# rikuu/Gap2Seq

Measured on AMD Instinct MI355X. Metric: gaps filled/sec (whole node), k=31 synthetic 3 Mbp DBG, higher is better.
Workload: dtype u32

## Files before the change

### gap2seq_amd/csrc/d3_device.h

```cpp
#pragma once
#include <hip/hip_runtime_api.h>
#include <stdint.h>

#include "d2_device.h"
#include "fill_device.h"

#define G2S_D3_BLOCK_VARS 16u
#define G2S_RAND_BLOCK 4096u
#define G2S_RAND_WINDOW 160u
#define G2S_D3_TABLE_BUDGET (8u << 20)

#define G2S_D3_UNHANDLED 0x1u
#define G2S_D3_BUDGET 0x2u
#define G2S_D3_ANOMALY 0x4u

namespace g2s {

struct D3Gap {
  uint64_t arena_off;
  int32_t skip_thr;
  uint16_t lmf;
  uint8_t kind;
  uint8_t pad;
};

struct D3HostItem {
  uint32_t gap, n_segs;
  uint64_t seg_off;
  uint64_t rnd_off;
  uint32_t draws;
  uint32_t pad;
};
struct D3Side {
  D3HostItem* items = nullptr;
  GapOut* outs = nullptr;
  SegRec* segs = nullptr;
  uint32_t* rnd = nullptr;
  uint64_t cap_items = 0, cap_segs = 0, cap_rnd = 0;
  unsigned long long* count = nullptr;
};

struct alignas(16) D3Var {
  uint32_t gap, R, toff, tile0;
  uint32_t base, dmin, dspread, ns;
  uint64_t sub_at;
  uint32_t start_seg, start_t;
  int32_t len0, len1, n_len;
  uint32_t pad;
};
struct alignas(16) D3Trace {
  uint64_t arena_off;
  uint64_t sub_at;
  uint32_t gi;
  uint32_t off, want;
  uint16_t lmf, nsegs;
};
static_assert(sizeof(D3Var) == 64 && sizeof(D3Trace) == 32, "record layouts");

struct D3Summary {
  uint32_t status, unhandled, n_var, anomalies;
  unsigned long long host_items, host_segs, host_rnd;
  uint32_t handoff_waves, tiles;
  uint64_t table_entries, block_entries;
  uint64_t draws_min, draws_spread, draws_total;
  uint64_t xA, sA, xB, sB, xD, sD, segs, fill_bytes;
  uint32_t seg_gaps, filled;
  uint32_t rand_state[31];
  uint32_t trace_waves;
  uint32_t big_gaps;
  uint32_t traced_gaps;
  uint32_t spec_gaps;
  uint32_t handoff_gaps;
};
static_assert(sizeof(D3Summary) <= 512, "the lap stamps live at byte 512 of the summary's slot");

struct RandTables {
  const uint32_t* hi = nullptr;
  const uint32_t* mid = nullptr;
  const uint32_t* lane = nullptr;
};
void rand_tables_host(uint32_t* hi , uint32_t* mid , uint32_t* lane );

struct D3Work {
  uint32_t* ginfo = nullptr;
  uint32_t* dmin = nullptr;
  uint32_t* dspread = nullptr;
  uint32_t* base = nullptr;
  uint32_t* vrank = nullptr;
  uint32_t* var_gap = nullptr;
  uint32_t* var_R = nullptr;
  uint32_t* var_toff = nullptr;
  uint32_t* var_tile = nullptr;
  uint32_t* blk_toff = nullptr;
  uint32_t* blk_in = nullptr;
  uint32_t* dvar = nullptr;
  int32_t* skip = nullptr;
  uint32_t* tile_var = nullptr;
  D3Var* vdesc = nullptr;
  D3Trace* tdesc = nullptr;
  uint32_t* host_slot = nullptr;
  D3HostItem* hitems = nullptr;
  uint16_t* tab = nullptr;
  uint32_t* btab = nullptr;
  D3Summary* sum = nullptr;
  unsigned long long* fill_bytes = nullptr;
  uint32_t* link = nullptr;
  const D2Out* d2out = nullptr;
  const uint32_t* d2runs = nullptr;
  uint64_t* hops = nullptr;
  const char* spec_text = nullptr;
  const uint32_t* spec_res = nullptr;
  uint8_t* tab_bad = nullptr;
};
size_t d3_work_bytes(uint32_t n);
void d3_work_carve(void* p, uint32_t n, D3Work* w);

struct D3Params {
  int32_t k, skip_confident, all_paths, unique_paths;
  uint64_t max_states;
  uint64_t arena_base;
  uint32_t n;
  uint32_t has_skip;
  uint32_t seg_cap;
  uint32_t map_cap;
  uint32_t group_size;
  uint64_t sub_region;
  uint32_t laps;
  uint32_t self_clean;
  uint32_t base0, R0, d_in;
  const unsigned long long* d2_done;
  uint32_t d2_wgs;
  uint32_t restart;
};

hipError_t launch_rand_fill(hipStream_t st, uint32_t* rnd_all, const RandTables& rt, const D3Summary* sum_dev, uint64_t capacity,
                            uint64_t first_value = 0);

hipError_t launch_d3_sharded_classes(hipStream_t st, const D3Params& P, const D3Work& W, const GapOut* outs, const D3Gap* dgaps,
                                     bool summary_is_clean);
hipError_t launch_d3_sharded_tables(hipStream_t st, const D3Params& P, const D3Work& W, const GapOut* outs, const SubRec* sub,
                                    uint32_t* rnd_all, uint64_t rnd_capacity, uint32_t* group_fn );
hipError_t launch_d3_sharded_trace(hipStream_t st, const D3Params& P, const D3Work& W, const GapOut* outs, const SubRec* sub,
                                   const char* lastch_up, const char* lastch_dn, uint32_t* rnd_all, uint64_t rnd_capacity,
                                   void* results, char* arena, const D3Side& side, void* summary_host,
                                   hipEvent_t ev_d2 = nullptr );

hipError_t launch_rand_window(hipStream_t st, uint32_t* rnd_all, const uint32_t* link);

hipError_t launch_d3(hipStream_t st, const D3Params& P, const D3Work& W, const GapDev* gaps, const GapOut* outs,
                     const D3Gap* dgaps, const SubRec* sub, const char* lastch_up, const char* lastch_dn,
                     const RandTables& rt, uint32_t* rnd_all ,
                     uint64_t rnd_capacity, void* results ,
                     char* arena , const D3Side& side ,
                     void* summary_host ,
                     bool summary_is_clean ,
                     uint32_t* clean_words ,
                     hipEvent_t ev_chain = nullptr ,
                     hipEvent_t ev_d2 = nullptr ,
                     hipEvent_t ev_stop = nullptr );

hipError_t test_d3_tables(const uint32_t* segs, uint32_t nsegs, int32_t n_len, int32_t len0, int32_t len1, uint32_t start_seg,
                          const uint32_t* rnd, uint64_t rnd_cap, uint32_t base, uint32_t R, uint32_t dmin, uint32_t dspread,
                          uint16_t* entries, uint8_t* bad, uint32_t* anomalies);

uint64_t d3_chain_launches();

}
```

### gap2seq_amd/csrc/d3_device.hip

```cpp
#include "sync_debug.h"
#include <hip/hip_runtime.h>
#include <hip/hip_ext.h>

#include <algorithm>
#include <atomic>
#include <cstddef>
#include <cstdlib>
#include <cstring>
#include <mutex>
#include <set>
#include <vector>

#include "../../include/g2s.h"
#include "d3_device.h"
#include "envcache.hpp"

namespace {

using g2s::D3Gap;
using g2s::D3Params;
using g2s::D3Summary;
using g2s::D3Work;

__device__ __forceinline__ uint32_t uni(uint32_t x) { return (uint32_t)__builtin_amdgcn_readfirstlane((int)x); }

#define GI_CLASS(x) ((x) & 3u)
#define GI_FILLED 0x4u
#define GI_SKIPPED 0x8u
#define GI_BAD 0x10u
#define GI_MEM 0x20u
#define GI_PHASE_D 0x40u
#define D3_TILE 256u
#define GI_HOST 0x80u

__device__ __forceinline__ void stamp(const D3Work& W, int slot) {
  ((unsigned long long*)((char*)W.sum + 512))[slot] = wall_clock64();
}

__device__ __forceinline__ const SubRec* sub_of(const D3Params& P, const SubRec* sub, uint32_t i) {
  return sub + (uint64_t)(i / P.group_size) * P.sub_region;
}

__device__ __forceinline__ int gap_count(const GapOut& go, const D3Params& P, bool phase_d) {
  if (phase_d && !P.skip_confident && P.all_paths) return go.count_s;
  return go.c_count;
}

__device__ __forceinline__ uint32_t dpp_scan_add(uint32_t x) {
  x += (uint32_t)__builtin_amdgcn_update_dpp(0, (int)x, 0x111, 0xF, 0xF, false);
  x += (uint32_t)__builtin_amdgcn_update_dpp(0, (int)x, 0x112, 0xF, 0xF, false);
  x += (uint32_t)__builtin_amdgcn_update_dpp(0, (int)x, 0x114, 0xF, 0xF, false);
  x += (uint32_t)__builtin_amdgcn_update_dpp(0, (int)x, 0x118, 0xF, 0xF, false);
  x += (uint32_t)__builtin_amdgcn_update_dpp(0, (int)x, 0x142, 0xA, 0xF, false);
  x += (uint32_t)__builtin_amdgcn_update_dpp(0, (int)x, 0x143, 0xC, 0xF, false);
  return x;
}
__device__ __forceinline__ uint32_t sat_add(uint32_t a, uint32_t b) { const uint32_t t = a + b; return t < a ? 0xFFFFFFFFu : t; }
__device__ __forceinline__ uint32_t dpp_scan_sat(uint32_t x) {
  x = sat_add(x, (uint32_t)__builtin_amdgcn_update_dpp(0, (int)x, 0x111, 0xF, 0xF, false));
  x = sat_add(x, (uint32_t)__builtin_amdgcn_update_dpp(0, (int)x, 0x112, 0xF, 0xF, false));
  x = sat_add(x, (uint32_t)__builtin_amdgcn_update_dpp(0, (int)x, 0x114, 0xF, 0xF, false));
  x = sat_add(x, (uint32_t)__builtin_amdgcn_update_dpp(0, (int)x, 0x118, 0xF, 0xF, false));
  x = sat_add(x, (uint32_t)__builtin_amdgcn_update_dpp(0, (int)x, 0x142, 0xA, 0xF, false));
  x = sat_add(x, (uint32_t)__builtin_amdgcn_update_dpp(0, (int)x, 0x143, 0xC, 0xF, false));
  return x;
}
__device__ __forceinline__ uint32_t dpp_sum(uint32_t x) { return (uint32_t)__builtin_amdgcn_readlane((int)dpp_scan_add(x), 63); }
__device__ __forceinline__ unsigned long long wave_add64(unsigned long long v) {
  const unsigned long long lo = dpp_sum((uint32_t)v & 0xFFFFFFu), mid = dpp_sum((uint32_t)(v >> 24) & 0xFFFFFFu), hi = dpp_sum((uint32_t)(v >> 48));
  return lo + (mid << 24) + (hi << 48);
}

__device__ __forceinline__ uint32_t d3_classify_body(const D3Params& P, const D3Work& W, const GapOut* __restrict__ outs,
                                                     const D3Gap* __restrict__ dgaps, uint32_t first, uint32_t stride,
                                                     uint32_t* l_gi, uint32_t* l_dm, uint32_t* l_ds, int32_t* l_sk,
                                                     unsigned long long* red, bool one_wg) {
  const uint32_t n = P.n;
  unsigned long long xA = 0, sA = 0, xB = 0, sB = 0, xD = 0, sD = 0, segs = 0;
  uint32_t unhandled = 0, seg_gaps = 0, big = 0, traced = 0, spec = 0, handoff = 0;
  for (uint32_t i = first; i < n; i += stride) {
    const D3Gap dg = dgaps[i];
    const GapOut& go = outs[i];
    const uint32_t flags = go.flags, n_states = go.n_states, n_right = go.n_right, x_right = go.x_right, x_left = go.x_left;
    const uint32_t x_sub = go.x_sub, n_sub = go.n_sub, nseg_b = go.stat[3], dflags = go.dflags, stop0 = go.stop[0], stop1 = go.stop[1];
    const int c_count = go.c_count, n_len = go.n_len, len0 = go.len[0], len1 = go.len[1], reached_j = go.reached_j, count_s = go.count_s;
    const uint32_t n_xl = go.n_xl;
    const uint64_t sub_off = go.sub_off;
    uint32_t gi = 0, dmin = 0, spread = 0;
    if (dg.kind != 0) gi = GI_BAD;
    else {
      if (flags & (G2S_DEV_OVERFLOW_A | G2S_DEV_OVERFLOW_B)) unhandled++;
      else if ((uint64_t)n_states > P.max_states || (uint64_t)n_right > P.max_states) gi = GI_MEM;
      else {
        xA += x_right; sA += n_right; xB += x_left; sB += n_states; xD += x_sub; sD += n_sub;
        segs += nseg_b;
        seg_gaps++;
        if (flags & G2S_DEV_BIG) big++;
        if (dflags & G2S_DEVA_TRACED) traced++;
        if (dflags & G2S_DEVA_SPEC) spec++;
        const bool phase_d = c_count > 0 && n_len > 0;
        const bool by_host = phase_d && !(dflags & (G2S_DEVA_ANALYSED | G2S_DEVA_D2_PENDING));
        const int cnt = (phase_d && !P.skip_confident && P.all_paths) ? count_s : c_count;
        if (cnt > 0 && (!P.unique_paths || cnt == 1)) gi |= GI_FILLED;
        if (n_len > 0) gi |= ((uint32_t)reached_j & 0xFFu) << 8;
        if (phase_d) {
          gi |= GI_PHASE_D;
          if (by_host) gi |= GI_HOST;
          if (by_host || (!P.skip_confident && (dflags & G2S_DEVA_D2_PENDING))) handoff++;
          int lo_d = 0x7FFFFFFF, hi_d = 0;
#pragma unroll
          for (int q = 0; q < 2; q++) {
            if (q >= n_len) continue;
            const uint32_t sw = q ? stop1 : stop0;
            const int lq = q ? len1 : len0;
            int lo = (int)(sw & 0xFFFFu), hi = (int)(sw >> 16);
            if (lo > hi || hi > (int)dg.lmf) { lo = 0; hi = (int)dg.lmf; }
            lo_d = min(lo_d, 1 + lq - hi);
            hi_d = max(hi_d, 1 + lq - lo);
          }
          lo_d = max(lo_d, 1);
          hi_d = max(hi_d, lo_d);
          dmin = (uint32_t)lo_d;
          spread = (uint32_t)(hi_d - lo_d);
          gi |= spread ? 2u : 1u;
        }
      }
    }
    gi |= (uint32_t)dg.lmf << 16;
    W.ginfo[i] = gi;
    W.dmin[i] = dmin;
    W.dspread[i] = spread;
    W.skip[i] = dg.skip_thr;
    if (l_gi) { l_gi[i] = gi; l_dm[i] = dmin; l_ds[i] = spread; l_sk[i] = dg.skip_thr; }
    uint4 h0;
    const uint64_t ao = P.arena_base + dg.arena_off, sa = (uint64_t)(i / P.group_size) * P.sub_region + sub_off;
    h0.x = (uint32_t)ao; h0.y = (uint32_t)(ao >> 32); h0.z = (uint32_t)sa; h0.w = (uint32_t)(sa >> 32);
    ((uint4*)&W.tdesc[i])[0] = h0;
    (void)n_xl;
  }
  xA = wave_add64(xA); sA = wave_add64(sA); xB = wave_add64(xB); sB = wave_add64(sB); xD = wave_add64(xD); sD = wave_add64(sD);
  segs = wave_add64(segs);
  const unsigned long long cnts = wave_add64(((unsigned long long)unhandled << 32) | seg_gaps);
  big = dpp_sum(big);
  if ((threadIdx.x & 63u) == 0u && big) atomicAdd(&W.sum->big_gaps, big);
  traced = dpp_sum(traced);
  if ((threadIdx.x & 63u) == 0u && traced) atomicAdd(&W.sum->traced_gaps, traced);
  spec = dpp_sum(spec);
  if ((threadIdx.x & 63u) == 0u && spec) atomicAdd(&W.sum->spec_gaps, spec);
  handoff = dpp_sum(handoff);
  if ((threadIdx.x & 63u) == 0u && handoff) atomicAdd(&W.sum->handoff_gaps, handoff);
  const uint32_t wave = threadIdx.x >> 6, nwaves = blockDim.x >> 6;
  if ((threadIdx.x & 63u) == 0u) {
    unsigned long long* r = red + wave * 8u;
    r[0] = xA; r[1] = sA; r[2] = xB; r[3] = sB; r[4] = xD; r[5] = sD; r[6] = segs; r[7] = cnts;
  }
  __syncthreads();
  unsigned long long tot = 0;
  if (threadIdx.x < 8u) for (uint32_t w = 0; w < nwaves; w++) tot += red[w * 8u + threadIdx.x];
  unsigned long long all_cnts = 0;
  for (uint32_t w = 0; w < nwaves; w++) all_cnts += red[w * 8u + 7u];
  D3Summary* S = W.sum;
  if (threadIdx.x < 7u) {
    unsigned long long* dst = (unsigned long long*)&S->xA + threadIdx.x;
    if (one_wg) *dst = tot; else if (tot) atomicAdd(dst, tot);
  } else if (threadIdx.x == 7u) {
    if (one_wg) { S->unhandled = (uint32_t)(tot >> 32); S->seg_gaps = (uint32_t)tot; }
    else {
      if (tot >> 32) atomicAdd(&S->unhandled, (uint32_t)(tot >> 32));
      if (tot & 0xFFFFFFFFull) atomicAdd(&S->seg_gaps, (uint32_t)tot);
    }
  }
  return (uint32_t)(all_cnts >> 32);
}
__global__ __launch_bounds__(256) void g2s_d3_classify(const D3Params P, const D3Work W, const GapOut* __restrict__ outs,
                                                       const D3Gap* __restrict__ dgaps) {
  __shared__ unsigned long long red[4 * 8];
  (void)d3_classify_body(P, W, outs, dgaps, blockIdx.x * blockDim.x + threadIdx.x, gridDim.x * blockDim.x, nullptr, nullptr, nullptr, nullptr, red, false);
}

__device__ __forceinline__ void block_scan3(uint64_t& a, uint64_t& b, uint32_t& c, uint64_t* sh , uint64_t* tot_a, uint64_t* tot_b,
                                            uint32_t* tot_c) {
  const int lane = (int)(threadIdx.x & 63u), wave = (int)(threadIdx.x >> 6);
  uint64_t ia = a, ib = b;
  uint32_t ic = c;
  for (int o = 1; o < 64; o <<= 1) {
    const uint64_t ya = __shfl_up(ia, o), yb = __shfl_up(ib, o);
    const uint32_t yc = __shfl_up(ic, o);
    if (lane >= o) { ia += ya; ib += yb; ic += yc; }
  }
  if (lane == 63) { sh[wave * 3] = ia; sh[wave * 3 + 1] = ib; sh[wave * 3 + 2] = ic; }
  __syncthreads();
  uint64_t wa = lane < 16 ? sh[lane * 3] : 0, wb = lane < 16 ? sh[lane * 3 + 1] : 0, wc = lane < 16 ? sh[lane * 3 + 2] : 0;
  for (int o = 1; o < 16; o <<= 1) {
    const uint64_t ya = __shfl_up(wa, o), yb = __shfl_up(wb, o), yc = __shfl_up(wc, o);
    if (lane >= o) { wa += ya; wb += yb; wc += yc; }
  }
  *tot_a = __shfl(wa, 15); *tot_b = __shfl(wb, 15); *tot_c = (uint32_t)__shfl(wc, 15);
  const uint64_t oa = wave ? __shfl(wa, wave - 1) : 0, ob = wave ? __shfl(wb, wave - 1) : 0, oc = wave ? __shfl(wc, wave - 1) : 0;
  a = oa + ia - a; b = ob + ib - b; c = (uint32_t)oc + ic - c;
}

__device__ __forceinline__ void block_scan3_short(uint32_t& a, uint32_t& b, uint32_t& c, uint32_t* sh , uint32_t* tot_a, uint32_t* tot_b,
                                                  uint32_t* tot_c) {
  const int lane = (int)(threadIdx.x & 63u), wave = (int)(threadIdx.x >> 6);
  const uint32_t ia = dpp_scan_add(a), ib = dpp_scan_add(b), ic = dpp_scan_sat(c);
  if (lane == 63) { sh[wave * 3] = ia; sh[wave * 3 + 1] = ib; sh[wave * 3 + 2] = ic; }
  __syncthreads();
  uint32_t wa = lane < 16 ? sh[lane * 3] : 0u, wb = lane < 16 ? sh[lane * 3 + 1] : 0u, wc = lane < 16 ? sh[lane * 3 + 2] : 0u;
  wa = dpp_scan_add(wa); wb = dpp_scan_add(wb); wc = dpp_scan_sat(wc);
  *tot_a = (uint32_t)__builtin_amdgcn_readlane((int)wa, 15); *tot_b = (uint32_t)__builtin_amdgcn_readlane((int)wb, 15);
  *tot_c = (uint32_t)__builtin_amdgcn_readlane((int)wc, 15);
  const int wp = (int)uni((uint32_t)max(wave - 1, 0));
  const uint32_t oa = wave ? (uint32_t)__builtin_amdgcn_readlane((int)wa, wp) : 0u, ob = wave ? (uint32_t)__builtin_amdgcn_readlane((int)wb, wp) : 0u;
  const uint32_t oc = wave ? (uint32_t)__builtin_amdgcn_readlane((int)wc, wp) : 0u;
  a = oa + ia - a; b = ob + ib - b;
  const uint32_t incl_c = sat_add(oc, ic);
  c = incl_c == 0xFFFFFFFFu ? 0xFFFFFFFFu : incl_c - c;
}

__device__ __forceinline__ void d3_scan_body(const D3Params& P, const D3Work& W, const GapOut* __restrict__ outs, uint32_t* gi_a,
                                             uint32_t* dm_a, uint32_t* ds_a, const int32_t* sk_a, bool dual, uint32_t unhandled,
                                             uint64_t* sh , uint32_t* sh_f , bool short_list ) {
  const uint32_t t = threadIdx.x, n = P.n;
  const uint32_t per = (n + 1023u) / 1024u;
  const uint32_t lo = min(n, t * per), hi = min(n, lo + per);
  if (P.has_skip) {
    auto s_of = [&](uint32_t i) -> bool {
      if (i == 0) return false;
      const int thr = sk_a[i];
      if (thr < 0) return false;
      const uint32_t pg = gi_a[i - 1];
      return (pg & GI_FILLED) && !(pg & (GI_BAD | GI_MEM)) && (int)((pg >> 8) & 0xFFu) > thr;
    };
    bool o0 = false, o1 = true;
    for (uint32_t i = lo; i < hi; i++) { const bool s = s_of(i); o0 = s && !o0; o1 = s && !o1; }
    sh_f[t] = (o0 ? 1u : 0u) | (o1 ? 2u : 0u);
    __syncthreads();
    if (t < 64u) {
      auto apply = [](uint32_t f, bool in) -> bool { return in ? (f & 2u) != 0 : (f & 1u) != 0; };
      uint32_t f = 2u;
      for (uint32_t q = 0; q < 16u; q++) { const uint32_t g = sh_f[t * 16u + q]; f = (apply(g, apply(f, false)) ? 1u : 0u) | (apply(g, apply(f, true)) ? 2u : 0u); }
      uint32_t inc = f;
      for (int o = 1; o < 64; o <<= 1) {
        const uint32_t pv = (uint32_t)__shfl_up((int)inc, o);
        if ((int)t >= o) inc = (apply(inc, apply(pv, false)) ? 1u : 0u) | (apply(inc, apply(pv, true)) ? 2u : 0u);
      }
      uint32_t before = (uint32_t)__shfl_up((int)inc, 1);
      if (t == 0) before = 2u;
      bool cur = apply(before, false);
      for (uint32_t q = 0; q < 16u; q++) { const uint32_t g = sh_f[t * 16u + q]; sh_f[t * 16u + q] = cur ? 1u : 0u; cur = apply(g, cur); }
    }
    __syncthreads();
    bool sk = sh_f[t] != 0;
    for (uint32_t i = lo; i < hi; i++) {
      sk = s_of(i) && !sk;
      if (sk) {
        const uint32_t g = (gi_a[i] & ~3u) | GI_SKIPPED;
        gi_a[i] = g; dm_a[i] = 0; ds_a[i] = 0;
        if (dual) { W.ginfo[i] = g; W.dmin[i] = 0; W.dspread[i] = 0; }
      }
    }
    __threadfence_block();
    __syncthreads();
  }
  auto load8 = [&](uint32_t i0, uint32_t* g8, uint32_t* m8, uint32_t* s8) {
#pragma unroll
    for (int q = 0; q < 8; q++) {
      const uint32_t i = i0 + (uint32_t)q;
      const bool have = i < hi;
      g8[q] = have ? gi_a[i] : GI_SKIPPED;
      m8[q] = have ? dm_a[i] : 0u;
      s8[q] = have ? ds_a[i] : 0u;
    }
  };
  if (t == 0) stamp(W, 20);
  uint64_t sd = 0, ss = 0;
  uint32_t nv = 0;
  for (uint32_t i0 = lo; i0 < hi; i0 += 8u) {
    uint32_t g8[8], m8[8], s8[8];
    load8(i0, g8, m8, s8);
#pragma unroll
    for (int q = 0; q < 8; q++) {
      if (g8[q] & GI_SKIPPED) continue;
      sd += m8[q];
      if (GI_CLASS(g8[q]) == 2u) { nv++; ss += s8[q]; }
    }
  }
  uint64_t tot_d, tot_s;
  uint32_t V;
  if (short_list) {
    uint32_t a = (uint32_t)sd, b = (uint32_t)ss, ta, tb;
    block_scan3_short(a, b, nv, (uint32_t*)sh, &ta, &tb, &V);
    sd = a; ss = b; tot_d = ta; tot_s = tb;
  } else block_scan3(sd, ss, nv, sh, &tot_d, &tot_s, &V);
  if (t == 0) stamp(W, 21);
  const bool too_wide = tot_d + tot_s + P.base0 + P.R0 >= 0xFFFF0000ull || tot_s + P.R0 >= (uint64_t)G2S_D3_TABLE_BUDGET;
  uint64_t my_tab = 0, my_blk = 0;
  uint32_t my_tiles = 0;
  {
    uint64_t d = sd + P.base0, r = ss + P.R0;
    uint32_t v = nv;
    for (uint32_t i0 = lo; i0 < hi; i0 += 8u) {
      uint32_t g8[8], m8[8], s8[8];
      load8(i0, g8, m8, s8);
#pragma unroll
      for (int q = 0; q < 8; q++) {
        const uint32_t i = i0 + (uint32_t)q;
        if (i >= hi) break;
        W.base[i] = (uint32_t)d;
        W.vrank[i] = v;
        if (g8[q] & GI_SKIPPED) continue;
        d += m8[q];
        if (GI_CLASS(g8[q]) == 2u) {
          W.var_gap[v] = i;
          W.var_R[v] = (uint32_t)r;
          my_tab += r + 1u;
          my_tiles += (uint32_t)((r + D3_TILE) / D3_TILE);
          if (v % G2S_D3_BLOCK_VARS == 0u) my_blk += r + 1u;
          v++;
          r += s8[q];
        }
      }
    }
    if (t == 1023u) W.var_R[V] = (uint32_t)tot_s + P.R0;
  }
  if (t == 0) stamp(W, 22);
  uint64_t to = my_tab, bo = my_blk, T, TB;
  uint32_t tl = my_tiles, tiles;
  if (short_list) {
    uint32_t b = (uint32_t)std::min<uint64_t>(bo, 0xFFFFFFFFull), c = (uint32_t)std::min<uint64_t>(to, 0xFFFFFFFFull), tb, tc;
    block_scan3_short(tl, b, c, (uint32_t*)(sh + 48), &tiles, &tb, &tc);
    bo = b; to = c; TB = tb; T = tc == 0xFFFFFFFFu ? ~0ull : tc;
  } else block_scan3(to, bo, tl, sh + 48, &T, &TB, &tiles);
  const bool over = too_wide || T > (uint64_t)G2S_D3_TABLE_BUDGET || TB > (uint64_t)(G2S_D3_TABLE_BUDGET / 4u);
  if (!over) {
    uint64_t d = sd + P.base0, r = ss + P.R0;
    uint32_t v = nv;
    for (uint32_t i0 = lo; i0 < hi; i0 += 8u) {
      uint32_t g8[8], m8[8], s8[8];
      load8(i0, g8, m8, s8);
#pragma unroll
      for (int q = 0; q < 8; q++) {
        if (g8[q] & GI_SKIPPED) continue;
        const uint32_t base_i = (uint32_t)d;
        d += m8[q];
        if (GI_CLASS(g8[q]) != 2u) continue;
        W.var_toff[v] = (uint32_t)to;
        W.var_tile[v] = tl;
        {
          const uint32_t i = i0 + (uint32_t)q;
          uint4 h0, h1;
          h0.x = i; h0.y = (uint32_t)r; h0.z = (uint32_t)to; h0.w = tl;
          h1.x = base_i; h1.y = m8[q]; h1.z = s8[q]; h1.w = 0u;
          ((uint4*)&W.vdesc[v])[0] = h0;
          ((uint4*)&W.vdesc[v])[1] = h1;
        }
        tl += (uint32_t)((r + D3_TILE) / D3_TILE);
        to += r + 1u;
        if (v % G2S_D3_BLOCK_VARS == 0u) { W.blk_toff[v / G2S_D3_BLOCK_VARS] = (uint32_t)bo; bo += r + 1u; }
        v++;
        r += s8[q];
      }
    }
    if (t == 1023u) { W.var_toff[V] = (uint32_t)T; W.var_tile[V] = tiles; W.blk_toff[(V + G2S_D3_BLOCK_VARS - 1u) / G2S_D3_BLOCK_VARS] = (uint32_t)TB; }
    __threadfence_block();
    __syncthreads();
    for (uint32_t v = t; v < V; v += 1024u) {
      const uint4 h0 = ((const uint4*)&W.vdesc[v])[0];
      const uint32_t i = h0.x, r = h0.y, tl0 = h0.w;
      const GapOut& go = outs[i];
      uint4 h2, h3;
      const uint64_t sa = (uint64_t)(i / P.group_size) * P.sub_region + go.sub_off;
      ((uint32_t*)&W.vdesc[v])[7] = go.n_xl;
      h2.x = (uint32_t)sa; h2.y = (uint32_t)(sa >> 32); h2.z = go.start_seg; h2.w = go.start_t;
      h3.x = (uint32_t)go.len[0]; h3.y = (uint32_t)go.len[1]; h3.z = (uint32_t)go.n_len; h3.w = 0u;
      ((uint4*)&W.vdesc[v])[2] = h2;
      ((uint4*)&W.vdesc[v])[3] = h3;
      const uint32_t nt = (r + D3_TILE) / D3_TILE;
      for (uint32_t x = 0; x < nt; x++) W.tile_var[tl0 + x] = v;
    }
  }
  if (t == 0) {
    stamp(W, 23);
    D3Summary* S = W.sum;
    S->status = (unhandled ? G2S_D3_UNHANDLED : 0u) | (over ? G2S_D3_BUDGET : 0u);
    S->n_var = V;
    S->tiles = over ? 0u : tiles;
    S->table_entries = T;
    S->block_entries = TB;
    S->draws_min = tot_d;
    S->draws_spread = tot_s;
  }
}
#define D3_SCAN_LDS_GAPS 12288u
__global__ __launch_bounds__(1024) void g2s_d3_scan(const D3Params P, const D3Work W, const GapOut* __restrict__ outs) {
  extern __shared__ __attribute__((aligned(16))) uint32_t dyn[];
  __shared__ uint64_t sh[96];
  __shared__ uint32_t sh_f[1024];
  if (P.n <= D3_SCAN_LDS_GAPS) {
    uint32_t *l_gi = dyn, *l_dm = dyn + P.n, *l_ds = dyn + 2u * P.n;
    for (uint32_t i = threadIdx.x; i < P.n; i += 1024u) { l_gi[i] = W.ginfo[i]; l_dm[i] = W.dmin[i]; l_ds[i] = W.dspread[i]; }
    const uint32_t unhandled = W.sum->unhandled;
    __syncthreads();
    d3_scan_body(P, W, outs, l_gi, l_dm, l_ds, W.skip, true, unhandled, sh, sh_f, true);
    return;
  }
  d3_scan_body(P, W, outs, W.ginfo, W.dmin, W.dspread, W.skip, false, W.sum->unhandled, sh, sh_f, P.n <= 262144u);
}

__global__ __launch_bounds__(64) void g2s_rand_window(uint32_t* __restrict__ Wd, const uint32_t* __restrict__ link) {
  __shared__ uint32_t w[G2S_RAND_WINDOW + 2];
  const uint32_t lane = threadIdx.x;
  if (lane < 31u) w[lane] = link[lane];
  __syncthreads();
  for (uint32_t i = 31u; i < G2S_RAND_WINDOW; i += 3u) {
    if (lane < 3u) w[i + lane] = w[i + lane - 31u] + w[i + lane - 3u];
    __syncthreads();
  }
  for (uint32_t i = lane; i < G2S_RAND_WINDOW; i += 64u) Wd[i] = w[i];
}
__global__ __launch_bounds__(64) void g2s_rand_fill(uint32_t* __restrict__ Wd, const g2s::RandTables rt, const D3Summary* sum,
                                                    uint64_t capacity, uint64_t first_block) {
  __shared__ uint32_t base[G2S_RAND_WINDOW], s1[96], s2[64];
  if (sum && sum->status) return;
  const uint64_t need = sum ? min(capacity, sum->draws_min + sum->draws_spread + 64ull) : capacity;
  const uint32_t lane = threadIdx.x;
  for (uint32_t i = lane; i < G2S_RAND_WINDOW; i += 64u) base[i] = Wd[i];
  __syncthreads();
  const uint64_t nblocks = (need + G2S_RAND_BLOCK - 1u) / G2S_RAND_BLOCK;
  for (uint64_t B = first_block + blockIdx.x; B < nblocks; B += gridDim.x) {
    const uint32_t* ph = rt.hi + (size_t)((B >> 8) & 127u) * 31u;
    const uint32_t* pm = rt.mid + (size_t)(B & 255u) * 31u;
    const uint32_t* pl = rt.lane + (size_t)lane * 31u;
    for (uint32_t i = lane; i < 91u; i += 64u) {
      uint32_t a = 0;
#pragma unroll
      for (int j = 0; j < 31; j++) a += ph[j] * base[i + (uint32_t)j];
      s1[i] = a;
    }
    __syncthreads();
    if (lane < 61u) {
      uint32_t a = 0;
#pragma unroll
      for (int j = 0; j < 31; j++) a += pm[j] * s1[lane + (uint32_t)j];
      s2[lane] = a;
    }
    __syncthreads();
    uint32_t c[31], r[31];
#pragma unroll
    for (int j = 0; j < 31; j++) c[j] = pl[j];
#pragma unroll
    for (int i = 0; i < 31; i++) {
      uint32_t a = 0;
#pragma unroll
      for (int j = 0; j < 31; j++) a += c[j] * s2[i + j];
      r[i] = a;
    }
    uint32_t* out = Wd + 31u + B * G2S_RAND_BLOCK + (uint64_t)lane * 64u;
    const uint64_t room = capacity > B * G2S_RAND_BLOCK + (uint64_t)lane * 64u ? capacity - (B * G2S_RAND_BLOCK + (uint64_t)lane * 64u) : 0ull;
#pragma unroll
    for (int q = 0; q < 64; q++) {
      const uint32_t v = r[q % 31] + r[(q + 28) % 31];
      r[q % 31] = v;
      if ((uint64_t)q < room) out[q] = v;
    }
    __syncthreads();
  }
}

struct SegW { uint32_t node, depth_len, cnt, ts_tt, par01, par23, flags, pad; };

__device__ __forceinline__ int seg_nparents(uint32_t p01, uint32_t p23) {
  return ((p01 & 0xFFFFu) != 0xFFFFu) + ((p01 >> 16) != 0xFFFFu) + ((p23 & 0xFFFFu) != 0xFFFFu) + ((p23 >> 16) != 0xFFFFu);
}
__device__ __forceinline__ uint32_t seg_parent(uint32_t p01, uint32_t p23, int sel) {
  const uint32_t ps[4] = {p01 & 0xFFFFu, p01 >> 16, p23 & 0xFFFFu, p23 >> 16};
  uint32_t chosen = 0xFFFFu;
  int idx = 0;
#pragma unroll
  for (int q = 0; q < 4; q++)
    if (ps[q] != 0xFFFFu) { if (idx == sel) chosen = ps[q]; idx++; }
  return chosen;
}

__device__ __forceinline__ int pick_parent(uint32_t rv, int nb) { return nb == 2 ? (int)(rv & 1u) : nb == 3 ? (int)(rv % 3u) : (int)(rv & 3u); }

struct SegLite { uint32_t depth_len, par01, par23, flags; };

__device__ __forceinline__ SegLite seg_lite(const SegLite* p, int i) { return p[i]; }
__device__ __forceinline__ SegLite seg_lite(const SegW* p, int i) {
  SegLite l;
  l.depth_len = p[i].depth_len; l.par01 = p[i].par01; l.par23 = p[i].par23; l.flags = p[i].flags;
  return l;
}
template <typename SegT>
__device__ int d3_walk_count(int n_len, int len0, int len1, uint32_t start_seg, uint32_t start_t, int nsegs,
                             const SegT* __restrict__ segs, const uint32_t* lwin ,
                             uint32_t nwin , uint64_t avail ,
                             bool* bad) {
  int draws = 1;
  if (avail < 1 || nwin < 1) { *bad = true; return draws; }
  const int pick = n_len > 1 ? (int)((lwin[0] >> 1) & 1u) : 0;
  int d2 = pick ? len1 : len0;
  const uint32_t sg = (start_seg >> (16 * pick)) & 0xFFFFu;
  int i = sg == 0xFFFFu ? -1 : (int)sg;
  int t = (int)((start_t >> (16 * pick)) & 0xFFFFu);
  if (i < 0 || i >= nsegs) { *bad = true; return draws; }
  SegLite s = seg_lite(segs, i);
  bool ended = false;
  for (int guard = 0; d2 >= 0; guard++) {
    if (guard > 70000) { *bad = true; break; }
    const int run = min(t, d2);
    draws += run; d2 -= run; t -= run;
    if (t == 0 && (s.flags & G2S_SUB_SOURCE)) { ended = true; break; }
    if (d2 > 0) {
      const int nb = seg_nparents(s.par01, s.par23);
      if (nb == 0 || (nb > 1 && !(s.flags & G2S_SEG_ORDERED)) || (uint64_t)draws >= avail || (uint32_t)draws >= nwin) { *bad = true; break; }
      const uint32_t rv = nb > 1 ? lwin[draws] >> 1 : 0u;
      draws++;
      i = (int)seg_parent(s.par01, s.par23, nb == 1 ? 0 : pick_parent(rv, nb));
// ... 221 lines not shown
      const uint32_t v = uni(u == uni(u_first) ? v_unit : W.tile_var[tile]);
      const uint4* vp = (const uint4*)&W.vdesc[v];
      const uint4 h0 = vp[0], h1 = vp[1], h2 = vp[2], h3 = vp[3];
      static_assert(offsetof(g2s::D3Var, R) == 4 && offsetof(g2s::D3Var, toff) == 8 && offsetof(g2s::D3Var, tile0) == 12 && offsetof(g2s::D3Var, base) == 16 &&
                    offsetof(g2s::D3Var, dmin) == 20 && offsetof(g2s::D3Var, dspread) == 24 && offsetof(g2s::D3Var, ns) == 28 && offsetof(g2s::D3Var, sub_at) == 32 &&
                    offsetof(g2s::D3Var, start_seg) == 40 && offsetof(g2s::D3Var, len0) == 48 && offsetof(g2s::D3Var, len1) == 52 && offsetof(g2s::D3Var, n_len) == 56, "D3Var by words");
      const uint32_t R = uni(h0.y), toff = h0.z, tile0 = uni(h0.w), base = uni(h1.x), dmin = h1.y, dspread = h1.z, ns = uni(h1.w);
      const uint32_t d = (tile - tile0) * D3_TILE + u % D3_TILE;
      if (stw) stamp(W, 5);
      if (d > R || ns > D3_TAB_SEGS) continue;
      worked = true;
      const uint64_t sub_at = (uint64_t)uni(h2.x) | ((uint64_t)uni(h2.y) << 32);
      const uint64_t at = (uint64_t)base + d;
      bool bad = false;
      const int draws = d3_count_wave((int)uni(h3.z), (int)h3.x, (int)h3.y, h2.z, ns, (const SegW*)(sub + sub_at), rnd + at,
                                      min(win_cap, dmin + dspread + 1u), capacity > at ? capacity - at : 0ull, jmp, dep, &bad);
      if (stw) stamp(W, 6);
      const int dev = draws - (int)dmin;
      if (dev < 0 || dev > (int)dspread) bad = true;
      if ((tid & 63u) == 0u) {
        W.tab[(uint64_t)toff + d] = bad ? (uint16_t)0 : (uint16_t)dev;
        if (W.tab_bad) W.tab_bad[(uint64_t)toff + d] = bad ? 1 : 0;
        bad_any |= bad;
      }
    }
  }
  for (uint32_t tile = blockIdx.x; tile < tiles; tile += gridDim.x) {
    if (by_wave && tile == blockIdx.x && ns_first <= D3_TAB_SEGS) continue;
    const uint32_t v = tile == blockIdx.x ? v_first : W.tile_var[tile];
    const g2s::D3Var vd = W.vdesc[v];
    const uint32_t ns = vd.ns;
    if (by_wave && ns <= D3_TAB_SEGS) continue;
    worked = true;
    const uint32_t d0 = (tile - vd.tile0) * D3_TILE, d = d0 + tid;
    const uint64_t at0 = (uint64_t)vd.base + d0;
    const bool mine = d <= vd.R;
    const uint32_t want = min(win_cap, min(vd.R - d0, D3_TILE - 1u) + vd.dmin + vd.dspread + 1u);
    if (st0 && !by_wave) stamp(W, 5);
    __syncthreads();
    {
      const SegW* gs = (const SegW*)(sub + vd.sub_at);
      const uint32_t in_lds = ns <= D3_TAB_SEGS ? ns : 0u;
#pragma unroll
      for (uint32_t it = 0; it < D3_TAB_SEGS / 256u; it++) {
        const uint32_t q = tid + 256u * it;
        if (q >= in_lds) continue;
        SegLite l;
        l.depth_len = gs[q].depth_len; l.par01 = gs[q].par01; l.par23 = gs[q].par23; l.flags = gs[q].flags;
        lseg[q] = l;
      }
      for (uint32_t x = tid; x < want; x += 256u) lwin[x] = at0 + x < capacity ? rnd[at0 + x] : 0u;
    }
    __syncthreads();
    if (st0 && !by_wave) stamp(W, 6);
    if (mine) {
      bool bad = false;
      const uint64_t at = at0 + tid;
      const uint32_t nw = want > tid ? want - tid : 0u;
      const uint64_t av = capacity > at ? capacity - at : 0ull;
      const int draws = ns > D3_TAB_SEGS
                            ? d3_walk_count(vd.n_len, vd.len0, vd.len1, vd.start_seg, vd.start_t, (int)ns, (const SegW*)(sub + vd.sub_at), lwin + tid, nw, av, &bad)
                            : d3_walk_count_lite(vd.n_len, vd.len0, vd.len1, vd.start_seg, (int)ns, lseg, lwin + tid, nw, av, &bad);
      const int dev = draws - (int)vd.dmin;
      if (dev < 0 || dev > (int)vd.dspread) bad = true;
      W.tab[(uint64_t)vd.toff + d] = bad ? (uint16_t)0 : (uint16_t)dev;
      if (W.tab_bad) W.tab_bad[(uint64_t)vd.toff + d] = bad ? 1 : 0;
      bad_any |= bad;
    }
  }
  if (bad_any) atomicAdd(&W.sum->anomalies, 1u);
  if (st0) stamp(W, 7);
  if (P.laps && (tid & 63u) == 0u) {
    unsigned long long* laps = (unsigned long long*)((char*)W.sum + 512);
    if (worked) atomicMax(&laps[32], wall_clock64());
    if (tid == 0) atomicMax(&laps[33], wall_clock64());
  }
}

__device__ __forceinline__ void d3_blocks_body(const D3Work& W, uint64_t first, uint64_t stride) {
  const D3Summary* S = W.sum;
  const uint32_t V = S->n_var;
  const uint32_t NB = (V + G2S_D3_BLOCK_VARS - 1u) / G2S_D3_BLOCK_VARS;
  const uint64_t TB = S->block_entries;
  for (uint64_t e = first; e < TB; e += stride) {
    uint32_t lo = 0, hi = NB;
    while (hi - lo > 1u) { const uint32_t mid = (lo + hi) >> 1; if ((uint64_t)W.blk_toff[mid] <= e) lo = mid; else hi = mid; }
    const uint32_t b = lo;
    uint32_t d = (uint32_t)(e - W.blk_toff[b]);
    const uint32_t v1 = min(V, (b + 1u) * G2S_D3_BLOCK_VARS);
    for (uint32_t v = b * G2S_D3_BLOCK_VARS; v < v1; v++) d += W.tab[(uint64_t)W.var_toff[v] + d];
    W.btab[e] = d;
  }
}
__global__ __launch_bounds__(256) void g2s_d3_blocks(const D3Work W) {
  if (W.sum->status) return;
  d3_blocks_body(W, (uint64_t)blockIdx.x * blockDim.x + threadIdx.x, (uint64_t)gridDim.x * blockDim.x);
}

__device__ __forceinline__ void d3_chain_body(const D3Work& W, const uint32_t* __restrict__ Wd, uint32_t* total_dev ,
                                              uint32_t base0 = 0u, uint32_t d_in = 0u) {
  D3Summary* S = W.sum;
  const uint32_t V = S->n_var;
  const uint32_t NB = (V + G2S_D3_BLOCK_VARS - 1u) / G2S_D3_BLOCK_VARS;
  __shared__ uint32_t l_toff[2048], l_in[2048];
  const bool in_lds = NB <= 2048u;
  if (in_lds) for (uint32_t b = threadIdx.x; b < NB; b += blockDim.x) l_toff[b] = W.blk_toff[b];
  __syncthreads();
  if (threadIdx.x == 0) {
    uint32_t d = d_in;
    if (in_lds) for (uint32_t b = 0; b < NB; b++) { l_in[b] = d; d = W.btab[(uint64_t)l_toff[b] + d]; }
    else for (uint32_t b = 0; b < NB; b++) { W.blk_in[b] = d; d = W.btab[(uint64_t)W.blk_toff[b] + d]; }
    W.dvar[V] = d;
    *total_dev = d;
  }
  __threadfence_block();
  __syncthreads();
  for (uint32_t b = threadIdx.x; b < NB; b += blockDim.x) {
    uint32_t d = in_lds ? l_in[b] : W.blk_in[b];
    if (in_lds) W.blk_in[b] = d;
    const uint32_t v0 = b * G2S_D3_BLOCK_VARS, v1 = min(V, (b + 1u) * G2S_D3_BLOCK_VARS);
    uint32_t toff[G2S_D3_BLOCK_VARS];
#pragma unroll
    for (uint32_t q = 0; q < G2S_D3_BLOCK_VARS; q++) toff[q] = v0 + q < v1 ? W.var_toff[v0 + q] : 0u;
#pragma unroll
    for (uint32_t q = 0; q < G2S_D3_BLOCK_VARS; q++)
      if (v0 + q < v1) { W.dvar[v0 + q] = d; d += W.tab[(uint64_t)toff[q] + d]; }
  }
  const uint64_t total = (uint64_t)base0 + S->draws_min + *total_dev;
  if (threadIdx.x == 0) S->draws_total = total;
  if (threadIdx.x < 31u) {
    const uint32_t w = Wd[total + threadIdx.x];
    S->rand_state[threadIdx.x] = w;
    if (W.link) W.link[threadIdx.x] = w;
  }
}
__global__ __launch_bounds__(1024) void g2s_d3_chain(const D3Work W, const uint32_t* __restrict__ Wd, uint32_t base0, uint32_t d_in) {
  __shared__ uint32_t total_dev;
  if (W.sum->status) return;
  d3_chain_body(W, Wd, &total_dev, base0, d_in);
}
__global__ __launch_bounds__(256) void g2s_d3_groupfn(const D3Work W, uint32_t R0, uint32_t* __restrict__ fn) {
  const D3Summary* S = W.sum;
  if (S->status) return;
  const uint32_t V = S->n_var;
  const uint32_t NB = (V + G2S_D3_BLOCK_VARS - 1u) / G2S_D3_BLOCK_VARS;
  for (uint32_t d0 = blockIdx.x * blockDim.x + threadIdx.x; d0 <= R0; d0 += gridDim.x * blockDim.x) {
    uint32_t d = d0;
    for (uint32_t b = 0; b < NB; b++) d = W.btab[(uint64_t)W.blk_toff[b] + d];
    fn[d0] = d;
  }
}

#define D3_FRONT_GAPS 3072u
__global__ __launch_bounds__(1024) void g2s_d3_front(const D3Params P, const D3Work W, const GapOut* __restrict__ outs,
                                                     const D3Gap* __restrict__ dgaps) {
  __shared__ uint64_t sh[96];
  __shared__ unsigned long long red[16 * 8];
  __shared__ uint32_t sh_f[1024];
  __shared__ uint32_t l_gi[D3_FRONT_GAPS], l_dm[D3_FRONT_GAPS], l_ds[D3_FRONT_GAPS];
  __shared__ int32_t l_sk[D3_FRONT_GAPS];
  if (threadIdx.x == 0) stamp(W, 0);
  const uint32_t unhandled = d3_classify_body(P, W, outs, dgaps, threadIdx.x, 1024u, l_gi, l_dm, l_ds, l_sk, red, true);
  __syncthreads();
  if (threadIdx.x == 0) stamp(W, 1);
  d3_scan_body(P, W, outs, l_gi, l_dm, l_ds, l_sk, true, unhandled, sh, sh_f, true);
  if (threadIdx.x == 0) stamp(W, 2);
}

template <bool RESTART>
__device__ __forceinline__ bool d3_handoff_body(const D3Params& P, const D3Work& W, const GapOut* __restrict__ outs,
                                                const SubRec* __restrict__ sub, const uint32_t* __restrict__ rnd, uint64_t capacity,
                                                const g2s::D3Side& side, uint32_t i0, const uint32_t* ldvar, const uint16_t* ltab,
                                                const uint32_t* ltoff, unsigned long long* lcur) {
  D3Summary* S = W.sum;
  const int lane = (int)(threadIdx.x & 63u);
  const uint32_t mine = i0 + (uint32_t)lane;
  const bool have = mine < P.n;
  uint32_t gi = 0, my_off = 0, my_want = 0, my_ns = 0;
  if (have) {
    gi = W.ginfo[mine];
    const uint32_t dmin = W.dmin[mine];
    const GapOut& go = outs[mine];
    my_ns = go.n_xl;
    if ((gi & GI_PHASE_D) && !P.skip_confident) {
      const uint32_t dfl = go.dflags;
      if ((dfl & G2S_DEVA_D2_PENDING) && (dfl & G2S_DEVA_D2_FAILED)) gi |= GI_HOST;
    }
    my_want = dmin;
    if constexpr (RESTART) {
      if (GI_CLASS(gi) == 2u) {
        const uint32_t dspread = W.dspread[mine];
        const uint4 h0 = ((const uint4*)&W.tdesc[mine])[0];
        const SegW* gs = (const SegW*)(sub + ((uint64_t)h0.z | ((uint64_t)h0.w << 32)));
        const uint32_t nwin = min(P.map_cap + D3_TILE, dmin + dspread + 1u);
        bool bad = false;
        const int draws = my_ns > D3_TAB_SEGS
                              ? d3_walk_count(go.n_len, go.len[0], go.len[1], go.start_seg, go.start_t, (int)my_ns, gs, rnd, nwin, capacity, &bad)
                              : d3_walk_count_lite(go.n_len, go.len[0], go.len[1], go.start_seg, (int)my_ns, gs, rnd, nwin, capacity, &bad);
        const int dev = draws - (int)dmin;
        if (dev < 0 || dev > (int)dspread) bad = true;
        if (bad) atomicAdd(&S->anomalies, 1u);
        else my_want += (uint32_t)dev;
      }
    } else {
      const uint32_t vr = W.vrank[mine], base = W.base[mine];
      const uint32_t dv = ldvar ? ldvar[vr] : W.dvar[vr];
      my_off = base + dv;
      if (GI_CLASS(gi) == 2u) my_want += ltab ? (uint32_t)ltab[ltoff[vr] + dv] : (uint32_t)W.tab[(uint64_t)W.var_toff[vr] + dv];
    }
    ((uint4*)&W.tdesc[mine])[1] = make_uint4(gi, my_off, my_want, (gi >> 16) | (min(my_ns, 0xFFFFu) << 16));
  }
  const bool host = have && (gi & GI_HOST) != 0u;
  const uint64_t hm = __ballot(host);
  for (uint64_t m = hm; m; m &= m - 1) {
    const int l = __builtin_ctzll(m);
    const uint32_t i = i0 + (uint32_t)l;
    const uint32_t off = (uint32_t)__shfl((int)my_off, l), want = (uint32_t)__shfl((int)my_want, l), ns = (uint32_t)__shfl((int)my_ns, l);
    unsigned long long it = 0, so = 0, ro = 0;
    if (lane == 0) {
      if (lcur) {
        it = atomicAdd(&lcur[0], 1ull); so = atomicAdd(&lcur[1], (unsigned long long)ns); ro = atomicAdd(&lcur[2], ((unsigned long long)want + 8ull) / 8ull);
      } else {
        it = atomicAdd(&S->host_items, 1ull);
        so = atomicAdd(&S->host_segs, (unsigned long long)ns);
        ro = atomicAdd(&S->host_rnd, ((unsigned long long)want + 8ull) / 8ull);
      }
    }
    it = __shfl(it, 0); so = __shfl(so, 0); ro = __shfl(ro, 0);
    if (it >= side.cap_items || so + ns > side.cap_segs || ro + (want + 8ull) / 8ull > side.cap_rnd || (uint64_t)off + want + 1ull > capacity) {
      if (lane == 0) { atomicAdd(&S->anomalies, 1u); W.host_slot[i] = 0xFFFFFFFFu; }
      continue;
    }
    if (lane == 0) {
      g2s::D3HostItem h;
      h.gap = i; h.n_segs = ns; h.seg_off = so; h.rnd_off = ro; h.draws = want; h.pad = 0;
      W.hitems[it] = h;
      W.host_slot[i] = (uint32_t)it;
      uint32_t* hi = (uint32_t*)&side.items[it];
      hi[0] = i; hi[1] = ns; hi[2] = (uint32_t)so; hi[3] = (uint32_t)(so >> 32); hi[4] = (uint32_t)ro; hi[5] = (uint32_t)(ro >> 32); hi[6] = want;
    }
  }
  if (hm != 0ull) __threadfence_system();
  (void)sub; (void)rnd; (void)outs;
  if constexpr (RESTART) {
    const uint32_t nv = (uint32_t)__popcll(__ballot(have && GI_CLASS(gi) == 2u));
    uint32_t mx = have ? my_want : 0u;
    for (int o = 32; o > 0; o >>= 1) mx = max(mx, (uint32_t)__shfl_xor((int)mx, o));
    if (lane == 0) {
      if (nv) atomicAdd(&S->n_var, nv);
      atomicMax((unsigned long long*)&S->draws_total, (unsigned long long)mx);
    }
  }
  return hm != 0ull;
}
__global__ __launch_bounds__(64) void g2s_d3_handoff(const D3Params P, const D3Work W, const GapOut* __restrict__ outs,
                                                     const SubRec* __restrict__ sub, const uint32_t* __restrict__ rnd, uint64_t capacity,
                                                     const g2s::D3Side side) {
  D3Summary* S = W.sum;
  const bool dead = S->status != 0u;
  if (!dead) (void)d3_handoff_body<false>(P, W, outs, sub, rnd, capacity, side, blockIdx.x * 64u, nullptr, nullptr, nullptr, nullptr);
  if ((threadIdx.x & 63u) == 0u) {
    asm volatile("s_waitcnt vmcnt(0)" ::: "memory");
    const unsigned int done = atomicAdd(&S->handoff_waves, 1u) + 1u;
    if (done == gridDim.x) {
      const unsigned long long items = atomicAdd(&S->host_items, 0ull);
      const uint32_t anomalies = atomicAdd(&S->anomalies, 0u);
      __hip_atomic_store(side.count, (items & 0x7FFFFFFFFFFFFFFFull) | ((unsigned long long)((anomalies || dead) ? 1u : 0u) << 63),
                         __ATOMIC_RELEASE, __HIP_MEMORY_SCOPE_SYSTEM);
    }
  }
}
__global__ __launch_bounds__(256) void g2s_d3_restart(const D3Params P, const D3Work W, const GapOut* __restrict__ outs,
                                                      const D3Gap* __restrict__ dgaps, const SubRec* __restrict__ sub,
                                                      const uint32_t* __restrict__ rnd, uint64_t capacity, const g2s::D3Side side) {
  __shared__ unsigned long long red[4 * 8];
  D3Summary* S = W.sum;
  (void)d3_classify_body(P, W, outs, dgaps, blockIdx.x * 256u + threadIdx.x, gridDim.x * 256u, nullptr, nullptr, nullptr, nullptr, red, false);
  (void)d3_handoff_body<true>(P, W, outs, sub, rnd, capacity, side, blockIdx.x * 256u + (threadIdx.x & ~63u), nullptr, nullptr, nullptr, nullptr);
  if ((threadIdx.x & 63u) == 0u) {
    asm volatile("s_waitcnt vmcnt(0)" ::: "memory");
    const unsigned int done = atomicAdd(&S->handoff_waves, 1u) + 1u;
    if (done == gridDim.x * 4u) {
      const unsigned long long items = atomicAdd(&S->host_items, 0ull);
      const uint32_t anomalies = atomicAdd(&S->anomalies, 0u), unhandled = atomicAdd(&S->unhandled, 0u);
      S->status = unhandled ? G2S_D3_UNHANDLED : 0u;
      __hip_atomic_store(side.count, (items & 0x7FFFFFFFFFFFFFFFull) | ((unsigned long long)((anomalies || unhandled) ? 1u : 0u) << 63),
                         __ATOMIC_RELEASE, __HIP_MEMORY_SCOPE_SYSTEM);
    }
  }
}
#define D3_BACK_TAB 24576u
#define D3_CHAIN_GAPS 768u
#define D3_CHAIN_ROOM 4096u
__global__ __launch_bounds__(1024) void g2s_d3_back(const D3Params P, const D3Work W, const GapOut* __restrict__ outs,
                                                    const SubRec* __restrict__ sub, const uint32_t* __restrict__ Wd, uint64_t capacity,
                                                    const g2s::D3Side side) {
  __shared__ uint32_t total_dev;
  __shared__ unsigned long long lcur[3];
  if (threadIdx.x < 3u) lcur[threadIdx.x] = 0ull;
  __shared__ uint16_t ltab[D3_BACK_TAB];
  __shared__ uint32_t ltoff[1025], ldvar[1025];
  D3Summary* S = W.sum;
  if (threadIdx.x == 0) stamp(W, 8);
  const uint32_t status = S->status, V = S->n_var;
  const uint64_t T = S->table_entries;
  if (status) {
    if (threadIdx.x == 0) __hip_atomic_store(side.count, 1ull << 63, __ATOMIC_RELEASE, __HIP_MEMORY_SCOPE_SYSTEM);
    return;
  }
  const bool in_lds = T <= (uint64_t)D3_BACK_TAB && V <= 1024u;
  if (in_lds) {
    for (uint32_t e = threadIdx.x; e < (uint32_t)T; e += 1024u) ltab[e] = W.tab[e];
    if (threadIdx.x <= V) ltoff[threadIdx.x] = W.var_toff[threadIdx.x];
    __syncthreads();
    if (threadIdx.x == 0) {
      stamp(W, 9);
      uint32_t d = 0;
      for (uint32_t v = 0; v < V; v++) { ldvar[v] = d; d += ltab[ltoff[v] + d]; }
      ldvar[V] = d;
      total_dev = d;
    }
    __syncthreads();
    if (threadIdx.x <= V) W.dvar[threadIdx.x] = ldvar[threadIdx.x];
    const uint64_t total = S->draws_min + total_dev;
    if (threadIdx.x == 0) S->draws_total = total;
    if (threadIdx.x < 31u) {
      const uint32_t w = Wd[total + threadIdx.x];
      S->rand_state[threadIdx.x] = w;
      if (W.link) W.link[threadIdx.x] = w;
    }
  } else {
    d3_blocks_body(W, threadIdx.x, 1024u);
    __threadfence();
    __syncthreads();
    d3_chain_body(W, Wd, &total_dev);
    __threadfence();
    __syncthreads();
  }
  if (threadIdx.x == 0) stamp(W, 10);
  for (uint32_t i0 = (threadIdx.x >> 6) * 64u; i0 < P.n; i0 += 1024u)
    (void)d3_handoff_body<false>(P, W, outs, sub, Wd + 31, capacity, side, i0, in_lds ? ldvar : nullptr, in_lds ? ltab : nullptr,
                          in_lds ? ltoff : nullptr, lcur);
  __syncthreads();
  if (threadIdx.x == 0) {
    stamp(W, 11);
    const unsigned long long items = lcur[0];
    S->host_items = items; S->host_segs = lcur[1]; S->host_rnd = lcur[2];
    const uint32_t anomalies = atomicAdd(&S->anomalies, 0u);
    __hip_atomic_store(side.count, (items & 0x7FFFFFFFFFFFFFFFull) | ((unsigned long long)(anomalies ? 1u : 0u) << 63), __ATOMIC_RELEASE,
                       __HIP_MEMORY_SCOPE_SYSTEM);
    stamp(W, 12);
  }
}

template <int NW, bool CHAIN = false>
__global__ __launch_bounds__(64 * NW) void g2s_d3_trace(const D3Params P, const D3Work W, GapOut* __restrict__ outs,
                                                   const SubRec* __restrict__ sub, const char* __restrict__ chu,
                                                   const char* __restrict__ chd, const uint32_t* __restrict__ rnd,
                                                   uint64_t capacity, g2s_result* __restrict__ results,
                                                   char* __restrict__ arena, uint32_t* __restrict__ summary_host,
                                                   const g2s::D3Side side, uint32_t* __restrict__ clean_words ,
                                                   uint32_t chain_room ) {
  static_assert(!CHAIN || NW == 4, "the chain's loads are laid out for 256 threads");
  extern __shared__ __attribute__((aligned(16))) uint32_t lds[];
  D3Summary* S = W.sum;
  const uint32_t i = blockIdx.x;
  constexpr int NT = 64 * NW;
  const int tid = (int)threadIdx.x, lane = tid & 63;
  const bool w0 = tid < 64;
#ifdef G2S_SYNC_DEBUG
  auto wg_sync = [&]() { if constexpr (NW > 1) __syncthreads(); else { g2s_sync_jitter(0xD3u); g2s_wait_all(); asm volatile("s_waitcnt lgkmcnt(0)" ::: "memory"); __builtin_amdgcn_wave_barrier(); } };
#else
  auto wg_sync = [&]() { if constexpr (NW > 1) __syncthreads(); else { asm volatile("s_waitcnt lgkmcnt(0)" ::: "memory"); __builtin_amdgcn_wave_barrier(); } };
#endif
  SegW* segs = (SegW*)lds;
  static_assert(sizeof(g2s_result) == 112, "g2s_result layout");
  unsigned long long* laps = (unsigned long long*)((char*)W.sum + 512);
  const unsigned long long tk0 = P.laps ? wall_clock64() : 0ull;
  unsigned long long tk1 = 0, tk2 = 0, tk3 = 0, hops = 0, tkm = 0;
  if (P.laps && i == 0 && tid == 0) laps[13] = tk0;
  const uint32_t status = uni(S->status);
  struct {
    uint32_t flags, dflags, start_seg, start_t, sub_vertices, sub_edges, top_level;
    int32_t c_count, n_len, len[2], reached_j, count_s;
  } go;
  {
    const GapOut& g = outs[i];
    go.top_level = uni(g.top_level);
    go.flags = uni(g.flags); go.dflags = uni(g.dflags); go.start_seg = uni(g.start_seg); go.start_t = uni(g.start_t);
    go.sub_vertices = uni(g.sub_vertices); go.sub_edges = uni(g.sub_edges);
    go.c_count = (int32_t)uni((uint32_t)g.c_count); go.n_len = (int32_t)uni((uint32_t)g.n_len);
    go.len[0] = (int32_t)uni((uint32_t)g.len[0]); go.len[1] = (int32_t)uni((uint32_t)g.len[1]);
    go.reached_j = (int32_t)uni((uint32_t)g.reached_j); go.count_s = (int32_t)uni((uint32_t)g.count_s);
  }
  g2s::D3Trace td;
  uint32_t c_dmin = 0, c_vr = 0, c_base = 0, c_V = 0, c_dev = 0, c_step = 0, c_ns = 0, c_handoff = 0;
  uint64_t c_T = 0, c_draws_min = 0;
  if constexpr (!CHAIN) {
    const uint4 h0 = ((const uint4*)&W.tdesc[i])[0], h1 = ((const uint4*)&W.tdesc[i])[1];
    td.arena_off = (uint64_t)uni(h0.x) | ((uint64_t)uni(h0.y) << 32);
    td.sub_at = (uint64_t)uni(h0.z) | ((uint64_t)uni(h0.w) << 32);
    td.gi = uni(h1.x); td.off = uni(h1.y); td.want = uni(h1.z);
    td.lmf = (uint16_t)(uni(h1.w) & 0xFFFFu); td.nsegs = (uint16_t)(uni(h1.w) >> 16);
  } else {
    const uint32_t n = P.n;
    const uint32_t toff_len = (n + 2u) & ~1u;
    const uint32_t tab_room = chain_room > toff_len ? min(chain_room - toff_len, D3_CHAIN_ROOM) & ~1u : 0u;
    uint16_t* ltoff = (uint16_t*)lds;
    uint16_t* ltab = ltoff + toff_len;
    const uint4 h0 = ((const uint4*)&W.tdesc[i])[0];
    uint32_t gi_w = W.ginfo[i], dm_w = W.dmin[i], vr_w = W.vrank[i], bs_w = W.base[i], ns_w = outs[i].n_xl, V_w = S->n_var;
    c_T = S->table_entries;
    c_draws_min = S->draws_min;
    uint32_t hg_w = S->handoff_gaps;
    static_assert(D3_CHAIN_ROOM <= 8u * 2u * 256u && D3_CHAIN_GAPS <= 4u * 256u, "the unrolled loads below cover the room");
    uint32_t tw[8], ow[4];
    const uint32_t* tab32 = (const uint32_t*)W.tab;
    const uint32_t tab_last = max(tab_room / 2u, 1u) - 1u;
#pragma unroll
    for (uint32_t q = 0; q < 8u; q++) tw[q] = tab32[min((uint32_t)tid + 256u * q, tab_last)];
#pragma unroll
    for (uint32_t q = 0; q < 4u; q++) ow[q] = W.var_toff[min((uint32_t)tid + 256u * q, n)];
#pragma unroll
    for (uint32_t q = 0; q < 8u; q++) { const uint32_t x = (uint32_t)tid + 256u * q; if (x < tab_room / 2u) ((uint32_t*)ltab)[x] = tw[q]; }
#pragma unroll
    for (uint32_t q = 0; q < 4u; q++) { const uint32_t x = (uint32_t)tid + 256u * q; if (x <= n) ltoff[x] = (uint16_t)ow[q]; }
    td.arena_off = (uint64_t)uni(h0.x) | ((uint64_t)uni(h0.y) << 32);
    td.sub_at = (uint64_t)uni(h0.z) | ((uint64_t)uni(h0.w) << 32);
    td.gi = uni(gi_w); td.off = 0u; td.want = 0u;
    td.lmf = (uint16_t)(td.gi >> 16);
    c_ns = uni(ns_w);
    td.nsegs = (uint16_t)min(c_ns, 0xFFFFu);
    c_dmin = uni(dm_w); c_vr = uni(vr_w); c_base = uni(bs_w); c_V = uni(V_w); c_handoff = uni(hg_w);
    c_T = (uint64_t)uni((uint32_t)c_T) | ((uint64_t)uni((uint32_t)(c_T >> 32)) << 32);
    c_draws_min = (uint64_t)uni((uint32_t)c_draws_min) | ((uint64_t)uni((uint32_t)(c_draws_min >> 32)) << 32);
    __syncthreads();
    if (!status) {
      const bool in_lds = c_T <= (uint64_t)tab_room && c_T <= 0xFFFFull && c_V <= n;
      const uint32_t v0 = min(c_vr, c_V), var = GI_CLASS(td.gi) == 2u && v0 < c_V ? 1u : 0u;
      const uint32_t v_end = i + 1u == n ? c_V : v0 + var;
      uint32_t d = 0, dv = 0, d1 = 0;
      if (in_lds) {
        uint32_t t = ltoff[0];
        for (uint32_t v = 0; v < v_end; v++) {
          const uint32_t tn = ltoff[v + 1u];
          if (v == v0) dv = d;
          d += ltab[min(t + d, tab_room - 1u)];
          if (v == v0) d1 = d;
          t = tn;
        }
      } else {
        for (uint32_t v = 0; v < v_end; v++) {
          if (v == v0) dv = d;
          d += W.tab[min((uint64_t)W.var_toff[v] + d, (uint64_t)G2S_D3_TABLE_BUDGET - 1u)];
          if (v == v0) d1 = d;
        }
      }
      if (v_end <= v0) dv = d;
      c_dev = uni(dv);
      c_step = var ? uni(d1) - c_dev : 0u;
      td.off = c_base + c_dev;
      td.want = c_dmin + c_step;
      if (i + 1u == n && w0) {
        const uint32_t d_all = uni(d);
        const uint64_t total = c_draws_min + d_all;
        if (lane == 0) {
          W.dvar[c_V] = d_all;
          __hip_atomic_store((unsigned long long*)&S->draws_total, (unsigned long long)total, __ATOMIC_RELAXED, __HIP_MEMORY_SCOPE_AGENT);
        }
        if (lane < 31) {
          const uint32_t w = (rnd - 31)[total + (uint32_t)lane];
          __hip_atomic_store(&S->rand_state[lane], w, __ATOMIC_RELAXED, __HIP_MEMORY_SCOPE_AGENT);
          if (W.link) W.link[lane] = w;
        }
        __threadfence();
      }
    }
    __syncthreads();
  }
  bool d2_lost = false;
  if ((go.dflags & G2S_DEVA_D2_PENDING) && !(go.dflags & (G2S_DEVA_RUNS | G2S_DEVA_D2_FAILED)) && !P.skip_confident) {
    uint32_t v = go.dflags;
    for (uint32_t spin = 0; spin < (1u << 22) && !(v & (G2S_DEVA_RUNS | G2S_DEVA_D2_FAILED)); spin++) {
      __builtin_amdgcn_s_sleep(8);
      v = uni(__hip_atomic_load(&outs[i].dflags, __ATOMIC_ACQUIRE, __HIP_MEMORY_SCOPE_AGENT));
    }
    __builtin_amdgcn_fence(__ATOMIC_ACQUIRE, "agent");
    go.dflags = v;
    go.sub_vertices = uni(__hip_atomic_load(&outs[i].sub_vertices, __ATOMIC_RELAXED, __HIP_MEMORY_SCOPE_AGENT));
    go.sub_edges = uni(__hip_atomic_load(&outs[i].sub_edges, __ATOMIC_RELAXED, __HIP_MEMORY_SCOPE_AGENT));
    if (!(v & (G2S_DEVA_RUNS | G2S_DEVA_D2_FAILED))) d2_lost = true;
  }
  uint32_t h_it = 0xFFFFFFFFu, h_ns = 0, h_want = 0;
  uint64_t h_so = 0, h_ro = 0;
  bool lost_counted = false;
  if constexpr (CHAIN) {
    const bool counts = (td.gi & GI_HOST) || ((td.gi & GI_PHASE_D) && !P.skip_confident && (go.dflags & G2S_DEVA_D2_PENDING));
    if (!status && !d2_lost) {
      if ((td.gi & GI_PHASE_D) && !P.skip_confident && (go.dflags & G2S_DEVA_D2_PENDING) && (go.dflags & G2S_DEVA_D2_FAILED)) td.gi |= GI_HOST;
      if (td.gi & GI_HOST) {
        __shared__ unsigned long long l_hand[3];
        if (tid == 0) {
          const uint32_t ns = c_ns, want = td.want;
          unsigned long long it = atomicAdd(&S->host_items, 1ull);
          const unsigned long long so = atomicAdd(&S->host_segs, (unsigned long long)ns);
          const unsigned long long ro = atomicAdd(&S->host_rnd, ((unsigned long long)want + 8ull) / 8ull);
          if (it >= side.cap_items || so + ns > side.cap_segs || ro + (want + 8ull) / 8ull > side.cap_rnd || (uint64_t)td.off + want + 1ull > capacity) {
            atomicAdd(&S->anomalies, 1u);
            it = 0xFFFFFFFFull;
          } else {
            uint32_t* hi = (uint32_t*)&side.items[it];
            hi[0] = i; hi[1] = ns; hi[2] = (uint32_t)so; hi[3] = (uint32_t)(so >> 32); hi[4] = (uint32_t)ro; hi[5] = (uint32_t)(ro >> 32); hi[6] = want;
            __threadfence_system();
          }
          l_hand[0] = it; l_hand[1] = so; l_hand[2] = ro;
        }
        __syncthreads();
        h_it = uni((uint32_t)l_hand[0]);
        h_so = (uint64_t)uni((uint32_t)l_hand[1]) | ((uint64_t)uni((uint32_t)(l_hand[1] >> 32)) << 32);
        h_ro = (uint64_t)uni((uint32_t)l_hand[2]) | ((uint64_t)uni((uint32_t)(l_hand[2] >> 32)) << 32);
        h_ns = c_ns; h_want = td.want;
      }
    }
    if (tid == 0 && (counts || (c_handoff == 0u && i == 0u))) {
      if (d2_lost && !status) { atomicAdd(&S->anomalies, 1u); lost_counted = true; }
      asm volatile("s_waitcnt vmcnt(0)" ::: "memory");
      const unsigned int done = counts ? atomicAdd(&S->handoff_waves, 1u) + 1u : 0u;
      if (done == c_handoff) {
        const unsigned long long items = atomicAdd(&S->host_items, 0ull);
        const uint32_t anomalies = atomicAdd(&S->anomalies, 0u);
        __hip_atomic_store(side.count, (items & 0x7FFFFFFFFFFFFFFFull) | ((unsigned long long)((anomalies || status) ? 1u : 0u) << 63),
                           __ATOMIC_RELEASE, __HIP_MEMORY_SCOPE_SYSTEM);
      }
    }
  }
  if ((go.dflags & G2S_DEVA_D2_PENDING) && (go.dflags & G2S_DEVA_D2_FAILED) && !(td.gi & GI_HOST) && (td.gi & GI_PHASE_D)) d2_lost = true;
  uint32_t gsp_all = 0, gsp_sent = 0;
  auto leave = [&](uint32_t fill_len) {
    if (!w0) return;
    uint32_t last = 0;
    if (lane == 0) {
      if (P.laps) {
        const unsigned long long tk4 = wall_clock64();
        atomicMax(&laps[14], tk1 ? tk1 - tk0 : 0ull); atomicMax(&laps[15], tk2 ? tk2 - tk1 : 0ull);
        atomicMax(&laps[16], tk3 ? tk3 - tk2 : 0ull); atomicMax(&laps[17], ((tk4 - tk0) << 24) | ((td.gi & GI_HOST) ? 1ull << 23 : 0ull) | (unsigned long long)(i & 0x7FFFFFu)); atomicMax(&laps[18], tk4);
        atomicMax(&laps[19], ((tk2 ? tk2 - tk1 : 0ull) << 32) | (hops << 16) | (tkm ? tkm - tk1 : 0ull));
        if ((P.laps >> 4) == i + 1u) { laps[26] = tk0; laps[27] = tk1; laps[28] = tkm; laps[29] = tk2; laps[30] = tk3; laps[31] = tk4; }
      }
      const uint32_t c = i & 63u, n = gridDim.x;
      const unsigned long long before = atomicAdd(&W.fill_bytes[c * 16u], (unsigned long long)fill_len | (1ull << 40));
      if (gsp_all) atomicAdd(&W.fill_bytes[c * 16u + 1u], (unsigned long long)gsp_all | ((unsigned long long)gsp_sent << 32));
      if ((uint32_t)(before >> 40) + 1u == (n + 63u - c) / 64u) last = atomicAdd(&S->trace_waves, 1u) + 1u == min(n, 64u) ? 1u : 0u;
    }
    if (P.self_clean && (uint32_t)lane < sizeof(GapOut) / 4u) ((uint32_t*)&outs[i])[lane] = 0u;
    if (!uni(last)) return;
    if (P.d2_done && lane == 0)
      for (uint32_t spin = 0; spin < (1u << 22) && __hip_atomic_load(P.d2_done, __ATOMIC_ACQUIRE, __HIP_MEMORY_SCOPE_AGENT) < (unsigned long long)P.d2_wgs; spin++)
        __builtin_amdgcn_s_sleep(8);
    uint32_t* src = (uint32_t*)S;
    if (P.laps && lane == 0) laps[24] = wall_clock64();
    static_assert(sizeof(D3Summary) <= 512, "two words a lane");
    const uint32_t s0 = __hip_atomic_load(src + lane, __ATOMIC_RELAXED, __HIP_MEMORY_SCOPE_AGENT);
    const uint32_t s1 = __hip_atomic_load(src + 64 + lane, __ATOMIC_RELAXED, __HIP_MEMORY_SCOPE_AGENT);
    const unsigned long long* cl = (const unsigned long long*)(src + 256 + 32 * lane);
    const unsigned long long c0 = __hip_atomic_load(cl, __ATOMIC_RELAXED, __HIP_MEMORY_SCOPE_AGENT);
    const unsigned long long c1 = __hip_atomic_load(cl + 1, __ATOMIC_RELAXED, __HIP_MEMORY_SCOPE_AGENT);
    summary_host[lane] = s0;
    summary_host[64 + lane] = s1;
    ((unsigned long long*)(summary_host + 256 + 32 * lane))[0] = c0;
    ((unsigned long long*)(summary_host + 256 + 32 * lane))[1] = c1;
    if (P.self_clean) {
      src[lane] = 0u; src[64 + lane] = 0u;
      ((unsigned long long*)(src + 256 + 32 * lane))[0] = 0ull;
      ((unsigned long long*)(src + 256 + 32 * lane))[1] = 0ull;
    }
    if (P.self_clean && clean_words && lane < 32) clean_words[lane] = 0u;
    if (P.laps && lane == 0) { asm volatile("s_waitcnt vmcnt(0)" ::: "memory"); laps[25] = wall_clock64(); }
  };
  if (status) { leave(0u); return; }
  if (d2_lost) {
    if (tid == 0) { if (!lost_counted) atomicAdd(&S->anomalies, 1u); arena[td.arena_off + td.lmf] = '\0'; }
    asm volatile("s_waitcnt vmcnt(0)" ::: "memory");
    leave(0u);
    return;
  }
  const uint32_t gi = td.gi;
  if ((go.dflags & G2S_DEVA_TRACED) && !(gi & (GI_BAD | GI_SKIPPED | GI_MEM | GI_HOST)) && (gi & GI_PHASE_D)) {
    asm volatile("s_waitcnt vmcnt(0)" ::: "memory");
    leave((go.top_level >> 16) - (go.top_level & 0xFFFFu));
    return;
  }
  const bool spec = (go.dflags & G2S_DEVA_SPEC) != 0u && W.spec_text != nullptr && !(gi & (GI_BAD | GI_SKIPPED | GI_MEM | GI_HOST)) && (gi & GI_PHASE_D);
  const int spec_stop = (int)(go.top_level & 0xFFFFu), spec_len = (int)(go.top_level >> 16);
  const unsigned long long spec_chain = spec ? ((unsigned long long)uni(outs[i].stat[6]) | ((unsigned long long)uni(outs[i].stat[7]) << 32)) : 0ull;
  struct { uint16_t lmf; } dg = {td.lmf};
  const uint64_t abs_off = td.arena_off;
  char* buf = arena + abs_off;
  const int k = P.k;
  uint32_t rw[24];
#pragma unroll
  for (int q = 0; q < 24; q++) rw[q] = 0u;
  int left_fuz = 0;
  bool spec_rec = false;
  uint32_t g_all = 0, g_sent = 0;
  auto finish = [&](uint32_t fill_len) {
    if (!w0) return;
    const uint64_t fo = abs_off + (uint64_t)((int)dg.lmf - left_fuz);
    rw[1] = (uint32_t)left_fuz;
    rw[4] = (uint32_t)fo; rw[5] = (uint32_t)(fo >> 32);
    rw[6] = fill_len;
    uint32_t mine = 0u;
#pragma unroll
    for (int q = 0; q < 24; q++) mine = lane == q ? rw[q] : mine;
    if (spec_rec) {
      const uint32_t was = lane < 28 ? W.spec_res[(size_t)i * 28u + (uint32_t)lane] : 0u;
      if (__ballot(lane < 28 && was != mine) == 0ull) return;
    }
    if (lane < 28) ((uint32_t*)&results[i])[lane] = mine;
  };
  if (gi & (GI_BAD | GI_SKIPPED | GI_MEM)) {
    rw[3] = (gi & GI_BAD) ? G2S_GAP_BAD_FLANK : (gi & GI_SKIPPED) ? G2S_GAP_SKIPPED : G2S_GAP_MEM_EXCEEDED;
    if (gi & GI_MEM) rw[0] = (uint32_t)-1;
    if (tid == 0) buf[dg.lmf] = '\0';
    finish(0u);
    leave(0u);
    return;
  }
  const bool phase_d = (gi & GI_PHASE_D) != 0;
  rw[20] = (uint32_t)go.c_count;
  rw[21] = (uint32_t)go.n_len;
  rw[22] = (uint32_t)go.len[0];
  rw[23] = (uint32_t)go.len[1];
  rw[3] = (go.flags & (G2S_DEV_Q7_A | G2S_DEV_Q7_B | G2S_DEV_Q7_D)) ? G2S_GAP_Q7 : 0u;
  rw[0] = (uint32_t)((phase_d && !P.skip_confident && P.all_paths) ? go.count_s : go.c_count);
  const bool by_runs = phase_d && !P.skip_confident && (go.dflags & G2S_DEVA_RUNS) != 0u && W.d2out != nullptr;
  uint32_t n_runs = 0;
  const uint32_t* runs = nullptr;
  if (phase_d && !P.skip_confident) {
    rw[8] = go.sub_vertices; rw[10] = go.sub_edges;
    rw[16] = go.sub_vertices; rw[18] = go.sub_edges;
    if (by_runs) {
      const uint4 o0 = ((const uint4*)&W.d2out[i])[0], o1 = ((const uint4*)&W.d2out[i])[1];
      runs = W.d2runs + 2ull * uni(o0.x);
      n_runs = uni(o0.y);
      rw[8] = uni(o0.z); rw[10] = uni(o0.w); rw[12] = uni(o1.x); rw[14] = uni(o1.y); rw[16] = uni(o1.z); rw[18] = uni(o1.w);
    }
  }
  if (!phase_d) {
    if (tid == 0) buf[dg.lmf] = '\0';
    finish(0u);
    leave(0u);
    return;
  }
  if (gi & GI_HOST) {
    const uint32_t it = CHAIN ? h_it : uni(W.host_slot[i]);
    if (it != 0xFFFFFFFFu) {
      const g2s::D3HostItem* hp = &W.hitems[CHAIN ? 0u : it];
      const uint64_t so = CHAIN ? h_so : (uint64_t)uni((uint32_t)hp->seg_off) | ((uint64_t)uni((uint32_t)(hp->seg_off >> 32)) << 32);
      const uint64_t ro = CHAIN ? h_ro : (uint64_t)uni((uint32_t)hp->rnd_off) | ((uint64_t)uni((uint32_t)(hp->rnd_off >> 32)) << 32);
      const uint32_t ns = CHAIN ? h_ns : uni(hp->n_segs), want = CHAIN ? h_want : uni(hp->draws);
      const GapOut& g = outs[i];
      if ((uint32_t)tid < sizeof(GapOut) / 4u) ((uint32_t*)&side.outs[it])[tid] = ((const uint32_t*)&g)[tid];
      const uint4* src = (const uint4*)(sub + td.sub_at);
      uint4* dst = (uint4*)(side.segs + so);
      for (uint32_t w = (uint32_t)tid; w < 2u * ns; w += (uint32_t)NT) dst[w] = src[w];
      for (uint32_t w = (uint32_t)tid; w < (want + 8u) / 8u; w += (uint32_t)NT) {
        uint32_t pk8 = 0u;
#pragma unroll
        for (uint32_t x = 0; x < 8u; x++) {
          const uint32_t at = 8u * w + x;
          if (at <= want) pk8 |= ((rnd[td.off + at] >> 1) % 12u) << (4u * x);
        }
        side.rnd[ro + w] = pk8;
      }
      __threadfence_system();
      if constexpr (NW > 1) __syncthreads();
      if (tid == 0) {
        __hip_atomic_store(&side.items[it].pad, 1u, __ATOMIC_RELEASE, __HIP_MEMORY_SCOPE_SYSTEM);
      }
    }
    leave(0u);
    return;
  }
  const bool big = (uint32_t)td.nsegs > P.seg_cap && by_runs && W.hops != nullptr;
  const uint32_t nsegs = big ? (uint32_t)td.nsegs : min((uint32_t)td.nsegs, P.seg_cap);
  const SegW* gsegs = (const SegW*)(sub + td.sub_at);
  uint64_t* ghop = big ? W.hops + td.sub_at / 2u : nullptr;
  uint32_t* cmap = lds + (size_t)P.seg_cap * 8u;
  uint32_t* lwin = cmap + P.map_cap;
  const uint32_t nwin = min(td.want, P.map_cap);
  for (uint32_t x = (uint32_t)tid; x < nwin; x += (uint32_t)NT) lwin[x] = (uint64_t)td.off + x < capacity ? rnd[td.off + x] : 0u;
  if (!big) {
    const uint4* src = (const uint4*)gsegs;
    uint4* dst = (uint4*)segs;
    for (uint32_t w = (uint32_t)tid; w < 2u * nsegs; w += (uint32_t)NT) dst[w] = src[w];
  }
  __syncthreads();
  if (P.laps) tk1 = wall_clock64();
  const bool sink_safe = (go.dflags & G2S_DEVA_SINK_SAFE) != 0;
  auto outside_safe = [&](uint32_t x) -> bool {
    for (uint32_t q = 0; q < nsegs; q++) {
      const uint32_t onode = segs[q].node, ots = segs[q].ts_tt;
      const int ts = (ots & 0x7FFFu) == 0x7FFFu ? -1 : (int)(ots & 0x7FFFu);
      const uint32_t oidx = onode >> 1;
      const int tq = (onode & 1u) ? (int)oidx - (int)x : (int)x - (int)oidx;
      if (tq >= 0 && tq <= ts) return tq <= (int)segs[q].pad ? (ots & 0x8000u) != 0 : (ots & 0x80000000u) != 0;
    }
    return sink_safe;
  };
  const uint32_t* lruns = nullptr;
  auto run_verdict = [&](uint32_t x, uint32_t* rlo, uint32_t* rhi) -> bool {
    const uint32_t* rr = lruns ? lruns : runs;
    uint32_t lo = 0, hi = n_runs;
    while (lo < hi) { const uint32_t mid = (lo + hi) >> 1; if (rr[2u * mid] <= x) lo = mid + 1u; else hi = mid; }
    if (lo > 0u) {
      const uint32_t f = rr[2u * (lo - 1u)], l = rr[2u * (lo - 1u) + 1u];
      if (x <= (l & 0x7FFFFFFFu)) { *rlo = f; *rhi = l & 0x7FFFFFFFu; return (l >> 31) != 0u; }
    }
    *rlo = x; *rhi = x;
    return sink_safe;
  };
  const uint32_t off = td.off;
  const uint64_t avail = min((uint64_t)nwin, capacity > off ? capacity - off : 0ull);
  const int want = (int)td.want;
  const int n_len = go.n_len, len0 = go.len[0], len1 = go.len[1];
  int draws = 1;
  auto value = [&](uint32_t x) -> uint32_t { return uni(lwin[x]); };
  const int pick = (n_len > 1 && avail > 0) ? (int)((value(0) >> 1) & 1u) : 0;
  int d2 = pick ? len1 : len0;
  const int len = d2;
  bool bad = false, ended = false;
  if ((uint32_t)len + 1u > P.map_cap || (!big && (uint32_t)td.nsegs > P.seg_cap) || td.want > P.map_cap) bad = true;
  uint2* hop = (uint2*)(lwin + P.map_cap);
  uint2* pk = hop + P.seg_cap;
  for (uint32_t q = (uint32_t)tid; q < nsegs && !big; q += (uint32_t)NT) {
    const uint32_t dl = segs[q].depth_len, p01 = segs[q].par01, p23 = segs[q].par23, fl = segs[q].flags;
    const int d0 = (int)(dl & 0xFFFFu);
    const int nb = seg_nparents(p01, p23);
    const int64_t at = 1 + (int64_t)len - d0;
    uint32_t w;
    if (nb == 0 || (nb > 1 && !(fl & G2S_SEG_ORDERED)) || at < 1 || (uint64_t)at >= avail) w = 0x80000000u;
    else {
      const uint32_t rv = nb > 1 ? lwin[at] >> 1 : 0u;
      w = seg_parent(p01, p23, nb == 1 ? 0 : pick_parent(rv, nb));
      if (w >= nsegs) w = 0x80000000u;
    }
    pk[q] = make_uint2(dl, w | ((fl & G2S_SUB_SOURCE) ? 0x40000000u : 0u));
  }
  wg_sync();
  int nh = 0;
  {
    const uint32_t sg = (go.start_seg >> (16 * pick)) & 0xFFFFu;
    int si = sg == 0xFFFFu ? -1 : (int)sg;
    const int t0 = (int)((go.start_t >> (16 * pick)) & 0xFFFFu);
    if (si < 0 || si >= (int)nsegs || avail < 1) bad = true;
    uint32_t last = 0x80000000u;
    const int hop_cap = (int)(big ? nsegs : min(nsegs, P.seg_cap));
    unsigned long long chain_hash = 14695981039346656037ull;
    const uint32_t L = nsegs > 1u ? 32u - (uint32_t)__builtin_clz(nsegs - 1u) : 0u;
    const bool jump = !big && L * nsegs <= 2u * P.map_cap;
    uint16_t* J = (uint16_t*)cmap;
    if (jump) {
      for (uint32_t q = (uint32_t)tid; q < nsegs && L > 0u; q += (uint32_t)NT) { const uint32_t y = pk[q].y; J[q] = (uint16_t)((y & 0xC0000000u) ? q : (y & 0xFFFFu)); }
      wg_sync();
      for (uint32_t j = 1; j < L; j++) {
        for (uint32_t q = (uint32_t)tid; q < nsegs; q += (uint32_t)NT) J[j * nsegs + q] = J[(j - 1u) * nsegs + J[(j - 1u) * nsegs + q]];
        wg_sync();
      }
    }
    if (!bad && jump) {
      bool ended_chain = false;
      for (uint32_t h0 = 0; h0 < (uint32_t)hop_cap; h0 += 64u) {
        const uint32_t h = h0 + (uint32_t)lane;
        const bool in = h < (uint32_t)hop_cap;
        uint32_t sq = (uint32_t)si;
        for (uint32_t j = 0; j < L; j++) { const uint32_t to = J[j * nsegs + sq]; sq = ((h >> j) & 1u) ? to : sq; }
        const uint32_t y = pk[sq].y;
        const uint32_t on = (uint32_t)__popcll(__ballot(in && !(y & 0xC0000000u)));
        if (in && (uint32_t)lane <= on) hop[h].y = sq;
        if (on < min(64u, (uint32_t)hop_cap - h0)) {
          nh = (int)(h0 + on) + 1;
          last = uni((uint32_t)__shfl((int)y, (int)on));
          ended_chain = true;
          break;
        }
      }
      if (!ended_chain) { nh = hop_cap; bad = true; }
      if (!bad && spec) {
        asm volatile("s_waitcnt lgkmcnt(0)" ::: "memory");
        __builtin_amdgcn_wave_barrier();
        for (int h = 0; h < nh; h++) chain_hash = (chain_hash ^ (unsigned long long)uni(hop[h].y)) * 1099511628211ull;
      }
    }
    if (!bad && !big && !jump) {
      if (spec) {
        for (;;) {
          if (nh >= hop_cap) { bad = true; break; }
          last = uni(pk[si].y);
          chain_hash = (chain_hash ^ (unsigned long long)(uint32_t)si) * 1099511628211ull;
          if (lane == 0) hop[nh].y = (uint32_t)si;
          nh++;
          if (last & 0xC0000000u) break;
          si = (int)(last & 0xFFFFu);
        }
      } else {
        uint32_t hv = 0u;
        for (;;) {
          if (nh >= hop_cap) { bad = true; break; }
          last = uni(pk[si].y);
          hv = lane == (nh & 63) ? (uint32_t)si : hv;
          nh++;
          if ((nh & 63) == 0) hop[nh - 64 + lane].y = hv;
          if (last & 0xC0000000u) break;
          si = (int)(last & 0xFFFFu);
        }
        if (!bad && (nh & 63) != 0 && lane < (nh & 63)) hop[(nh & ~63) + lane].y = hv;
      }
    }
    if (!bad && !big) {
      if (P.laps) hops = (unsigned long long)nh;
      if (!bad && spec && pick == 0 && len == spec_len && (last & 0x40000000u) && chain_hash == spec_chain) {
        gsp_all = 1u;
        leave((uint32_t)(spec_len - spec_stop));
        return;
      }
    }
    if (!bad && big) {
      for (;;) {
        if (nh >= hop_cap) { bad = true; break; }
        if (P.laps) hops++;
        const uint32_t dl = uni(gsegs[si].depth_len), p01 = uni(gsegs[si].par01), p23 = uni(gsegs[si].par23), fl = uni(gsegs[si].flags);
        const int d0 = (int)(dl & 0xFFFFu);
        const int nb = seg_nparents(p01, p23);
        const int64_t at = 1 + (int64_t)len - d0;
        uint32_t w;
        if (nb == 0 || (nb > 1 && !(fl & G2S_SEG_ORDERED)) || at < 1 || (uint64_t)at >= avail) w = 0x80000000u;
        else {
          const uint32_t rv = nb > 1 ? value((uint32_t)at) >> 1 : 0u;
          w = seg_parent(p01, p23, nb == 1 ? 0 : pick_parent(rv, nb));
          if (w >= nsegs) w = 0x80000000u;
        }
        last = w | ((fl & G2S_SUB_SOURCE) ? 0x40000000u : 0u);
        if (lane == 0) ghop[nh] = (uint64_t)(uint32_t)si << 32;
        nh++;
        if (last & 0xC0000000u) break;
        si = (int)(last & 0xFFFFu);
      }
      __threadfence_block();
// ... 143 lines not shown
}

}

namespace g2s {

void rand_tables_host(uint32_t* hi, uint32_t* mid, uint32_t* lane) {
  auto mulmod = [](const uint32_t* a, const uint32_t* b, uint32_t* out) {
    uint32_t c[61];
    for (int i = 0; i < 61; i++) c[i] = 0;
    for (int i = 0; i < 31; i++) {
      if (!a[i]) continue;
      for (int j = 0; j < 31; j++) c[i + j] += a[i] * b[j];
    }
    for (int d = 60; d >= 31; d--) { c[d - 3] += c[d]; c[d - 31] += c[d]; }
    for (int i = 0; i < 31; i++) out[i] = c[i];
  };
  auto power = [&](uint64_t N, uint32_t* q) {
    uint32_t r[31] = {0}, b[31] = {0}, t[31];
    r[0] = 1; b[1] = 1;
    for (; N; N >>= 1) {
      if (N & 1) { mulmod(r, b, t); for (int i = 0; i < 31; i++) r[i] = t[i]; }
      mulmod(b, b, t);
      for (int i = 0; i < 31; i++) b[i] = t[i];
    }
    for (int i = 0; i < 31; i++) q[i] = r[i];
  };
  auto series = [&](uint64_t step, int count, uint32_t* out) {
    uint32_t s[31];
    power(step, s);
    for (int i = 0; i < 31; i++) out[i] = i == 0 ? 1u : 0u;
    for (int a = 1; a < count; a++) mulmod(out + (size_t)(a - 1) * 31, s, out + (size_t)a * 31);
  };
  series(1ull << 20, 128, hi);
  series(4096, 256, mid);
  series(64, 64, lane);
}

size_t d3_work_bytes(uint32_t n) {
  const size_t per = (((size_t)n + 64) * 4 + 63) & ~(size_t)63;
  return 14 * per + 64 * 128 + (size_t)G2S_D3_TABLE_BUDGET * 2 + (size_t)(G2S_D3_TABLE_BUDGET / 4u) * 4 + 4096 +
         ((size_t)n + 64) * (sizeof(D3Var) + sizeof(D3Trace) + sizeof(D3HostItem)) + ((size_t)n + G2S_D3_TABLE_BUDGET / 256u + 64) * 4;
}

void d3_work_carve(void* p, uint32_t n, D3Work* w) {
  char* c = (char*)p;
  const size_t per = (((size_t)n + 64) * 4 + 63) & ~(size_t)63;
  w->sum = (D3Summary*)c; c += 1024;
  w->fill_bytes = (unsigned long long*)c; c += 64 * 128;
  w->ginfo = (uint32_t*)c; c += per;
  w->dmin = (uint32_t*)c; c += per;
  w->dspread = (uint32_t*)c; c += per;
  w->base = (uint32_t*)c; c += per;
  w->vrank = (uint32_t*)c; c += per;
  w->var_gap = (uint32_t*)c; c += per;
  w->var_R = (uint32_t*)c; c += per;
  w->var_toff = (uint32_t*)c; c += per;
  w->var_tile = (uint32_t*)c; c += per;
  w->blk_toff = (uint32_t*)c; c += per;
  w->blk_in = (uint32_t*)c; c += per;
  w->dvar = (uint32_t*)c; c += per;
  w->skip = (int32_t*)c; c += per;
  w->host_slot = (uint32_t*)c; c += per;
  w->vdesc = (D3Var*)c; c += ((size_t)n + 64) * sizeof(D3Var);
  w->tdesc = (D3Trace*)c; c += ((size_t)n + 64) * sizeof(D3Trace);
  w->hitems = (D3HostItem*)c; c += ((size_t)n + 64) * sizeof(D3HostItem);
  w->tile_var = (uint32_t*)c; c += ((size_t)n + G2S_D3_TABLE_BUDGET / 256u + 64) * 4;
  w->btab = (uint32_t*)c; c += (size_t)(G2S_D3_TABLE_BUDGET / 4u) * 4;
  w->tab = (uint16_t*)c;
}

hipError_t launch_rand_fill(hipStream_t st, uint32_t* rnd_all, const RandTables& rt, const D3Summary* sum_dev, uint64_t capacity,
                            uint64_t first_value) {
  const uint64_t first_block = first_value / G2S_RAND_BLOCK;
  const uint64_t all = (capacity + G2S_RAND_BLOCK - 1) / G2S_RAND_BLOCK;
  const uint32_t rblocks = (uint32_t)std::min<uint64_t>(all > first_block ? all - first_block : 1, 4096);
  hipLaunchKernelGGL(g2s_rand_fill, dim3(std::max(1u, rblocks)), dim3(64), 0, st, rnd_all, rt, sum_dev, capacity, first_block);
  return hipGetLastError();
}

static void launch_scan(hipStream_t st, const D3Params& P, const D3Work& W, const GapOut* outs) {
  static std::mutex mu;
  static std::set<int> done;
  int dev = 0;
  (void)hipGetDevice(&dev);
  {
    std::lock_guard<std::mutex> lk(mu);
    if (done.insert(dev).second)
      (void)hipFuncSetAttribute((const void*)g2s_d3_scan, hipFuncAttributeMaxDynamicSharedMemorySize, (int)(12u * D3_SCAN_LDS_GAPS));
  }
  const size_t lds = P.n <= D3_SCAN_LDS_GAPS ? 12u * (size_t)P.n : 0u;
  hipLaunchKernelGGL(g2s_d3_scan, dim3(1), dim3(1024), lds, st, P, W, outs);
}

static hipError_t launch_tables(hipStream_t st, const D3Params& P, const D3Work& W, const SubRec* sub, uint32_t* rnd_all, uint64_t rnd_capacity) {
  const size_t win = ((size_t)P.map_cap + D3_TILE) * 4;
  const bool waves = P.n <= D3_FRONT_GAPS;
  const hipError_t e = hipFuncSetAttribute(waves ? (const void*)g2s_d3_tables_waves : (const void*)g2s_d3_tables, hipFuncAttributeMaxDynamicSharedMemorySize, (int)win);
  if (e != hipSuccess) return e;
  if (waves) hipLaunchKernelGGL(g2s_d3_tables_waves, dim3(D3_WAVE_GRID), dim3(256), win, st, P, W, sub, rnd_all + 31, rnd_capacity);
  else hipLaunchKernelGGL(g2s_d3_tables, dim3(std::min(8192u, std::max(128u, P.n / 2u))), dim3(256), win, st, P, W, sub, rnd_all + 31, rnd_capacity);
  return hipGetLastError();
}

hipError_t test_d3_tables(const uint32_t* segs, uint32_t nsegs, int32_t n_len, int32_t len0, int32_t len1, uint32_t start_seg,
                          const uint32_t* rnd, uint64_t rnd_cap, uint32_t base, uint32_t R, uint32_t dmin, uint32_t dspread,
                          uint16_t* entries, uint8_t* bad, uint32_t* anomalies) {
  const uint32_t tiles = (R + D3_TILE) / D3_TILE;
  const size_t n_tile_var = 8192u + tiles, n_rnd = 31u + (size_t)rnd_cap + 64u;
  std::vector<SegW> hs(std::max(nsegs, 1u));
  for (uint32_t q = 0; q < nsegs; q++) {
    SegW w = {};
    w.depth_len = segs[4u * q]; w.par01 = segs[4u * q + 1u]; w.par23 = segs[4u * q + 2u]; w.flags = segs[4u * q + 3u];
    hs[q] = w;
  }
  std::vector<uint32_t> hr(n_rnd, 0u);
  for (uint64_t x = 0; x < rnd_cap; x++) hr[31u + x] = rnd[x];
  D3Var vd = {};
  vd.gap = 0; vd.R = R; vd.toff = 0; vd.tile0 = 0; vd.base = base; vd.dmin = dmin; vd.dspread = dspread; vd.ns = nsegs;
  auto start_t = [&](int pick) -> uint32_t {
    const uint32_t sg = (start_seg >> (16 * pick)) & 0xFFFFu;
    const int t = sg < nsegs ? (pick ? len1 : len0) - (int)(segs[4u * sg] & 0xFFFFu) : 0;
    return t >= 0 && t <= 0xFFFF ? (uint32_t)t : 0u;
  };
  vd.sub_at = 0; vd.start_seg = start_seg; vd.start_t = start_t(0) | (start_t(1) << 16); vd.len0 = len0; vd.len1 = len1; vd.n_len = n_len;
  D3Summary sum = {};
  sum.n_var = 1; sum.tiles = tiles; sum.table_entries = (uint64_t)R + 1u;
  void *d_sum = nullptr, *d_vd = nullptr, *d_tv = nullptr, *d_seg = nullptr, *d_rnd = nullptr, *d_tab = nullptr, *d_bad = nullptr;
  auto release = [&]() { for (void* p : {d_sum, d_vd, d_tv, d_seg, d_rnd, d_tab, d_bad}) if (p) (void)hipFree(p); };
  hipError_t e = hipSuccess;
  auto ok = [&](hipError_t x) { if (e == hipSuccess) e = x; return e == hipSuccess; };
  if (ok(hipMalloc(&d_sum, 1024)) && ok(hipMalloc(&d_vd, 4 * sizeof(D3Var))) && ok(hipMalloc(&d_tv, n_tile_var * 4)) &&
      ok(hipMalloc(&d_seg, hs.size() * sizeof(SegW))) && ok(hipMalloc(&d_rnd, n_rnd * 4)) && ok(hipMalloc(&d_tab, ((size_t)R + 1u) * 2)) &&
      ok(hipMalloc(&d_bad, (size_t)R + 1u)) && ok(hipMemset(d_sum, 0, 1024)) && ok(hipMemset(d_vd, 0, 4 * sizeof(D3Var))) &&
      ok(hipMemset(d_tv, 0, n_tile_var * 4)) && ok(hipMemset(d_tab, 0xFF, ((size_t)R + 1u) * 2)) && ok(hipMemset(d_bad, 0xFF, (size_t)R + 1u)) &&
      ok(hipMemcpy(d_sum, &sum, sizeof sum, hipMemcpyHostToDevice)) && ok(hipMemcpy(d_vd, &vd, sizeof vd, hipMemcpyHostToDevice)) &&
      ok(hipMemcpy(d_seg, hs.data(), hs.size() * sizeof(SegW), hipMemcpyHostToDevice)) &&
      ok(hipMemcpy(d_rnd, hr.data(), n_rnd * 4, hipMemcpyHostToDevice))) {
    D3Params P;
    memset(&P, 0, sizeof P);
    P.n = 1; P.group_size = 1;
    P.map_cap = ((uint32_t)std::max(std::max(len0, len1), 0) + 2u + 3u) & ~3u;
    D3Work W;
    W.sum = (D3Summary*)d_sum; W.vdesc = (D3Var*)d_vd; W.tile_var = (uint32_t*)d_tv; W.tab = (uint16_t*)d_tab; W.tab_bad = (uint8_t*)d_bad;
    if (ok(launch_tables(nullptr, P, W, (const SubRec*)d_seg, (uint32_t*)d_rnd, rnd_cap)) && ok(hipDeviceSynchronize()) &&
        ok(hipMemcpy(entries, d_tab, ((size_t)R + 1u) * 2, hipMemcpyDeviceToHost)) && ok(hipMemcpy(bad, d_bad, (size_t)R + 1u, hipMemcpyDeviceToHost)) &&
        ok(hipMemcpy(&sum, d_sum, sizeof sum, hipMemcpyDeviceToHost)))
      *anomalies = sum.anomalies;
  }
  release();
  return e;
}

hipError_t launch_rand_window(hipStream_t st, uint32_t* rnd_all, const uint32_t* link) {
  hipLaunchKernelGGL(g2s_rand_window, dim3(1), dim3(64), 0, st, rnd_all, link);
  return hipGetLastError();
}

hipError_t launch_d3_sharded_classes(hipStream_t st, const D3Params& P, const D3Work& W, const GapOut* outs, const D3Gap* dgaps,
                                     bool summary_is_clean) {
  if (P.n == 0) return hipSuccess;
  hipError_t e = summary_is_clean ? hipSuccess : hipMemsetAsync(W.sum, 0, 1024 + 64 * 128, st);
  if (e != hipSuccess) return e;
  hipLaunchKernelGGL(g2s_d3_classify, dim3((P.n + 255u) / 256u), dim3(256), 0, st, P, W, outs, dgaps);
  launch_scan(st, P, W, outs);
  return hipGetLastError();
}
hipError_t launch_d3_sharded_tables(hipStream_t st, const D3Params& P, const D3Work& W, const GapOut* outs, const SubRec* sub,
                                    uint32_t* rnd_all, uint64_t rnd_capacity, uint32_t* group_fn) {
  if (P.n == 0) return hipSuccess;
  launch_scan(st, P, W, outs);
  const hipError_t e = launch_tables(st, P, W, sub, rnd_all, rnd_capacity);
  if (e != hipSuccess) return e;
  hipLaunchKernelGGL(g2s_d3_blocks, dim3(256), dim3(256), 0, st, W);
  hipLaunchKernelGGL(g2s_d3_groupfn, dim3(std::min(256u, (P.R0 + 256u) / 256u)), dim3(256), 0, st, W, P.R0, group_fn);
  return hipGetLastError();
}
hipError_t launch_d3_sharded_trace(hipStream_t st, const D3Params& P, const D3Work& W, const GapOut* outs, const SubRec* sub,
                                   const char* lastch_up, const char* lastch_dn, uint32_t* rnd_all, uint64_t rnd_capacity,
                                   void* results, char* arena, const D3Side& side, void* summary_host, hipEvent_t ev_d2) {
  if (P.n == 0) return hipSuccess;
  hipLaunchKernelGGL(g2s_d3_chain, dim3(1), dim3(1024), 0, st, W, rnd_all, P.base0, P.d_in);
  if (ev_d2) { const hipError_t e2 = hipStreamWaitEvent(st, ev_d2, 0); if (e2 != hipSuccess) return e2; }
  hipLaunchKernelGGL(g2s_d3_handoff, dim3((P.n + 63u) / 64u), dim3(64), 0, st, P, W, outs, sub, rnd_all + 31, rnd_capacity, side);
  const size_t lds = (size_t)P.seg_cap * (sizeof(SegRec) + 16) + (size_t)P.map_cap * 8 + 16;
  hipError_t e = hipFuncSetAttribute((const void*)g2s_d3_trace<1>, hipFuncAttributeMaxDynamicSharedMemorySize, (int)lds);
  if (e != hipSuccess) return e;
  hipLaunchKernelGGL(g2s_d3_trace<1>, dim3(P.n), dim3(64), lds, st, P, W, const_cast<GapOut*>(outs), sub, lastch_up, lastch_dn, rnd_all + 31, rnd_capacity,
                     (g2s_result*)results, arena, (uint32_t*)summary_host, side, (uint32_t*)nullptr, 0u);
  return hipGetLastError();
}

static std::atomic<uint64_t> chain_launches{0};
uint64_t d3_chain_launches() { return chain_launches.load(std::memory_order_relaxed); }

hipError_t launch_d3(hipStream_t st, const D3Params& P, const D3Work& W, const GapDev* gaps, const GapOut* outs,
                     const D3Gap* dgaps, const SubRec* sub, const char* lastch_up, const char* lastch_dn,
                     const RandTables& rt, uint32_t* rnd_all, uint64_t rnd_capacity, void* results, char* arena,
                     const D3Side& side, void* summary_host, bool summary_is_clean, uint32_t* clean_words, hipEvent_t ev_chain,
                     hipEvent_t ev_d2, hipEvent_t ev_stop) {
  if (P.n == 0) return hipSuccess;
  (void)gaps;
  (void)rt;
  static_assert(sizeof(D3Summary) <= 1024, "summary slot");
  hipError_t e = summary_is_clean ? hipSuccess : hipMemsetAsync(W.sum, 0, 1024 + 64 * 128, st);
  if (e != hipSuccess) return e;
  const bool short_list = P.n <= D3_FRONT_GAPS;
  if (P.restart) {
    if (ev_d2) { e = hipStreamWaitEvent(st, ev_d2, 0); if (e != hipSuccess) return e; }
    hipLaunchKernelGGL(g2s_d3_restart, dim3((P.n + 255u) / 256u), dim3(256), 0, st, P, W, outs, dgaps, sub, rnd_all + 31, rnd_capacity, side);
  } else if (short_list) hipLaunchKernelGGL(g2s_d3_front, dim3(1), dim3(1024), 0, st, P, W, outs, dgaps);
  else {
    hipLaunchKernelGGL(g2s_d3_classify, dim3((P.n + 255u) / 256u), dim3(256), 0, st, P, W, outs, dgaps);
    launch_scan(st, P, W, outs);
  }
  if (!P.restart) { e = launch_tables(st, P, W, sub, rnd_all, rnd_capacity); if (e != hipSuccess) return e; }
  if (ev_d2 && short_list && !P.restart) { e = hipStreamWaitEvent(st, ev_d2, 0); if (e != hipSuccess) return e; }
  const char* waves_s = GENV("G2S_TRACE_WAVES");
  const int waves_env = waves_s ? atoi(waves_s) : 0;
  const bool four = waves_env ? waves_env == 4 : P.n <= 768u;
  const size_t lds = (size_t)P.seg_cap * (sizeof(SegRec) + 16) + (size_t)P.map_cap * 8 + 16;
  bool chain_in_trace = false;
  uint32_t chain_room = 0;
  static_assert(D3_CHAIN_GAPS <= 768u, "g2s_d3_trace<4, true> is the four-wave kernel");
  if (!P.restart && four && P.n <= D3_CHAIN_GAPS && ev_chain == nullptr && P.group_size >= P.n && !P.base0 && !P.R0 && !P.d_in) {
    const char* back_s = GENV("G2S_D3_BACK");
    chain_in_trace = !(back_s && atoi(back_s) != 0);
    const char* room_s = GENV("G2S_TEST_CHAIN_ROOM");
    chain_room = (uint32_t)std::min<size_t>(lds / 2u, 0x7FFFFFFFu);
    if (room_s) chain_room = std::min(chain_room, (uint32_t)std::max(atoi(room_s), 0));
  }
  if (P.restart) (void)ev_chain;
  else if (chain_in_trace) (void)ev_chain;
  else if (short_list) {
    hipLaunchKernelGGL(g2s_d3_back, dim3(1), dim3(1024), 0, st, P, W, outs, sub, rnd_all, rnd_capacity, side);
    if (ev_chain) { e = hipEventRecord(ev_chain, st); if (e != hipSuccess) return e; }
  } else {
    hipLaunchKernelGGL(g2s_d3_blocks, dim3(256), dim3(256), 0, st, W);
    hipLaunchKernelGGL(g2s_d3_chain, dim3(1), dim3(1024), 0, st, W, rnd_all, 0u, 0u);
    if (ev_chain) { e = hipEventRecord(ev_chain, st); if (e != hipSuccess) return e; }
    if (ev_d2) { e = hipStreamWaitEvent(st, ev_d2, 0); if (e != hipSuccess) return e; }
    hipLaunchKernelGGL(g2s_d3_handoff, dim3((P.n + 63u) / 64u), dim3(64), 0, st, P, W, outs, sub, rnd_all + 31, rnd_capacity, side);
  }
  e = hipFuncSetAttribute(chain_in_trace ? (const void*)g2s_d3_trace<4, true> : four ? (const void*)g2s_d3_trace<4> : (const void*)g2s_d3_trace<1>,
                          hipFuncAttributeMaxDynamicSharedMemorySize, (int)lds);
  if (e != hipSuccess) return e;
  if (chain_in_trace) {
    chain_launches.fetch_add(1, std::memory_order_relaxed);
    if (ev_stop != nullptr)
      hipExtLaunchKernelGGL((g2s_d3_trace<4, true>), dim3(P.n), dim3(256), (uint32_t)lds, st, nullptr, ev_stop, 0u, P, W, const_cast<GapOut*>(outs), sub, lastch_up, lastch_dn,
                            rnd_all + 31, rnd_capacity, (g2s_result*)results, arena, (uint32_t*)summary_host, side, clean_words, chain_room);
    else
      hipLaunchKernelGGL((g2s_d3_trace<4, true>), dim3(P.n), dim3(256), lds, st, P, W, const_cast<GapOut*>(outs), sub, lastch_up, lastch_dn, rnd_all + 31, rnd_capacity,
                         (g2s_result*)results, arena, (uint32_t*)summary_host, side, clean_words, chain_room);
    return hipGetLastError();
  }
  if (ev_stop != nullptr) {
    if (four)
      hipExtLaunchKernelGGL(g2s_d3_trace<4>, dim3(P.n), dim3(256), (uint32_t)lds, st, nullptr, ev_stop, 0u, P, W, const_cast<GapOut*>(outs), sub, lastch_up, lastch_dn,
                            rnd_all + 31, rnd_capacity, (g2s_result*)results, arena, (uint32_t*)summary_host, side, clean_words, 0u);
    else
      hipExtLaunchKernelGGL(g2s_d3_trace<1>, dim3(P.n), dim3(64), (uint32_t)lds, st, nullptr, ev_stop, 0u, P, W, const_cast<GapOut*>(outs), sub, lastch_up, lastch_dn,
                            rnd_all + 31, rnd_capacity, (g2s_result*)results, arena, (uint32_t*)summary_host, side, clean_words, 0u);
    return hipGetLastError();
  }
  if (four)
    hipLaunchKernelGGL(g2s_d3_trace<4>, dim3(P.n), dim3(256), lds, st, P, W, const_cast<GapOut*>(outs), sub, lastch_up, lastch_dn, rnd_all + 31, rnd_capacity,
                       (g2s_result*)results, arena, (uint32_t*)summary_host, side, clean_words, 0u);
  else
    hipLaunchKernelGGL(g2s_d3_trace<1>, dim3(P.n), dim3(64), lds, st, P, W, const_cast<GapOut*>(outs), sub, lastch_up, lastch_dn, rnd_all + 31, rnd_capacity,
                       (g2s_result*)results, arena, (uint32_t*)summary_host, side, clean_words, 0u);
  return hipGetLastError();
}

}
```

### gap2seq_amd/csrc/g2s_api.hip

```cpp
#include <hip/hip_runtime.h>
#include <cstdarg>
#include <sys/prctl.h>
#include <pthread.h>
#include <sched.h>
#include <time.h>

#include <algorithm>
#include <atomic>
#include <chrono>
#include <cstdio>
#include <cstdlib>
#include <condition_variable>
#include <cstring>
#include <functional>
#include <mutex>
#include <string>
#include <thread>
#include <vector>

#include "../../include/g2s.h"
#include "../../include/g2s_test.h"
#include "envcache.hpp"
#include "d2_device.h"
#include "d3_device.h"
// ... 3396 lines not shown
  const FillParams fp = fill_params_of(s);
  const bool timed = dpp->timed, res_direct = dpp->res_direct, arena_direct = dpp->arena_direct;
  const bool self_clean = dpp->self_clean;
  const D3Side& side_h = dpp->side_h;
  const D3Work& W = dpp->W;
  D3Summary* hsum = dpp->hsum;
  hipEvent_t d3_begin = dpp->d3_begin;
  g2s_result* results = dpp->results;
  char* arena = dpp->arena;
  const auto t_enter = dpp->t_enter, t_launched = dpp->t_launched;
  if (hipSetDevice(s->device) != hipSuccess) return fail(G2S_ERR_NO_DEVICE, "cannot select device");
  hipStream_t st = s->stream;
  unsigned long long handed = ~0ull;
  if (dpp->discard) {
    HIP_TRY_S(hipStreamSynchronize(st));
    if (!self_clean) HIP_TRY_S(hipMemsetAsync(W.sum, 0, 1024 + 64 * 128, st));
    s->d_d3.clean = 1024 + 64 * 128;
    s->self_cleaned = self_clean && hsum->status == 0;
    s->side_dirty = SIZE_MAX;
    *ms_d3_out = 0;
    *fell_back = true;
    return G2S_OK;
  }
  const SegEarly eh = s->early_host;
  std::atomic<uint32_t> early_next(0);
  std::atomic<int> early_done(0);
  std::function<void(size_t)> early_worker;
  bool early_posted = false;
  const bool early_inline = eh.cap_items && L.groups.size() == 1 && L.dmax < 2500 && n < 3072;
  std::vector<std::pair<uint32_t, uint32_t>>& inline_done = s->early_inline_done;
  inline_done.clear();
  uint32_t inline_next = 0;
  auto early_take_ready = [&]() {
    while (inline_next < eh.cap_items && __atomic_load_n(&eh.items[8 * (size_t)inline_next + 4], __ATOMIC_ACQUIRE) != 0u) {
      const uint32_t idx = inline_next++;
      const uint32_t gap = eh.items[8 * (size_t)idx], ns = eh.items[8 * (size_t)idx + 1], so = eh.items[8 * (size_t)idx + 2];
      if (ns == 0u || gap >= n) continue;
      if (s->early_prep.size() <= idx) { s->early_prep.resize((size_t)idx + 8); s->early_scratch.resize((size_t)idx + 8); }
      SubPrep& pp = s->early_prep[idx];
      pp.reset();
      std::vector<uint64_t>& sc = s->early_scratch[idx];
      if (sc.size() < 3 * (size_t)ns + 1) sc.resize(3 * (size_t)ns + 1);
      SubView v;
      v.out = &eh.outs[idx]; v.segs = eh.segs + so; v.n_segs = ns;
      if (seg_analyze(fp, L.groups[0]->jobs[gap], v, &pp, sc.data())) inline_done.emplace_back(gap, idx);
    }
  };
  if (!early_inline && eh.cap_items && L.groups.size() == 1 && s->pool->size() > 0 &&
      __atomic_load_n(side_h.count, __ATOMIC_ACQUIRE) == ~0ull) {
    s->early_of_gap.assign(n, -1);
    if (s->early_prep.size() < eh.cap_items) { s->early_prep.resize(eh.cap_items); s->early_scratch.resize(eh.cap_items); }
    early_worker = [&](size_t) {
      for (;;) {
        uint32_t idx = early_next.load(std::memory_order_acquire);
        const bool ready = idx < eh.cap_items && __atomic_load_n(&eh.items[8 * (size_t)idx + 4], __ATOMIC_ACQUIRE) != 0u;
        if (ready) {
          if (!early_next.compare_exchange_weak(idx, idx + 1u)) continue;
          const uint32_t gap = eh.items[8 * (size_t)idx], ns = eh.items[8 * (size_t)idx + 1], so = eh.items[8 * (size_t)idx + 2];
          if (ns == 0u || gap >= n) continue;
          SubPrep& pp = s->early_prep[idx];
          pp.reset();
          std::vector<uint64_t>& sc = s->early_scratch[idx];
          if (sc.size() < 3 * (size_t)ns + 1) sc.resize(3 * (size_t)ns + 1);
          SubView v;
          v.out = &eh.outs[idx]; v.segs = eh.segs + so; v.n_segs = ns;
          if (seg_analyze(fp, L.groups[0]->jobs[gap], v, &pp, sc.data())) s->early_of_gap[gap] = (int32_t)idx;
          continue;
        }
        if (early_done.load(std::memory_order_acquire)) {
          idx = early_next.load(std::memory_order_acquire);
          if (idx < eh.cap_items && __atomic_load_n(&eh.items[8 * (size_t)idx + 4], __ATOMIC_ACQUIRE) != 0u) continue;
          return;
        }
        cpu_relax();
      }
    };
    s->pool->post((size_t)std::min(s->pool->size(), 15), early_worker);
    early_posted = true;
  }
  for (unsigned spins = 0;; spins++) {
    handed = __atomic_load_n(side_h.count, __ATOMIC_ACQUIRE);
    if (handed != ~0ull) break;
    if (early_inline) early_take_ready();
    if ((spins & 1023u) == 1023u && hipStreamQuery(st) != hipErrorNotReady) {
      handed = __atomic_load_n(side_h.count, __ATOMIC_ACQUIRE);
      if (handed == ~0ull) handed = 1ull << 63;
      break;
    }
    cpu_relax();
  }
  if (early_inline && handed != ~0ull && !(handed >> 63) && (handed & 0x7FFFFFFFFFFFFFFFull)) early_take_ready();
  if (early_posted) { early_done.store(1, std::memory_order_release); s->pool->finish(); }
  const auto t_handed = std::chrono::steady_clock::now();
  std::atomic<int> host_bad(0);
  const size_t ni = (size_t)(handed & 0x7FFFFFFFFFFFFFFFull);
  g2s_result* rs_host = res_direct ? results : (g2s_result*)s->h_res.p;
  uint64_t host_fill_bytes = 0;
  if (ni && !(handed >> 63)) {
    char* text = arena_direct ? arena : (char*)s->h_text.p;
    auto one = [&](size_t x) {
      for (unsigned spins = 0; __atomic_load_n(&side_h.items[x].pad, __ATOMIC_ACQUIRE) == 0u; spins++) {
        if ((spins & 4095u) == 4095u && hipStreamQuery(st) != hipErrorNotReady &&
            __atomic_load_n(&side_h.items[x].pad, __ATOMIC_ACQUIRE) == 0u) { host_bad.fetch_add(1); return; }
        cpu_relax();
      }
      const D3HostItem& h = side_h.items[x];
      const size_t q = h.gap / L.group_size, loc = h.gap % L.group_size;
      const g2s_batch* gb = L.groups[q];
      const auto t_one = std::chrono::steady_clock::now();
      struct Lap { const std::chrono::steady_clock::time_point t0, th; const D3HostItem& h; size_t x; bool on;
                   ~Lap() { if (on && h.n_segs >= 2000) fprintf(stderr, "[g2s] host-finished item %zu (gap %u): %u segments, %u draws: picked up %.3f ms after the hand-over, %.3f ms\n", x, h.gap, h.n_segs, h.draws,
                                                              ms_between(th, t0), ms_since(t0)); } }
          lap{t_one, t_handed, h, x, dbg_analysis_stats};
      int32_t ei = early_posted ? s->early_of_gap[h.gap] : -1;
      if (early_inline) for (const auto& pr : inline_done) if (pr.first == h.gap) { ei = (int32_t)pr.second; break; }
      const bool ok = ei >= 0 && eh.items[8 * (size_t)ei + 1] == h.n_segs
          ? finish_gap_on_host(g, fp, gb->jobs[loc], eh.outs[ei], eh.segs + eh.items[8 * (size_t)ei + 2], h.n_segs, side_h.rnd + h.rnd_off,
                               h.draws, (uint64_t)(L.group_arena[q] + gb->arena_off[loc]), text, &rs_host[h.gap], &s->early_prep[(size_t)ei], true)
          : finish_gap_on_host(g, fp, gb->jobs[loc], side_h.outs[x], side_h.segs + h.seg_off, h.n_segs, side_h.rnd + h.rnd_off, h.draws,
                               (uint64_t)(L.group_arena[q] + gb->arena_off[loc]), text, &rs_host[h.gap], nullptr, true);
      if (!ok) host_bad.fetch_add(1);
    };
    std::vector<uint32_t>& lpt = s->host_order;
    lpt.resize(ni);
    for (size_t x = 0; x < ni; x++) lpt[x] = (uint32_t)x;
    if (ni > 2) {
      std::sort(lpt.begin(), lpt.end(), [&](uint32_t a, uint32_t b) {
        const uint32_t na = side_h.items[a].n_segs, nb = side_h.items[b].n_segs;
        return na != nb ? na > nb : a < b;
      });
      s->pool->run(ni, [&](size_t x) { one((size_t)lpt[x]); });
    } else for (size_t x = 0; x < ni; x++) one(x);
    for (size_t x = 0; x < ni; x++) host_fill_bytes += (uint64_t)rs_host[side_h.items[x].gap].fill_len;
    if (const char* path = GENV("G2S_HOST_ITEMS_DUMP")) {
      if (FILE* f = fopen(path, "wb")) {
        for (size_t x = 0; x < ni; x++) {
          const D3HostItem& h = side_h.items[x];
          const GapOut& go = side_h.outs[x];
          const int32_t hd[8] = {(int32_t)h.gap, (int32_t)h.n_segs, go.c_count, go.n_len, go.len[0], go.len[1], go.reached_j, go.final_d};
          fwrite(hd, sizeof hd, 1, f);
          fwrite(side_h.segs + h.seg_off, sizeof(SegRec), h.n_segs, f);
        }
        fclose(f);
      }
    }
  }
  const auto t_finished = std::chrono::steady_clock::now();
  HIP_TRY_S(hipStreamSynchronize(st));
  const auto t_synced = std::chrono::steady_clock::now();
  float ms_d3 = 0;
  if (timed) HIP_TRY_S(hipEventElapsedTime(&ms_d3, d3_begin, s->ev[3]));
  *ms_d3_out = ms_d3;
  if (GENV("G2S_DEBUG")) {
    unsigned long long lp[34];
    HIP_TRY_S(hipMemcpy(lp, (char*)W.sum + 512, sizeof lp, hipMemcpyDeviceToHost));
    auto us = [&](int a, int b) { return lp[a] && lp[b] ? ((double)lp[b] - (double)lp[a]) / 100.0 : -1.0; };
    fprintf(stderr, "[g2s] phase D3 laps (us): front classify %.1f scan %.1f | to tables %.1f: status %.1f records %.1f closure %.1f walks %.1f | to back %.1f: tables into LDS %.1f chain %.1f hand-off %.1f fence %.1f | to trace %.1f, longest wave: to closure %.1f walk %.1f bases %.1f all %.1f, first entry to last end %.1f\n",
            us(0, 1), us(1, 2), us(2, 3), us(3, 4), us(4, 5), us(5, 6), us(6, 7), us(7, 8), us(8, 9), us(9, 10), us(10, 11), us(11, 12), us(12, 13),
            lp[14] / 100.0, lp[15] / 100.0, lp[16] / 100.0, (double)(lp[17] >> 24) / 100.0, us(13, 18));
    fprintf(stderr, "[g2s] the longest wave of the trace kernel: gap %llu%s\n", lp[17] & 0x7FFFFFull, (lp[17] >> 23) & 1ull ? " (handed to the host)" : "");
    fprintf(stderr, "[g2s] scan (us): sums %.1f, base + layout pass %.1f, table offsets + records %.1f\n", us(20, 21), us(21, 22), us(22, 23));
    fprintf(stderr, "[g2s] the last wave of the trace kernel: the summary's copy to the host begins %.1f us after the kernel's first entry and takes %.1f us\n", us(13, 24), us(24, 25));
    if (GENV("G2S_DEBUG_GAP") && lp[26])
      fprintf(stderr, "[g2s] gap %s in the trace kernel (us): enters %.1f behind the kernel's first wave | to closure in LDS %.1f | chain %.1f | bases classified %.1f | text %.1f | record %.1f\n",
              GENV("G2S_DEBUG_GAP"), us(13, 26), us(26, 27), us(27, 28), us(28, 29), us(29, 30), us(30, 31));
    fprintf(stderr, "[g2s] g2s_d3_tables: the last workgroup with a tile ends %.1f us after the first workgroup's entry, the last workgroup of all %.1f us\n", us(3, 32), us(3, 33));
    fprintf(stderr, "[g2s] the wave with the longest walk: %.1f us, %llu segments entered in %.1f us\n", (double)(lp[19] >> 32) / 100.0, (lp[19] >> 16) & 0xFFFF, (double)(lp[19] & 0xFFFF) / 100.0);
  }
  if (!self_clean) HIP_TRY_S(hipMemsetAsync(W.sum, 0, 1024 + 64 * 128, st));
  s->d_d3.clean = 1024 + 64 * 128;
  s->self_cleaned = self_clean && hsum->status == 0;
  uint64_t spec_groups = 0, spec_sent = 0;
  for (int q = 0; q < 64; q++) {
    hsum->fill_bytes += ((const unsigned long long*)((const char*)hsum + 1024))[q * 16] & ((1ull << 40) - 1);
    const unsigned long long gw = ((const unsigned long long*)((const char*)hsum + 1024))[q * 16 + 1];
    spec_groups += gw & 0xFFFFFFFFull; spec_sent += gw >> 32;
  }
  hsum->fill_bytes += host_fill_bytes;
  bool test_fallback = false;
  if (const char* tf = GENV("G2S_RESIDENT_TEST_FALLBACK")) {
    static std::mutex mu;
    static std::string seen;
    static int waits = 0;
    std::lock_guard<std::mutex> lk(mu);
    if (seen != tf) { seen = tf; waits = 0; }
    const int mine = waits++;
    test_fallback = strncmp(tf, "rel:", 4) != 0 || mine == atoi(tf + 4);
  }
  if (hsum->status != 0 || hsum->anomalies != 0 || test_fallback || host_bad.load() || hsum->host_items != ni) {
    if (GENV("G2S_DEBUG"))
      fprintf(stderr, "[g2s] resident mode: list of %zu gaps goes to the host path (status %#x, %u gaps not finished on the device, %u anomalies, %llu table entries, %d host-finished gaps disagree)\n",
              n, hsum->status, hsum->unhandled, hsum->anomalies, (unsigned long long)hsum->table_entries, host_bad.load());
    const bool defect = hsum->anomalies != 0 || host_bad.load();
    if (hsum->unhandled) s->segw_quiet = 0;
    if (!test_fallback && defect && ++s->resident_strikes >= 3) s->resident_off = true;
    *fell_back = true;
    return G2S_OK;
  }
  s->resident_strikes = 0;
  s->segw_quiet = hsum->big_gaps ? 0 : std::min(s->segw_quiet + 1, 1 << 20);
  s->side_dirty = ni;
  if (!res_direct || !arena_direct) {
    const g2s_result* rs = res_direct ? results : (const g2s_result*)s->h_res.p;
    const char* text = (const char*)s->h_text.p;
    const size_t per_task = 256, ntasks = (n + per_task - 1) / per_task;
    auto copy_range = [&](size_t t) {
      const size_t lo = t * per_task, hi = std::min(n, lo + per_task);
      if (!res_direct) memcpy(results + lo, rs + lo, (hi - lo) * sizeof(g2s_result));
      if (!arena_direct)
        for (size_t i = lo; i < hi; i++) memcpy(arena + rs[i].fill_off, text + rs[i].fill_off, (size_t)rs[i].fill_len + 1);
    };
    if (ntasks > 2) s->pool->run(ntasks, copy_range);
    else for (size_t t = 0; t < ntasks; t++) copy_range(t);
  }
  if (!dpp->sharded && !L.restart) s->rcache.jump((size_t)hsum->draws_total, hsum->rand_state);
  g2s_timing& tm = *tm_out;
  tm.xA += hsum->xA; tm.sA += hsum->sA; tm.xB += hsum->xB; tm.sB += hsum->sB; tm.xD += hsum->xD; tm.sD += hsum->sD;
  tm.seg_segments += hsum->segs;
  tm.seg_tier_gaps += hsum->seg_gaps - hsum->big_gaps;
  tm.segx_tier_gaps += hsum->big_gaps;
  tm.fill_bytes += hsum->fill_bytes;
  tm.ms_d3 += ms_d3;
  tm.resident_launches++;
  tm.draw_dependent_gaps += hsum->n_var;
  tm.host_finished_gaps += (uint32_t)hsum->host_items;
  tm.traced_in_fill_gaps += hsum->traced_gaps;
  tm.guessed_in_fill_gaps += hsum->spec_gaps;
  tm.guessed_groups += (uint32_t)spec_groups; tm.guessed_groups_resent += (uint32_t)spec_sent;
  tm.d3_table_entries += hsum->table_entries;
  const auto t_end = std::chrono::steady_clock::now();
  s->lap_d3_queued = t_launched; s->lap_handed = t_handed; s->lap_finished = t_finished; s->lap_synced = t_synced; s->lap_end = t_end;
  s->laps_valid = true;
  if (GENV("G2S_DEBUG"))
    fprintf(stderr, "[g2s] resident mode, phase D3 of %zu gaps: set-up + launches %.3f ms, wait for the hand-over %.3f ms, %zu gaps finished by the host in %.3f ms, wait for the trace kernel %.3f ms, results %.3f ms (kernels %.3f ms); %u draw-dependent gaps, %llu table entries, %llu draws; results %s, text %s\n",
            n, ms_between(t_enter, t_launched), ms_between(t_launched, t_handed), ni, ms_between(t_handed, t_finished),
            ms_between(t_finished, t_synced), ms_between(t_synced, t_end), ms_d3, hsum->n_var,
            (unsigned long long)hsum->table_entries, (unsigned long long)hsum->draws_total, res_direct ? "direct" : "staged",
            arena_direct ? "direct" : "staged");
  return G2S_OK;
}

static int resident_d3(g2s_session* s, const ResidentList& L, bool timed, bool rand_launched, g2s_result* results, char* arena,
                       g2s_timing* tm_out, double* ms_d3_out, bool* fell_back) {
  *fell_back = false;
  const int rc = resident_d3_launch(s, L, timed, rand_launched, results, arena, false);
  if (rc != G2S_OK) return rc;
  return resident_d3_wait(s, tm_out, ms_d3_out, fell_back);
}

static ResidentList resident_list_of(g2s_batch* b, size_t arena_base, size_t arena_total) {
  g2s_session* s = b->s;
  const size_t n = b->jobs.size();
  ResidentList L;
  L.groups.push_back(b);
  L.n = n; L.group_size = std::max<size_t>(n, 1);
  L.group_arena.push_back(arena_base);
  L.arena_bytes = arena_total;
  L.outs_dev = (const GapOut*)s->d_outs.p;
  L.sub_dev = (const SubRec*)s->d_sub.p;
  L.sub_region = 0;
  L.pin = &s->h_d3;
  L.rnd_cap = b->rnd_cap; L.dmax = b->dmax; L.has_skip = b->has_skip;
  L.gaps_dev = (const GapDev*)s->d_gaps.p;
  return L;
}
static void shift_arena_offsets(g2s_session* s, size_t n, size_t base) {
  D3Gap* dq = (D3Gap*)s->h_d3.p;
  for (size_t i = 0; i < n; i++) dq[i].arena_off += (uint64_t)base;
}
static void resident_abandon(g2s_session* s, size_t n) {
  (void)hipSetDevice(s->device);
  (void)hipStreamSynchronize(s->stream);
  (void)hipStreamSynchronize(s->stream2);
  delete (D3Pending*)s->d3_pending;
  s->d3_pending = nullptr;
  s->d_d3.clean = 0;
  if (n) (void)resident_reset_fill(s, n);
}

enum { SHARD_NOT_RESIDENT = 1,
       SHARD_NOT_D3 = 2,
       SHARD_BEYOND_DEVICE = 3
};
static int shard_fill(g2s_batch* b, g2s_result* results, char* arena, size_t arena_total, ResidentLaunch* rl, uint64_t totals[2],
                      const char* what) {
  g2s_session* s = b->s;
  int rc = resident_launch_fill(b, rl);
  if (rc != G2S_OK) return rc == 1 ? (int)SHARD_NOT_RESIDENT : rc;
  const ResidentList L = resident_list_of(b, b->arena_base, arena_total);
  if (b->arena_base) shift_arena_offsets(s, L.n, b->arena_base);
  rc = resident_d3_launch(s, L, rl->timed, false, results, arena, true, true);
  if (rc == 1) return SHARD_NOT_D3;
  if (rc == G2S_OK && hipStreamSynchronize(s->stream) != hipSuccess) rc = fail(G2S_ERR_HIP, what);
  if (rc != G2S_OK) return rc;
  const D3Summary* hs = ((D3Pending*)s->d3_pending)->hsum;
  if (hs->status != 0) return SHARD_BEYOND_DEVICE;
  totals[0] = hs->draws_min; totals[1] = hs->draws_spread;
  return G2S_OK;
}
static int shard_tables(g2s_session* s, uint32_t base0, uint32_t R0, const uint32_t* win, const uint32_t** group_fn, const char* what) {
  int rc = resident_d3_sharded_tables(s, base0, R0, win);
  if (rc == G2S_OK && hipStreamSynchronize(s->stream) != hipSuccess) rc = fail(G2S_ERR_HIP, what);
  if (rc != G2S_OK) return rc;
  const D3Pending* dp = (const D3Pending*)s->d3_pending;
  if (dp->hsum->status != 0) return SHARD_BEYOND_DEVICE;
  *group_fn = dp->group_fn;
  return G2S_OK;
}
static int shard_trace(g2s_batch* b, uint32_t d_in, double* ms_d3, bool* fell_back) {
  g2s_session* s = b->s;
  *fell_back = false;
  int rc = resident_d3_sharded_trace(s, d_in);
  if (rc == G2S_OK) rc = resident_d3_wait(s, &b->timing, ms_d3, fell_back);
  if (rc == G2S_OK) rc = resident_reset_fill(s, b->jobs.size());
  return rc;
// ... 1080 lines not shown
  if (ustart_out) memcpy(ustart_out, g.ustart.data(), (size_t)((g.n + 63) / 64) * 8);
  return G2S_OK;
}

extern "C" int64_t g2s_graph_validate(const g2s_graph* gr, char* msg, size_t msg_cap) {
  if (!gr || !gr->g) return -1;
  const Graph& g = *gr->g;
  std::string text;
  int64_t bad = 0;
  auto note = [&](const char* what, uint64_t i) {
    if (bad++ < 8) text += std::string(what) + " at k-mer " + std::to_string(i) + "; ";
  };
  auto only = [&](uint32_t v, uint32_t want) {
    int cnt = 0;
    bool hit = false;
    for (int nt = 0; nt < 4; nt++) {
      const uint32_t w = g.succ_of(v, nt);
      if (w == kInvalidNode) continue;
      cnt++;
      hit = hit || w == want;
    }
    return cnt == 1 && hit;
  };
  uint64_t starts = 0;
  for (uint64_t i = 0; i < g.n; i++) {
    const bool start = (g.ustart[i >> 6] >> (i & 63)) & 1;
    starts += start;
    if (i == 0) { if (!start) note("first k-mer is not a unitig start", i); continue; }
    if (start) continue;
    const uint32_t a = (uint32_t)(2 * (i - 1)), b = (uint32_t)(2 * i);
    if (!only(a, b)) note("internal edge is not the only successor (even orientation)", i);
    if (!only(b ^ 1u, a ^ 1u)) note("internal edge is not the only successor (odd orientation)", i);
  }
  if (starts != g.n_unitigs) note("bitmap population differs from the unitig count", starts);
  if (!g.set_lo.empty()) {
    if (g.set_lo.front() != 0 || g.set_lo.back() != g.n) note("set ranges do not cover the k-mers", g.n);
    for (size_t s = 0; s + 1 < g.set_lo.size(); s++) {
      if (g.set_lo[s] > g.set_lo[s + 1]) { note("set ranges not ascending", g.set_lo[s]); continue; }
      for (uint64_t i = g.set_lo[s]; i < g.set_lo[s + 1]; i++)
        for (uint32_t v = (uint32_t)(2 * i); v <= (uint32_t)(2 * i + 1); v++)
          for (int nt = 0; nt < 4; nt++) {
            const uint32_t w = g.succ_of(v, nt);
            if (w != kInvalidNode && ((w >> 1) < g.set_lo[s] || (w >> 1) >= g.set_lo[s + 1])) note("successor outside its set", i);
          }
    }
  }
  for (uint64_t v = 0; v < 2 * g.n; v++)
    for (int nt = 0; nt < 4; nt++) {
      const uint32_t w = g.succ_of((uint32_t)v, nt);
      if (w == kInvalidNode) continue;
      if (w >= 2 * g.n) { note("successor out of range", v >> 1); continue; }
      if (g.lastnt[w] != nt) note("last base of a successor differs from its slot", v >> 1);
    }
  if (msg && msg_cap) {
    const size_t c = std::min(text.size(), msg_cap - 1);
    memcpy(msg, text.data(), c);
    msg[c] = 0;
  }
  return bad;
}

extern "C" int g2s_test_worker_pool(int32_t threads, int32_t rounds, int32_t n) {
  if (threads < 1 || rounds < 0 || n < 0) return fail(G2S_ERR_ARG, "g2s_test_worker_pool: bad argument");
  WorkerPool pool(threads - 1);
  std::vector<std::atomic<int>> hits((size_t)n);
  for (int r = 0; r < rounds; r++) {
    for (auto& h : hits) h.store(0);
    std::atomic<long long> sum(0);
    const int nn = (r % 7 == 0) ? std::min(n, 3) : n;
    pool.run((size_t)nn, [&](size_t i) { hits[i].fetch_add(1); sum.fetch_add((long long)i + 1); });
    if (sum.load() != (long long)nn * (nn + 1) / 2) return fail(G2S_ERR_STATE, "worker pool: wrong task sum");
    for (int i = 0; i < nn; i++)
      if (hits[(size_t)i].load() != 1) return fail(G2S_ERR_STATE, "worker pool: task not run exactly once");
  }
  return G2S_OK;
}

extern "C" int g2s_test_group_queue(int32_t nworkers, uint64_t n, uint64_t group_size, int32_t* owner) {
  return g2s_test_group_queue_slow(nworkers, n, group_size, -1, 0, owner);
}
extern "C" int g2s_test_group_queue_slow(int32_t nworkers, uint64_t n, uint64_t group_size, int32_t slow_worker,
                                         uint32_t slow_us, int32_t* owner) {
  if (nworkers < 1 || !owner) return fail(G2S_ERR_ARG, "g2s_test_group_queue: bad argument");
  for (uint64_t i = 0; i < n; i++) owner[i] = -1;
  GroupQueue queue((size_t)n, (size_t)group_size);
  std::atomic<int> clash(0);
  auto worker = [&](int t) {
    size_t gi = 0, off = 0, cnt = 0;
    while (queue.pull(&gi, &off, &cnt)) {
      for (size_t i = off; i < off + cnt; i++) { if (owner[i] != -1) clash.fetch_add(1); owner[i] = t; }
      std::this_thread::sleep_for(std::chrono::microseconds(20 + (t == slow_worker ? slow_us : 0u)));
    }
  };
  std::vector<std::thread> th;
  for (int t = 1; t < nworkers; t++) th.emplace_back(worker, t);
  worker(0);
  for (auto& x : th) x.join();
  if (clash.load()) return fail(G2S_ERR_STATE, "group queue: a gap was handed out twice");
  for (uint64_t i = 0; i < n; i++) if (owner[i] < 0) return fail(G2S_ERR_STATE, "group queue: a gap was never handed out");
  return G2S_OK;
}

extern "C" int g2s_test_device_rand(int device, uint32_t seed, uint64_t skip, uint32_t n, int32_t* out) {
  if (!out) return fail(G2S_ERR_ARG, "g2s_test_device_rand: bad argument");
  int ndev = 0;
  if (hipGetDeviceCount(&ndev) != hipSuccess || device < 0 || device >= ndev) return fail(G2S_ERR_NO_DEVICE, "no such device");
  HIP_TRY(hipSetDevice(device));
  GlibcRandStream st;
  st.seed(seed);
  for (uint64_t left = skip; left;) {
    const size_t c = (size_t)std::min<uint64_t>(left, 1u << 20);
    st.ensure(c);
    st.consume(c);
    left -= c;
  }
  std::vector<uint32_t> tables((128 + 256 + 64) * 31);
  rand_tables_host(tables.data(), tables.data() + 128 * 31, tables.data() + (128 + 256) * 31);
  const uint64_t cap = ((uint64_t)n + 2 * G2S_RAND_BLOCK) & ~(uint64_t)(G2S_RAND_BLOCK - 1);
  uint32_t *d_tab = nullptr, *d_rnd = nullptr;
  D3Summary* d_sum = nullptr;
  HIP_TRY(hipMalloc((void**)&d_tab, tables.size() * 4));
  HIP_TRY(hipMalloc((void**)&d_rnd, (31 + cap + 64) * 4));
  HIP_TRY(hipMalloc((void**)&d_sum, sizeof(D3Summary)));
  D3Summary sum;
  memset(&sum, 0, sizeof sum);
  sum.draws_min = n;
  HIP_TRY(hipMemcpy(d_tab, tables.data(), tables.size() * 4, hipMemcpyHostToDevice));
  HIP_TRY(hipMemcpy(d_sum, &sum, sizeof sum, hipMemcpyHostToDevice));
  HIP_TRY(hipMemcpy(d_rnd, st.window(G2S_RAND_WINDOW), G2S_RAND_WINDOW * 4, hipMemcpyHostToDevice));
  RandTables rt;
  rt.hi = d_tab; rt.mid = d_tab + 128 * 31; rt.lane = d_tab + (128 + 256) * 31;
  HIP_TRY(launch_rand_fill(nullptr, d_rnd, rt, d_sum, cap));
  HIP_TRY(hipDeviceSynchronize());
  std::vector<uint32_t> h(n);
  HIP_TRY(hipMemcpy(h.data(), d_rnd + 31, (size_t)n * 4, hipMemcpyDeviceToHost));
  for (uint32_t i = 0; i < n; i++) out[i] = (int32_t)(h[i] >> 1);
  (void)hipFree(d_tab); (void)hipFree(d_rnd); (void)hipFree(d_sum);
  return G2S_OK;
}

extern "C" int g2s_test_d3_tables(int device, const uint32_t* segs, uint32_t n_segs, int32_t n_len, int32_t len0, int32_t len1,
                                  uint32_t start_seg, const uint32_t* rnd, uint64_t rnd_cap, uint32_t base, uint32_t R, uint32_t dmin,
                                  uint32_t dspread, uint16_t* entries, uint8_t* bad, uint32_t* anomalies) {
  if ((!segs && n_segs) || (!rnd && rnd_cap) || !entries || !bad || !anomalies || n_segs > 0xFFFFu || n_len < 1 || n_len > 2 ||
      (uint64_t)R + 1u > (uint64_t)G2S_D3_TABLE_BUDGET)
    return fail(G2S_ERR_ARG, "g2s_test_d3_tables: bad argument");
  int ndev = 0;
  if (hipGetDeviceCount(&ndev) != hipSuccess || device < 0 || device >= ndev) return fail(G2S_ERR_NO_DEVICE, "no such device");
  HIP_TRY(hipSetDevice(device));
  HIP_TRY(test_d3_tables(segs, n_segs, n_len, len0, len1, start_seg, rnd, rnd_cap, base, R, dmin, dspread, entries, bad, anomalies));
  return G2S_OK;
}

extern "C" uint64_t g2s_test_d3_chain_launches(void) { return d3_chain_launches(); }

extern "C" int g2s_test_rand_skip(uint32_t seed, uint64_t skip, uint32_t n, int32_t* out) {
  if (!out) return fail(G2S_ERR_ARG, "g2s_test_rand_skip: bad argument");
  GlibcRandStream st;
  st.seed(seed);
  st.skip(skip);
  st.ensure(n);
  for (uint32_t i = 0; i < n; i++) out[i] = st.value(i);
  return G2S_OK;
}
extern "C" int g2s_test_rand_stream(uint32_t seed, uint32_t skip, uint32_t n, int32_t* out) {
  if (!out) return fail(G2S_ERR_ARG, "g2s_test_rand_stream: bad argument");
  GlibcRandStream st;
  st.seed(seed);
  st.ensure(skip / 2 + 1);
  st.consume(skip / 2);
  st.ensure(skip - skip / 2 + n);
  st.consume(skip - skip / 2);
  for (uint32_t i = 0; i < n; i++) out[i] = st.value(i);
  return G2S_OK;
}
```

### gap2seq_amd/lib.py

```python
import ctypes as C
import os

G2S_OK = 0
G2S_ERR_IO = -2
G2S_ERR_NO_DEVICE = -3
G2S_ERR_STATE = -6
G2S_INVALID_NODE = 0xFFFFFFFF
G2S_MAX_PATHS = 2147483647 // 2 - 1
G2S_MAX_IN_FLIGHT = 3
G2S_GROUP_PER_SESSION = (1 << 64) - 1
G2S_GAP_SKIPPED = 0x1
G2S_GAP_Q7 = 0x2
G2S_GAP_MEM_EXCEEDED = 0x4
G2S_GAP_BACKTRACE_FAIL = 0x8
G2S_GAP_BAD_FLANK = 0x10
G2S_GAP_PHASE_D = 0x20


class G2SError(RuntimeError):
    def __init__(self, code, msg):
        super().__init__("g2s error %d: %s" % (code, msg))
        self.code = code


# ... 48 lines not shown
class g2s_filter_opts(C.Structure):
    _fields_ = [("mean_insert", C.c_int32), ("std_dev", C.c_int32), ("breakpoint", C.c_int32), ("gap_length", C.c_int32),
                ("flank_length", C.c_int32), ("unmapped_only", C.c_int32), ("threads", C.c_int32),
                ("scaffold", C.c_char_p)]


class g2s_filter_gap(C.Structure):
    _fields_ = [("scaffold", C.c_char_p), ("breakpoint", C.c_int32), ("gap_length", C.c_int32),
                ("flank_length", C.c_int32)]


class g2s_filter_stats(C.Structure):
    _fields_ = [("file_passes", C.c_uint32), ("on_device", C.c_uint32), ("ms_inflate", C.c_double),
                ("ms_join", C.c_double), ("ms_text", C.c_double)]


class g2s_read_pool(C.Structure):
    _fields_ = [("n_reads", C.c_uint64), ("bases", C.POINTER(C.c_char)), ("base_off", C.POINTER(C.c_uint64)),
                ("names", C.POINTER(C.c_char)), ("name_off", C.POINTER(C.c_uint64)), ("gap_begin", C.POINTER(C.c_uint64)),
                ("gap_read", C.POINTER(C.c_uint32)), ("n_unmapped", C.c_uint64), ("unmapped_read", C.POINTER(C.c_uint32))]


_VP = C.c_void_p
TEXT_FN = C.CFUNCTYPE(None, C.POINTER(C.c_char), C.c_size_t, C.c_void_p)
_SIGS = {
    "g2s_abi_version": (C.c_int, []),
    "g2s_fill_begin": (C.c_int, [_VP, C.POINTER(g2s_gap), C.c_size_t, C.POINTER(g2s_result), C.c_void_p, C.c_size_t]),
    "g2s_fill_end": (C.c_int, [_VP]),
    "g2s_fill_in_flight": (C.c_int, [_VP]),
    "g2s_share_begin": (C.c_int, [_VP, C.POINTER(g2s_gap), C.c_size_t, C.POINTER(g2s_result), C.c_void_p, C.c_size_t,
                                  C.POINTER(C.c_uint64)]),
    "g2s_share_tables": (C.c_int, [_VP, C.c_uint64, C.c_uint64, C.POINTER(C.POINTER(C.c_uint32))]),
    "g2s_share_trace": (C.c_int, [_VP, C.c_uint32]),
    "g2s_share_end": (C.c_int, [_VP, C.c_uint64]),
    "g2s_backtrace_text": (C.c_size_t, [C.POINTER(g2s_gap), C.POINTER(g2s_result), C.c_int, C.c_char_p, C.c_size_t]),
    "g2s_last_error": (C.c_char_p, []),
    "g2s_graph_build_files": (C.c_int, [C.c_char_p, C.c_int, C.c_int, C.c_int, C.POINTER(_VP)]),
    "g2s_graph_build_seqs": (C.c_int, [C.POINTER(C.c_char_p), C.POINTER(C.c_uint64), C.c_int, C.c_int, C.c_int,
                                       C.c_int, C.POINTER(_VP)]),
    "g2s_graph_build_sets": (C.c_int, [C.POINTER(C.c_char_p), C.POINTER(C.c_uint64), C.POINTER(C.c_uint32), C.c_int,
                                       C.c_uint32, C.c_int, C.c_int, C.c_int, C.POINTER(_VP)]),
    "g2s_graph_build_pool": (C.c_int, [C.POINTER(C.c_char_p), C.POINTER(C.c_uint64), C.c_uint64, C.POINTER(C.c_uint64),
                                       C.POINTER(C.c_uint32), C.POINTER(C.c_uint32), C.c_uint64, C.POINTER(C.c_uint8),
                                       C.c_uint32, C.c_int, C.c_int, C.c_int, C.POINTER(_VP)]),
    "g2s_graph_build_pool_reach": (C.c_int, [C.POINTER(C.c_char_p), C.POINTER(C.c_uint64), C.c_uint64, C.POINTER(C.c_uint64),
                                             C.POINTER(C.c_uint32), C.POINTER(C.c_uint32), C.c_uint64, C.POINTER(C.c_uint8),
                                             C.c_uint32, C.c_int, C.c_int, C.c_int, C.POINTER(g2s_gap), C.POINTER(C.c_int32),
                                             C.POINTER(_VP)]),
    "g2s_test_last_pool_reach": (C.c_int, [C.POINTER(C.c_uint64), C.POINTER(C.c_uint64), C.POINTER(C.c_int), C.POINTER(C.c_uint64),
                                           C.POINTER(C.c_uint32), C.POINTER(C.c_int)]),
    "g2s_test_last_pool_build": (C.c_int, [C.POINTER(C.c_uint64), C.POINTER(C.c_uint64), C.POINTER(C.c_uint64),
                                           C.POINTER(C.c_int)]),
    "g2s_test_last_solid_count": (C.c_int, [C.POINTER(C.c_uint64), C.POINTER(C.c_uint32), C.POINTER(C.c_uint32),
                                            C.POINTER(C.c_uint64), C.POINTER(C.c_uint64), C.POINTER(C.c_int)]),
    "g2s_test_plan_passes": (C.c_int, [C.POINTER(C.c_uint64), C.c_uint32, C.c_uint64, C.POINTER(C.c_uint32), C.c_uint32,
                                       C.POINTER(C.c_uint32), C.POINTER(C.c_uint32)]),
    "g2s_test_seg_back_record": (C.c_int, [_VP, C.c_int, C.c_uint32, C.POINTER(C.c_uint32)]),
    "g2s_graph_num_sets": (C.c_uint32, [_VP]),
    "g2s_graph_set_nodes": (C.c_int, [_VP, C.c_uint32, C.POINTER(C.c_uint64), C.POINTER(C.c_uint64)]),
    "g2s_graph_set_node": (C.c_uint32, [_VP, C.c_uint32, C.c_char_p]),
    "g2s_graph_save": (C.c_int, [_VP, C.c_char_p]),
    "g2s_graph_load": (C.c_int, [C.c_char_p, C.POINTER(_VP)]),
    "g2s_graph_free": (None, [_VP]),
    "g2s_graph_k": (C.c_int, [_VP]),
    "g2s_graph_solid": (C.c_int, [_VP]),
    "g2s_graph_num_kmers": (C.c_uint64, [_VP]),
    "g2s_graph_num_unitigs": (C.c_uint64, [_VP]),
    "g2s_graph_node": (C.c_uint32, [_VP, C.c_char_p]),
    "g2s_graph_successors": (C.c_int, [_VP, C.c_uint32, C.POINTER(C.c_uint32)]),
    "g2s_graph_predecessors": (C.c_int, [_VP, C.c_uint32, C.POINTER(C.c_uint32)]),
    "g2s_graph_node_string": (C.c_int, [_VP, C.c_uint32, C.c_char_p]),
    "g2s_graph_upload": (C.c_int, [_VP, C.c_int]),
    "g2s_graph_device_bytes": (C.c_uint64, [_VP, C.c_int]),
    "g2s_session_create": (C.c_int, [_VP, C.c_int, C.POINTER(g2s_params), C.POINTER(_VP)]),
    "g2s_session_destroy": (None, [_VP]),
    "g2s_session_srand": (C.c_int, [_VP, C.c_uint32]),
    "g2s_session_skip_draws": (C.c_int, [_VP, C.c_uint64]),
    "g2s_session_graph": (_VP, [_VP]),
    "g2s_session_get_params": (C.c_int, [_VP, C.POINTER(g2s_params)]),
    "g2s_batch_prepare": (C.c_int, [_VP, C.POINTER(g2s_gap), C.c_size_t, C.POINTER(_VP)]),
    "g2s_batch_run": (C.c_int, [_VP, C.POINTER(g2s_result), C.c_char_p, C.c_size_t]),
    "g2s_batch_arena_bytes": (C.c_size_t, [_VP]),
    "g2s_batch_timing": (C.c_int, [_VP, C.POINTER(g2s_timing)]),
    "g2s_batch_free": (None, [_VP]),
    "g2s_session_last_timing": (C.c_int, [_VP, C.POINTER(g2s_timing)]),
    "g2s_fill_batch": (C.c_int, [_VP, C.POINTER(g2s_gap), C.c_size_t, C.POINTER(g2s_result), C.c_char_p,
                                 C.c_size_t]),
    "g2s_team_fill": (C.c_int, [C.POINTER(_VP), C.c_int, C.POINTER(g2s_gap), C.c_size_t, C.c_size_t,
                                C.POINTER(g2s_result), C.c_char_p, C.c_size_t, C.POINTER(g2s_timing)]),
    "g2s_team_arena_bytes": (C.c_size_t, [_VP, C.POINTER(g2s_gap), C.c_size_t]),
    "g2s_fill_sets": (C.c_int, [_VP, C.POINTER(g2s_gap), C.POINTER(C.c_uint32), C.c_size_t, C.POINTER(g2s_result),
                                C.c_char_p, C.c_size_t]),
    "g2s_session_set_team": (C.c_int, [_VP, C.POINTER(_VP), C.c_int, C.c_size_t]),
    "g2s_execute_scaffolds_stream": (C.c_int, [_VP, C.POINTER(g2s_run_opts), C.c_char_p, C.c_char_p, C.c_char_p, C.c_size_t,
                                             TEXT_FN, TEXT_FN, _VP, C.POINTER(C.c_int32), C.POINTER(C.c_int32)]),
    "g2s_execute_scaffolds": (C.c_int, [_VP, C.POINTER(g2s_run_opts), C.c_char_p, C.c_char_p, C.c_char_p,
                                        C.POINTER(_VP), C.POINTER(_VP), C.POINTER(C.c_int32),
                                        C.POINTER(C.c_int32)]),
    "g2s_execute_single": (C.c_int, [_VP, C.POINTER(g2s_run_opts), C.c_char_p, C.c_char_p, C.c_char_p, C.c_char_p,
                                     C.c_int32, C.POINTER(_VP), C.POINTER(_VP)]),
    "g2s_free": (None, [_VP]),
    "g2s_host_alloc": (_VP, [C.c_size_t]),
    "g2s_host_free": (None, [_VP]),
    "g2s_cut_scaffolds": (C.c_int, [C.c_char_p, C.c_int, C.c_int, C.c_int, C.c_int, C.c_char_p, C.c_char_p, C.c_char_p,
                                    C.c_char_p, C.POINTER(_VP), C.POINTER(_VP), C.POINTER(_VP), C.POINTER(_VP)]),
    "g2s_merge_scaffolds": (C.c_int, [C.c_char_p, C.c_char_p, C.c_char_p, C.c_char_p, C.c_char_p, C.POINTER(_VP),
                                      C.POINTER(_VP)]),
    "g2s_filter_reads": (C.c_int, [C.c_char_p, C.POINTER(g2s_filter_opts), C.POINTER(_VP), C.POINTER(_VP),
                                   C.POINTER(_VP), C.POINTER(C.c_int64), C.POINTER(C.c_int64)]),
    "g2s_filter_reads_mem": (C.c_int, [C.c_char_p, C.c_size_t, C.POINTER(g2s_filter_opts), C.POINTER(_VP),
                                       C.POINTER(_VP), C.POINTER(_VP), C.POINTER(C.c_int64), C.POINTER(C.c_int64)]),
    "g2s_filter_reads_gaps": (C.c_int, [C.c_char_p, C.POINTER(g2s_filter_opts), C.POINTER(g2s_filter_gap), C.c_size_t,
                                        C.c_int, C.POINTER(_VP), C.POINTER(_VP), C.POINTER(_VP), C.POINTER(C.c_int64),
                                        C.POINTER(C.c_int64), C.POINTER(_VP), C.POINTER(C.c_int64),
                                        C.POINTER(g2s_filter_stats)]),
    "g2s_filter_reads_gaps_mem": (C.c_int, [C.c_char_p, C.c_size_t, C.POINTER(g2s_filter_opts), C.POINTER(g2s_filter_gap),
                                            C.c_size_t, C.c_int, C.POINTER(_VP), C.POINTER(_VP), C.POINTER(_VP),
                                            C.POINTER(C.c_int64), C.POINTER(C.c_int64), C.POINTER(_VP),
                                            C.POINTER(C.c_int64), C.POINTER(g2s_filter_stats)]),
    "g2s_filter_reads_gaps_pool": (C.c_int, [C.c_char_p, C.POINTER(g2s_filter_opts), C.POINTER(g2s_filter_gap), C.c_size_t,
                                             C.c_int, C.c_int, C.c_int, C.POINTER(C.POINTER(g2s_read_pool)),
                                             C.POINTER(C.c_int64), C.POINTER(g2s_filter_stats)]),
    "g2s_filter_reads_gaps_pool_mem": (C.c_int, [C.c_char_p, C.c_size_t, C.POINTER(g2s_filter_opts), C.POINTER(g2s_filter_gap),
                                                 C.c_size_t, C.c_int, C.c_int, C.c_int, C.POINTER(C.POINTER(g2s_read_pool)),
                                                 C.POINTER(C.c_int64), C.POINTER(g2s_filter_stats)]),
    "g2s_read_pool_free": (None, [C.POINTER(g2s_read_pool)]),
    "g2s_filter_reads_gaps_dpool": (C.c_int, [C.c_char_p, C.POINTER(g2s_filter_opts), C.POINTER(g2s_filter_gap), C.c_size_t,
                                              C.c_int, C.c_int, C.POINTER(_VP), C.POINTER(C.c_int64),
                                              C.POINTER(g2s_filter_stats)]),
    "g2s_filter_reads_gaps_dpool_mem": (C.c_int, [C.c_char_p, C.c_size_t, C.POINTER(g2s_filter_opts), C.POINTER(g2s_filter_gap),
                                                  C.c_size_t, C.c_int, C.c_int, C.POINTER(_VP), C.POINTER(C.c_int64),
                                                  C.POINTER(g2s_filter_stats)]),
    "g2s_device_pool_view": (C.POINTER(g2s_read_pool), [_VP]),
    "g2s_device_pool_device": (C.c_int, [_VP]),
    "g2s_device_pool_bytes": (C.c_uint64, [_VP]),
    "g2s_device_pool_read": (C.c_int, [_VP, C.c_uint64, C.c_char_p]),
    "g2s_device_pool_free": (None, [_VP]),
    "g2s_graph_build_dpool_reach": (C.c_int, [C.POINTER(_VP), C.c_uint32, C.POINTER(C.c_uint64), C.POINTER(C.c_uint32),
                                              C.POINTER(C.c_uint32), C.c_uint64, C.POINTER(C.c_uint8), C.c_uint32, C.c_int,
                                              C.c_int, C.c_int, C.POINTER(g2s_gap), C.POINTER(C.c_int32), C.POINTER(_VP)]),
    "g2s_test_last_dpool": (C.c_int, [C.POINTER(C.c_int), C.POINTER(C.c_uint64), C.POINTER(C.c_uint64),
                                      C.POINTER(C.c_uint64)]),
    "g2s_filter_last_error": (C.c_char_p, []),
    "g2s_device_count": (C.c_int, []),
    "g2s_synth_genome": (C.c_int, [C.c_uint64, C.c_uint32, C.c_uint64, C.POINTER(_VP)]),
    "g2s_synth_gaps": (C.c_int, [C.c_char_p, C.c_int, C.c_int, C.c_int, C.c_int, C.c_int, C.c_uint64,
                                 C.POINTER(_VP)]),
    "g2s_test_rand_skip": (C.c_int, [C.c_uint32, C.c_uint64, C.c_uint32, C.POINTER(C.c_int32)]),
    "g2s_test_rand_stream": (C.c_int, [C.c_uint32, C.c_uint32, C.c_uint32, C.POINTER(C.c_int32)]),
    "g2s_test_device_rand": (C.c_int, [C.c_int, C.c_uint32, C.c_uint64, C.c_uint32, C.POINTER(C.c_int32)]),
    "g2s_test_d3_tables": (C.c_int, [C.c_int, C.POINTER(C.c_uint32), C.c_uint32, C.c_int32, C.c_int32, C.c_int32, C.c_uint32,
                                     C.POINTER(C.c_uint32), C.c_uint64, C.c_uint32, C.c_uint32, C.c_uint32, C.c_uint32,
                                     C.POINTER(C.c_uint16), C.POINTER(C.c_uint8), C.POINTER(C.c_uint32)]),
    "g2s_test_d3_chain_launches": (C.c_uint64, []),
    "g2s_test_post_closure": (C.c_int, [_VP, C.POINTER(g2s_params), C.POINTER(g2s_gap), C.c_uint32,
                                        C.POINTER(C.c_uint32), C.c_uint32, C.POINTER(C.c_uint64), C.c_int32, C.c_int32,
                                        C.POINTER(C.c_int32), C.c_int32, C.c_int32, C.c_uint32, C.c_uint64,
                                        C.POINTER(g2s_result), C.c_char_p]),
    "g2s_test_graph_tables": (C.c_int, [_VP, C.POINTER(C.c_uint32), C.POINTER(C.c_uint64)]),
    "g2s_test_post_segments": (C.c_int, [_VP, C.POINTER(g2s_params), C.POINTER(g2s_gap), C.c_uint32,
                                         C.POINTER(C.c_uint32), C.c_int32, C.c_int32, C.POINTER(C.c_int32), C.c_int32,
                                         C.c_int32, C.c_uint32, C.c_uint64, C.POINTER(g2s_result), C.c_char_p,
                                         C.POINTER(C.c_int32)]),
    "g2s_test_seg_expand": (C.c_int, [_VP, C.POINTER(g2s_params), C.POINTER(g2s_gap), C.c_uint32, C.POINTER(C.c_uint32),
                                      C.c_int32, C.POINTER(C.c_int32), C.c_int32, C.c_uint32, C.POINTER(C.c_uint32),
                                      C.c_uint32, C.POINTER(C.c_uint64)]),
    "g2s_test_worker_pool": (C.c_int, [C.c_int32, C.c_int32, C.c_int32]),
    "g2s_test_group_queue": (C.c_int, [C.c_int32, C.c_uint64, C.c_uint64, C.POINTER(C.c_int32)]),
    "g2s_test_group_queue_slow": (C.c_int, [C.c_int32, C.c_uint64, C.c_uint64, C.c_int32, C.c_uint32, C.POINTER(C.c_int32)]),
    "g2s_test_filter_join": (C.c_int, [C.c_int, C.c_int32, C.c_uint64, C.POINTER(C.c_int32), C.POINTER(C.c_int32),
                                       C.POINTER(C.c_int64), C.POINTER(C.c_uint32), C.POINTER(C.c_uint64),
                                       C.POINTER(C.c_uint64), C.c_int64, C.c_uint64, C.c_uint64, C.POINTER(C.c_int64),
                                       C.c_uint64, C.POINTER(C.c_uint64), C.c_uint64, C.POINTER(C.c_uint64),
                                       C.POINTER(C.c_uint64), C.c_uint64, C.POINTER(C.c_uint64)]),
    "g2s_test_reads_text": (C.c_int, [C.c_char_p, C.c_size_t, C.c_int, C.c_size_t, C.POINTER(C.c_uint8), C.c_size_t,
                                      C.POINTER(C.c_size_t)]),
    "g2s_test_last_reads_load": (C.c_int, [C.POINTER(C.c_uint64), C.POINTER(C.c_uint64), C.POINTER(C.c_uint64),
                                           C.POINTER(C.c_uint64), C.POINTER(C.c_uint64), C.POINTER(C.c_int),
                                           C.POINTER(C.c_int), C.c_uint64, C.POINTER(C.c_uint64)]),
    "g2s_test_last_reads_bam": (C.c_int, [C.POINTER(C.c_uint64), C.POINTER(C.c_uint64), C.POINTER(C.c_uint64),
                                          C.POINTER(C.c_int), C.POINTER(C.c_int), C.POINTER(C.c_int)]),
    "g2s_test_last_reads_bam_stream": (C.c_int, [C.POINTER(C.c_uint64), C.POINTER(C.c_uint64), C.POINTER(C.c_uint64)]),
    "g2s_test_bgzf_inflate": (C.c_int, [C.c_char_p, C.c_size_t, C.c_int, C.POINTER(C.c_uint8), C.c_size_t,
                                        C.POINTER(C.c_size_t), C.POINTER(C.c_int64)]),
    "g2s_test_last_filter_inflate": (C.c_int, [C.POINTER(C.c_int), C.POINTER(C.c_uint64), C.POINTER(C.c_uint64),
                                               C.POINTER(C.c_uint64), C.POINTER(C.c_double), C.POINTER(C.c_double)]),
    "g2s_test_bam_rows": (C.c_int, [C.c_char_p, C.c_size_t, C.c_int, C.c_size_t, C.c_uint64, C.POINTER(C.c_int32),
                                    C.POINTER(C.c_int32), C.POINTER(C.c_int64), C.POINTER(C.c_uint32), C.POINTER(C.c_uint64),
                                    C.POINTER(C.c_uint64), C.POINTER(C.c_uint64), C.POINTER(C.c_int32), C.POINTER(C.c_int64)]),
    "g2s_test_bam_rows_kept": (C.c_int, [C.c_char_p, C.c_size_t, C.c_int, C.c_size_t, C.c_uint64, C.POINTER(C.c_int32),
                                         C.POINTER(C.c_int32), C.POINTER(C.c_int64), C.POINTER(C.c_uint32), C.POINTER(C.c_uint64),
                                         C.POINTER(C.c_uint64), C.POINTER(C.c_uint64), C.POINTER(C.c_int32), C.POINTER(C.c_int64)]),
    "g2s_test_name_hash": (C.c_int, [C.c_char_p, C.c_size_t, C.c_int, C.POINTER(C.c_uint64), C.POINTER(C.c_uint64)]),
    "g2s_test_last_filter_rows": (C.c_int, [C.POINTER(C.c_int), C.POINTER(C.c_uint64), C.POINTER(C.c_uint64),
                                            C.POINTER(C.c_uint64), C.POINTER(C.c_int)]),
    "g2s_filter_set_one_pass": (C.c_int, [C.c_int]),
    "g2s_reads_set_device_gzip": (C.c_int, [C.c_int]),
    "g2s_test_gzip_inflate": (C.c_int, [C.c_char_p, C.c_size_t, C.c_int, C.c_uint32, C.c_uint32, C.POINTER(C.c_uint8),
                                        C.c_size_t, C.POINTER(C.c_size_t), C.POINTER(C.c_int)]),
    "g2s_test_last_reads_gzip": (C.c_int, [C.POINTER(C.c_uint64), C.POINTER(C.c_uint64), C.POINTER(C.c_uint64),
                                           C.POINTER(C.c_uint64), C.POINTER(C.c_uint64), C.POINTER(C.c_uint64),
                                           C.POINTER(C.c_int), C.POINTER(C.c_uint64)]),
    "g2s_test_last_filter_text": (C.c_int, [C.POINTER(C.c_int), C.POINTER(C.c_int), C.POINTER(C.c_uint64), C.POINTER(C.c_uint64),
                                            C.POINTER(C.c_uint64)]),
    "g2s_test_bam_text": (C.c_int, [C.c_char_p, C.c_size_t, C.c_int, C.POINTER(C.c_uint32), C.c_uint64, C.c_int, C.c_int,
                                    C.POINTER(C.c_uint8), C.c_uint64, C.POINTER(C.c_uint64), C.POINTER(C.c_uint8), C.c_uint64,
                                    C.POINTER(C.c_uint64), C.POINTER(C.c_uint64), C.POINTER(C.c_uint64), C.c_uint64,
                                    C.POINTER(C.c_uint64)]),
    "g2s_test_bam_text_store": (C.c_int, [C.c_char_p, C.c_size_t, C.c_int, C.c_size_t, C.POINTER(C.c_uint32), C.c_uint64, C.c_int,
                                          C.c_int, C.POINTER(C.c_uint8), C.c_uint64, C.POINTER(C.c_uint64), C.POINTER(C.c_uint8),
                                          C.c_uint64, C.POINTER(C.c_uint64), C.POINTER(C.c_uint64), C.POINTER(C.c_uint64),
                                          C.c_uint64, C.POINTER(C.c_uint64)]),
    "g2s_test_filter_store_plan": (C.c_int, [C.c_char_p, C.c_size_t] + [C.POINTER(C.c_uint64)] * 6),
    "g2s_test_bam_store": (C.c_int, [C.c_char_p, C.c_size_t, C.c_int, C.c_size_t, C.POINTER(C.c_uint8), C.c_uint64,
                                     C.POINTER(C.c_uint64), C.POINTER(C.c_uint64), C.c_uint64, C.POINTER(C.c_uint64)]),
    "g2s_test_last_filter_store": (C.c_int, [C.POINTER(C.c_int)] + [C.POINTER(C.c_uint64)] * 5 + [C.POINTER(C.c_int)]),
    "g2s_graph_validate": (C.c_int64, [C.c_void_p, C.c_char_p, C.c_size_t]),
    "g2s_test_post_gap": (C.c_int, [_VP, C.POINTER(g2s_params), C.POINTER(g2s_gap), C.c_int32,
                                    C.POINTER(C.c_uint32), C.POINTER(C.c_int32), C.POINTER(C.c_uint32), C.c_int32,
                                    C.c_int32, C.POINTER(C.c_int32), C.c_int32, C.c_int32, C.c_uint32, C.c_uint32,
                                    C.POINTER(g2s_result), C.c_char_p]),
}


def library_path():
    return os.environ.get("G2S_LIBRARY") or os.path.join(os.path.dirname(os.path.abspath(__file__)), "libg2s_hip.so")


_LIB = None


def load_library():
    global _LIB
    if _LIB is None:
        path = library_path()
        if not os.path.exists(path):
            raise OSError("%s is missing: run `python -c 'import __graft_entry__ as g; g.build()'` "
                          "(hipcc, gfx950). There is no CPU fallback." % path)
        lib = C.CDLL(path)
        for name, (res, args) in _SIGS.items():
            fn = getattr(lib, name)
            fn.restype = res
            fn.argtypes = args
        _LIB = lib
    return _LIB


def _check(rc):
    if rc != G2S_OK:
        raise G2SError(rc, (load_library().g2s_last_error() or b"").decode("utf-8", "replace"))


def _take_text(ptr):
    lib = load_library()
    if not ptr:
        return ""
    s = C.string_at(ptr).decode("ascii")
    lib.g2s_free(ptr)
    return s


class G2S:

    @staticmethod
    def device_count():
        return load_library().g2s_device_count()

    @staticmethod
    def synth_genome(length, variant, seed):
        out = _VP()
        _check(load_library().g2s_synth_genome(length, variant, seed, C.byref(out)))
        return _take_text(out)

    @staticmethod
    def synth_gaps(reads_fasta, k, fuz, ngaps, min_len, max_len, seed):
        out = _VP()
        _check(load_library().g2s_synth_gaps(reads_fasta.encode("ascii"), k, fuz, ngaps, min_len, max_len, seed,
                                             C.byref(out)))
        return _take_text(out)


def cut_scaffolds(scaffolds_text, k=31, fuz=10, mask=False, no_split=False, labels=("scaffolds.fa", "contigs.fa", "gaps.fa", "gaps.bed")):
    outs = [_VP(), _VP(), _VP(), _VP()]
    _check(load_library().g2s_cut_scaffolds(scaffolds_text.encode("ascii"), k, fuz, int(mask), int(no_split),
                                            *[x.encode() for x in labels], *[C.byref(o) for o in outs]))
    return tuple(_take_text(o) for o in outs)


def merge_scaffolds(contigs_text, gaps_text, labels=("merged.fa", "contigs.fa", "filled.fa")):
    out, log = _VP(), _VP()
    _check(load_library().g2s_merge_scaffolds(contigs_text.encode("ascii"), gaps_text.encode("ascii"),
                                              *[x.encode() for x in labels], C.byref(out), C.byref(log)))
    return _take_text(out), _take_text(log)


def filter_reads(bam, mean, std_dev, scaffold, breakpoint, gap_length=-1, flank_length=-1, unmapped_only=False,
                 threads=0):
    lib = load_library()
    o = g2s_filter_opts(mean, std_dev, breakpoint, gap_length, flank_length, int(unmapped_only), threads,
                        scaffold.encode())
    outs = [_VP(), _VP(), _VP()]
    ext, tot = C.c_int64(0), C.c_int64(0)
    tail = [C.byref(o)] + [C.byref(x) for x in outs] + [C.byref(ext), C.byref(tot)]
    if isinstance(bam, (bytes, bytearray)):
        rc = lib.g2s_filter_reads_mem(bytes(bam), len(bam), *tail)
    else:
# ... 618 lines not shown
            res = rbuf.array(g2s_result, max(1, len(gaps)))
            hs = (_VP * len(sessions))(*[s.h for s in sessions])
            t = g2s_timing()
            try:
                _check(lib.g2s_team_fill(hs, len(sessions), arr, len(gaps), group_size, res, C.cast(arena.p, C.c_char_p), nbytes, C.byref(t)))
                raw = arena.raw
                out = [FillResult(res[i], raw) for i in range(len(gaps))]
            finally:
                arena.free()
                rbuf.free()
            return (out, t) if want_timing else out
        arena = C.create_string_buffer(max(1, nbytes))
        res = (g2s_result * max(1, len(gaps)))()
        prepared = (arr, keep, arena, res, nbytes)
    arr, keep, arena, res, nbytes = prepared
    hs = (_VP * len(sessions))(*[s.h for s in sessions])
    t = g2s_timing()
    _check(lib.g2s_team_fill(hs, len(sessions), arr, len(gaps), group_size, res, arena, nbytes, C.byref(t)))
    if want_timing == "raw":
        return prepared, t
    raw = arena.raw
    out = [FillResult(res[i], raw) for i in range(len(gaps))]
    return (out, t) if want_timing else out


class PreparedBatch:
    def __init__(self, session, gaps):
        lib = load_library()
        self.session = session
        self.n = len(gaps)
        self._arr, self._keep = _gap_array(gaps)
        self.h = _VP()
        _check(lib.g2s_batch_prepare(session.h, self._arr, self.n, C.byref(self.h)))
        self.nbytes = lib.g2s_batch_arena_bytes(self.h)
        self.arena = C.create_string_buffer(max(1, self.nbytes))
        self.res = (g2s_result * max(1, self.n))()

    def run(self):
        _check(load_library().g2s_batch_run(self.h, self.res, self.arena, self.nbytes))

    def timing(self):
        t = g2s_timing()
        _check(load_library().g2s_batch_timing(self.h, C.byref(t)))
        return t

    def results(self):
        raw = self.arena.raw
        return [FillResult(self.res[i], raw) for i in range(self.n)]

    def free(self):
        if self.h:
            load_library().g2s_batch_free(self.h)
            self.h = None


def test_post_gap(graph, params, gap, states, c_count, lengths, reached_j, final_d, seed, skip):
    lib = load_library()
    arr, keep = _gap_array([gap])
    n = len(states)
    nodes = (C.c_uint32 * max(1, n))(*[s[0] for s in states])
    depths = (C.c_int32 * max(1, n))(*[s[1] for s in states])
    counts = (C.c_uint32 * max(1, n))(*[s[2] for s in states])
    lens = (C.c_int32 * 2)(*(list(lengths) + [0, 0])[:2])
    res = g2s_result()
    buf = C.create_string_buffer(gap.gap_len + graph.k + params.d_err + gap.lmf + gap.rmf + 3)
    _check(lib.g2s_test_post_gap(graph.h, C.byref(params), arr, n, nodes, depths, counts, c_count, len(lengths), lens,
                                 reached_j, final_d, seed, skip, C.byref(res), buf))
    return FillResult(res, buf.raw)


def test_post_closure(graph, params, gap, records, xp, c_count, lengths, reached_j, final_d, seed, skip):
    lib = load_library()
    arr, keep = _gap_array([gap])
    n = len(records)
    flat = (C.c_uint32 * max(1, 4 * n))()
    for i, (node, cnt, meta, pred) in enumerate(records):
        flat[4 * i], flat[4 * i + 1], flat[4 * i + 2], flat[4 * i + 3] = node, cnt, meta, pred & 0xFFFFFFFF
    xs = (C.c_uint64 * max(1, len(xp)))(*xp)
    lens = (C.c_int32 * 2)(*(list(lengths) + [0, 0])[:2])
    res = g2s_result()
    buf = C.create_string_buffer(gap.gap_len + graph.k + params.d_err + gap.lmf + gap.rmf + 3)
    _check(lib.g2s_test_post_closure(graph.h, C.byref(params), arr, n, flat, len(xp), xs, c_count, len(lengths), lens,
                                     reached_j, final_d, seed, skip, C.byref(res), buf))
    return FillResult(res, buf.raw)


def test_post_segments(graph, params, gap, segs, c_count, lengths, reached_j, final_d, seed, skip):
    lib = load_library()
    arr, keep = _gap_array([gap])
    flat = (C.c_uint32 * max(1, 8 * len(segs)))()
    for i, rec in enumerate(segs):
        for q in range(8):
            flat[8 * i + q] = rec[q] & 0xFFFFFFFF
    lens = (C.c_int32 * 2)(*(list(lengths) + [0, 0])[:2])
    res = g2s_result()
    on = C.c_int32(0)
    buf = C.create_string_buffer(gap.gap_len + graph.k + params.d_err + gap.lmf + gap.rmf + 3)
    _check(lib.g2s_test_post_segments(graph.h, C.byref(params), arr, len(segs), flat, c_count, len(lengths), lens,
                                      reached_j, final_d, seed, skip, C.byref(res), buf, C.byref(on)))
    return FillResult(res, buf.raw), bool(on.value)


def test_seg_expand(graph, params, gap, segs, lengths, reached_j, n_records, n_xp):
    lib = load_library()
    arr, keep = _gap_array([gap])
    flat = (C.c_uint32 * max(1, 8 * len(segs)))()
    for i, rec in enumerate(segs):
        for q in range(8):
            flat[8 * i + q] = rec[q] & 0xFFFFFFFF
    lens = (C.c_int32 * 2)(*(list(lengths) + [0, 0])[:2])
    out = (C.c_uint32 * max(1, 4 * n_records))()
    xs = (C.c_uint64 * max(1, n_xp))()
    _check(lib.g2s_test_seg_expand(graph.h, C.byref(params), arr, len(segs), flat, len(lengths), lens, reached_j,
                                   n_records, out, n_xp, xs))
    recs = [(out[4 * i], out[4 * i + 1], out[4 * i + 2], out[4 * i + 3] - (1 << 32) if out[4 * i + 3] >> 31 else out[4 * i + 3])
            for i in range(n_records)]
    return recs, sorted(xs[i] for i in range(n_xp))


def test_graph_tables(graph):
    n = graph.num_kmers
    succ = (C.c_uint32 * max(1, 8 * n))()
    words = (C.c_uint64 * max(1, (n + 63) // 64))()
    _check(load_library().g2s_test_graph_tables(graph.h, succ, words))
    return succ, words


def test_worker_pool(threads, rounds, n):
    _check(load_library().g2s_test_worker_pool(threads, rounds, n))


def test_group_queue(nworkers, n, group_size):
    owner = (C.c_int32 * max(1, n))()
    _check(load_library().g2s_test_group_queue(nworkers, n, group_size, owner))
    return [owner[i] for i in range(n)]


def test_device_rand(device, seed, skip, n):
    out = (C.c_int32 * max(1, n))()
    _check(load_library().g2s_test_device_rand(device, seed, skip, n, out))
    return [out[i] for i in range(n)]


def test_d3_tables(device, segs, n_len, len0, len1, start_seg, rnd, base, R, dmin, dspread):
    flat = [w for s in segs for w in s]
    sa = (C.c_uint32 * max(1, len(flat)))(*flat)
    ra = (C.c_uint32 * max(1, len(rnd)))(*rnd)
    ent, bad, anom = (C.c_uint16 * (R + 1))(), (C.c_uint8 * (R + 1))(), C.c_uint32()
    _check(load_library().g2s_test_d3_tables(device, sa, len(segs), n_len, len0, len1, start_seg, ra, len(rnd), base, R, dmin,
                                             dspread, ent, bad, C.byref(anom)))
    return list(ent), list(bad), anom.value


def test_d3_chain_launches():
    return int(load_library().g2s_test_d3_chain_launches())


def test_group_queue_slow(nworkers, n, group_size, slow_worker, slow_us):
    owner = (C.c_int32 * max(1, n))()
    _check(load_library().g2s_test_group_queue_slow(nworkers, n, group_size, slow_worker, slow_us, owner))
    return [owner[i] for i in range(n)]


def test_rand_skip(seed, skip, n):
    out = (C.c_int32 * max(1, n))()
    _check(load_library().g2s_test_rand_skip(seed, skip, n, out))
    return [out[i] for i in range(n)]


def test_rand_stream(seed, skip, n):
    out = (C.c_int32 * max(1, n))()
    _check(load_library().g2s_test_rand_stream(seed, skip, n, out))
    return [out[i] for i in range(n)]


def reach_radius(gap, d_err):
    return max(0, gap.gap_len + d_err) + gap.lmf + gap.rmf


def test_last_pool_reach():
    a, b, d = C.c_uint64(), C.c_uint64(), C.c_uint64()
    known, on = C.c_int(), C.c_int()
    lv = C.c_uint32()
    _check(load_library().g2s_test_last_pool_reach(C.byref(a), C.byref(b), C.byref(known), C.byref(d), C.byref(lv), C.byref(on)))
    return dict(reach_sets=a.value, full_kmers=b.value if known.value else None, kept_kmers=d.value, levels=lv.value,
                on_device=on.value)


def test_seg_back_record(graph, device, node):
    out = (C.c_uint32 * 5)()
    _check(load_library().g2s_test_seg_back_record(graph.h, device, node, out))
    return list(out[:4]), out[4]


def test_last_pool_build():
    a, b, c, d = C.c_uint64(), C.c_uint64(), C.c_uint64(), C.c_int()
    _check(load_library().g2s_test_last_pool_build(C.byref(a), C.byref(b), C.byref(c), C.byref(d)))
    return dict(own_positions=a.value, shared_positions=b.value, keys_sorted=c.value, on_device=d.value)


def test_last_solid_count():
    pos, mx, so = C.c_uint64(), C.c_uint64(), C.c_uint64()
    ps, rf, on = C.c_uint32(), C.c_uint32(), C.c_int()
    _check(load_library().g2s_test_last_solid_count(C.byref(pos), C.byref(ps), C.byref(rf), C.byref(mx), C.byref(so), C.byref(on)))
    return dict(positions=pos.value, passes=ps.value, refined_bins=rf.value, max_pass_keys=mx.value, solid=so.value,
                on_device=on.value)


def test_plan_passes(hist, cap):
    nb = len(hist)
    h = (C.c_uint64 * max(1, nb))(*hist)
    first = (C.c_uint32 * max(1, nb))()
    n, over = C.c_uint32(), C.c_uint32()
    _check(load_library().g2s_test_plan_passes(h, nb, cap, first, nb, C.byref(n), C.byref(over)))
    assert n.value <= nb
    return list(first[:n.value]), (over.value if over.value < nb else None)


def test_filter_join(ref_id, pos, end, flag, h_own, h_mate, max_span, bits, windows, max_pairs, device=-1, threads=1):
    lib = load_library()
    nr, n = len(pos), len(windows) // 3
    assert len(windows) == 3 * n and all(len(x) == nr for x in (ref_id, end, flag, h_own, h_mate))
    flat = [v for w in windows for v in w]
    args = [(C.c_int32 * max(1, nr))(*ref_id), (C.c_int32 * max(1, nr))(*pos), (C.c_int64 * max(1, nr))(*end),
            (C.c_uint32 * max(1, nr))(*flag), (C.c_uint64 * max(1, nr))(*h_own), (C.c_uint64 * max(1, nr))(*h_mate)]
    win = (C.c_int64 * max(1, len(flat)))(*flat)
    cap1 = cap2 = 1 << 16
    while True:
        l1, l2 = (C.c_uint64 * cap1)(), (C.c_uint64 * cap2)()
        n1, n2 = C.c_uint64(0), C.c_uint64(0)
        rc = lib.g2s_test_filter_join(device, threads, nr, *args, max_span, bits, n, win, max_pairs, l1, cap1,
                                      C.byref(n1), l2, cap2, C.byref(n2))
        if rc != G2S_OK or (n1.value <= cap1 and n2.value <= cap2):
            break
        cap1, cap2 = max(cap1, n1.value), max(cap2, n2.value)
    msg = (lib.g2s_filter_last_error() or b"").decode("utf-8", "replace")
    return rc, [(x >> 32, x & 0xFFFFFFFF) for x in l1[:n1.value]], [(x >> 32, x & 0xFFFFFFFF) for x in l2[:n2.value]], msg


def reads_text(data, device=-1, piece_bytes=0):
    lib = load_library()
    data = bytes(data)
    cap = max(1 << 12, 2 * len(data))
    while True:
        out = (C.c_uint8 * cap)()
        n = C.c_size_t(0)
        _check(lib.g2s_test_reads_text(data, len(data), device, piece_bytes, out, cap, C.byref(n)))
        if n.value <= cap:
            return bytes(out[:n.value])
        cap = n.value


def last_reads_load():
    f, rb, ps, rc, pc, gr = (C.c_uint64() for _ in range(6))
    on = C.c_int()
    _check(load_library().g2s_test_last_reads_load(C.byref(f), None, None, None, None, None, None, 0, None))
    how = (C.c_int * max(1, f.value))()
    _check(load_library().g2s_test_last_reads_load(C.byref(f), C.byref(rb), C.byref(ps), C.byref(rc), C.byref(pc), C.byref(on),
                                                   how, f.value, C.byref(gr)))
    return dict(files=f.value, raw_bytes=rb.value, positions=ps.value, records=rc.value, pieces=pc.value,
                on_device=on.value, inflate=[("none", "zlib", "device", "mixed", "device-gzip")[x] for x in how[:f.value]], grows=gr.value)


BAM_READS_REASONS = ("kernels", "not asked", "rows anomaly", "over the cap", "hip")


def last_reads_bam():
    f, kept, skipped = C.c_uint64(), C.c_uint64(), C.c_uint64()
    kernels, reason, anomaly = C.c_int(), C.c_int(), C.c_int()
    _check(load_library().g2s_test_last_reads_bam(C.byref(f), C.byref(kept), C.byref(skipped), C.byref(kernels),
                                                  C.byref(reason), C.byref(anomaly)))
    return dict(files=f.value, kept=kept.value, skipped=skipped.value, kernels=kernels.value,
                reason=BAM_READS_REASONS[reason.value], anomaly=anomaly.value)


def last_reads_bam_stream():
    f, w, peak = C.c_uint64(), C.c_uint64(), C.c_uint64()
    _check(load_library().g2s_test_last_reads_bam_stream(C.byref(f), C.byref(w), C.byref(peak)))
    return dict(streamed_files=f.value, windows=w.value, peak_device_bytes=peak.value)


GZIP_OUTCOMES = ("done", "too few starts", "boundary mismatch", "slot full", "corrupt", "trailer", "memory", "hip", "header")


def set_device_gzip(mode=1):
    return load_library().g2s_reads_set_device_gzip(int(mode))


def gzip_inflate(data, device=-1, chunk_bytes=0, window_chunks=0):
    lib = load_library()
    data = bytes(data)
    cap = max(1 << 16, 8 * len(data))
    while True:
        out = (C.c_uint8 * cap)()
        n, oc = C.c_size_t(0), C.c_int(0)
        _check(lib.g2s_test_gzip_inflate(data, len(data), device, chunk_bytes, window_chunks, out, cap, C.byref(n), C.byref(oc)))
        if n.value <= cap:
            return bytes(out[:n.value]), GZIP_OUTCOMES[oc.value]
        cap = n.value


def last_reads_gzip():
    v = [C.c_uint64() for _ in range(7)]
    oc = C.c_int()
    _check(load_library().g2s_test_last_reads_gzip(C.byref(v[0]), C.byref(v[1]), C.byref(v[2]), C.byref(v[3]), C.byref(v[4]),
                                                   C.byref(v[5]), C.byref(oc), C.byref(v[6])))
# ... 138 lines not shown
```

Measured before the change: 3.213 million.

## Stash per-gap records in LDS during front scan and prefetch trace segments early

For short gap lists, the front kernel now stashes each gap's sub-address, start and length fields in shared memory during classification. The scan writes the full variant descriptors and tile map directly from that stash, skipping its second pass over global memory and one block barrier. The chained trace kernel issues its segment-record and random-window loads into registers before the offset-chain walk and copies them into LDS afterwards, so that load latency overlaps the walk. The trace LDS layout is moved to put the chain table after the main region, which costs extra shared memory and a second specialized front kernel.

```diff
diff --git a/gap2seq_amd/csrc/d3_device.h b/gap2seq_amd/csrc/d3_device.h
--- a/gap2seq_amd/csrc/d3_device.h
+++ b/gap2seq_amd/csrc/d3_device.h
@@ -163,6 +163,11 @@
                           const uint32_t* rnd, uint64_t rnd_cap, uint32_t base, uint32_t R, uint32_t dmin, uint32_t dspread,
                           uint16_t* entries, uint8_t* bad, uint32_t* anomalies);
 
+hipError_t test_d3_front(uint32_t n, bool generic, const uint32_t* segs, uint32_t nsegs, int32_t n_len, int32_t len0, int32_t len1,
+                         uint32_t start_seg, const uint32_t* stops, uint32_t lmf, const uint32_t* rnd, uint64_t rnd_cap,
+                         uint32_t* vdesc, uint32_t* tile_var, uint32_t tile_cap, uint16_t* entries, uint8_t* bad, uint32_t entry_cap,
+                         uint64_t* counts);
+
 uint64_t d3_chain_launches();
 
 }
diff --git a/gap2seq_amd/csrc/d3_device.hip b/gap2seq_amd/csrc/d3_device.hip
--- a/gap2seq_amd/csrc/d3_device.hip
+++ b/gap2seq_amd/csrc/d3_device.hip
@@ -74,18 +74,21 @@
 __device__ __forceinline__ uint32_t d3_classify_body(const D3Params& P, const D3Work& W, const GapOut* __restrict__ outs,
                                                      const D3Gap* __restrict__ dgaps, uint32_t first, uint32_t stride,
                                                      uint32_t* l_gi, uint32_t* l_dm, uint32_t* l_ds, int32_t* l_sk,
-                                                     unsigned long long* red, bool one_wg) {
+                                                     uint4* l_st, unsigned long long* red, bool one_wg) {
   const uint32_t n = P.n;
   unsigned long long xA = 0, sA = 0, xB = 0, sB = 0, xD = 0, sD = 0, segs = 0;
   uint32_t unhandled = 0, seg_gaps = 0, big = 0, traced = 0, spec = 0, handoff = 0;
   for (uint32_t i = first; i < n; i += stride) {
     const D3Gap dg = dgaps[i];
     const GapOut& go = outs[i];
-    const uint32_t flags = go.flags, n_states = go.n_states, n_right = go.n_right, x_right = go.x_right, x_left = go.x_left;
-    const uint32_t x_sub = go.x_sub, n_sub = go.n_sub, nseg_b = go.stat[3], dflags = go.dflags, stop0 = go.stop[0], stop1 = go.stop[1];
-    const int c_count = go.c_count, n_len = go.n_len, len0 = go.len[0], len1 = go.len[1], reached_j = go.reached_j, count_s = go.count_s;
-    const uint32_t n_xl = go.n_xl;
+    uint32_t flags = go.flags, n_states = go.n_states, n_right = go.n_right, x_right = go.x_right, x_left = go.x_left;
+    uint32_t nseg_b = go.stat[3], dflags = go.dflags, stop0 = go.stop[0], stop1 = go.stop[1];
+    const uint32_t x_sub = go.x_sub, n_sub = go.n_sub;
+    const int c_count = go.c_count, n_len = go.n_len, len0 = go.len[0], len1 = go.len[1], reached_j = go.reached_j;
+    int count_s = go.count_s;
+    const uint32_t n_xl = go.n_xl, start_seg = go.start_seg, start_t = go.start_t;
     const uint64_t sub_off = go.sub_off;
+    asm volatile("" : "+v"(flags), "+v"(n_states), "+v"(n_right), "+v"(x_right), "+v"(x_left), "+v"(nseg_b), "+v"(dflags), "+v"(stop0), "+v"(stop1), "+v"(count_s));
     uint32_t gi = 0, dmin = 0, spread = 0;
     if (dg.kind != 0) gi = GI_BAD;
     else {
@@ -136,7 +139,10 @@
     const uint64_t ao = P.arena_base + dg.arena_off, sa = (uint64_t)(i / P.group_size) * P.sub_region + sub_off;
     h0.x = (uint32_t)ao; h0.y = (uint32_t)(ao >> 32); h0.z = (uint32_t)sa; h0.w = (uint32_t)(sa >> 32);
     ((uint4*)&W.tdesc[i])[0] = h0;
-    (void)n_xl;
+    if (l_st) {
+      l_st[2u * i] = make_uint4(h0.z, h0.w, start_seg, start_t);
+      l_st[2u * i + 1u] = make_uint4((uint32_t)len0, (uint32_t)len1, (uint32_t)n_len, n_xl);
+    }
   }
   xA = wave_add64(xA); sA = wave_add64(sA); xB = wave_add64(xB); sB = wave_add64(sB); xD = wave_add64(xD); sD = wave_add64(sD);
   segs = wave_add64(segs);
@@ -175,7 +181,7 @@
 __global__ __launch_bounds__(256) void g2s_d3_classify(const D3Params P, const D3Work W, const GapOut* __restrict__ outs,
                                                        const D3Gap* __restrict__ dgaps) {
   __shared__ unsigned long long red[4 * 8];
-  (void)d3_classify_body(P, W, outs, dgaps, blockIdx.x * blockDim.x + threadIdx.x, gridDim.x * blockDim.x, nullptr, nullptr, nullptr, nullptr, red, false);
+  (void)d3_classify_body(P, W, outs, dgaps, blockIdx.x * blockDim.x + threadIdx.x, gridDim.x * blockDim.x, nullptr, nullptr, nullptr, nullptr, nullptr, red, false);
 }
 
 __device__ __forceinline__ void block_scan3(uint64_t& a, uint64_t& b, uint32_t& c, uint64_t* sh , uint64_t* tot_a, uint64_t* tot_b,
@@ -220,7 +226,8 @@
 
 __device__ __forceinline__ void d3_scan_body(const D3Params& P, const D3Work& W, const GapOut* __restrict__ outs, uint32_t* gi_a,
                                              uint32_t* dm_a, uint32_t* ds_a, const int32_t* sk_a, bool dual, uint32_t unhandled,
-                                             uint64_t* sh , uint32_t* sh_f , bool short_list ) {
+                                             uint64_t* sh , uint32_t* sh_f , bool short_list ,
+                                             const uint4* l_st = nullptr) {
   const uint32_t t = threadIdx.x, n = P.n;
   const uint32_t per = (n + 1023u) / 1024u;
   const uint32_t lo = min(n, t * per), hi = min(n, lo + per);
@@ -352,6 +359,14 @@
           uint4 h0, h1;
           h0.x = i; h0.y = (uint32_t)r; h0.z = (uint32_t)to; h0.w = tl;
           h1.x = base_i; h1.y = m8[q]; h1.z = s8[q]; h1.w = 0u;
+          if (l_st) {
+            const uint4 s0 = l_st[2u * i], s1 = l_st[2u * i + 1u];
+            h1.w = s1.w;
+            ((uint4*)&W.vdesc[v])[2] = s0;
+            ((uint4*)&W.vdesc[v])[3] = make_uint4(s1.x, s1.y, s1.z, 0u);
+            const uint32_t nt = (uint32_t)((r + D3_TILE) / D3_TILE);
+            for (uint32_t x = 0; x < nt; x++) W.tile_var[tl + x] = v;
+          }
           ((uint4*)&W.vdesc[v])[0] = h0;
           ((uint4*)&W.vdesc[v])[1] = h1;
         }
@@ -363,9 +378,9 @@
       }
     }
     if (t == 1023u) { W.var_toff[V] = (uint32_t)T; W.var_tile[V] = tiles; W.blk_toff[(V + G2S_D3_BLOCK_VARS - 1u) / G2S_D3_BLOCK_VARS] = (uint32_t)TB; }
-    __threadfence_block();
-    __syncthreads();
-    for (uint32_t v = t; v < V; v += 1024u) {
+    if (!l_st) __threadfence_block();
+    if (!l_st) __syncthreads();
+    for (uint32_t v = t; v < V && !l_st; v += 1024u) {
       const uint4 h0 = ((const uint4*)&W.vdesc[v])[0];
       const uint32_t i = h0.x, r = h0.y, tl0 = h0.w;
       const GapOut& go = outs[i];
@@ -893,18 +908,24 @@
 }
 
 #define D3_FRONT_GAPS 3072u
+#define D3_CHAIN_GAPS 768u
+#define D3_CHAIN_ROOM 4096u
+#define D3_WIN_AHEAD 1280u
+template <uint32_t CAP, bool STASH>
 __global__ __launch_bounds__(1024) void g2s_d3_front(const D3Params P, const D3Work W, const GapOut* __restrict__ outs,
                                                      const D3Gap* __restrict__ dgaps) {
   __shared__ uint64_t sh[96];
   __shared__ unsigned long long red[16 * 8];
   __shared__ uint32_t sh_f[1024];
-  __shared__ uint32_t l_gi[D3_FRONT_GAPS], l_dm[D3_FRONT_GAPS], l_ds[D3_FRONT_GAPS];
-  __shared__ int32_t l_sk[D3_FRONT_GAPS];
+  __shared__ uint32_t l_gi[CAP], l_dm[CAP], l_ds[CAP];
+  __shared__ int32_t l_sk[CAP];
+  __shared__ uint4 l_stash[STASH ? 2u * CAP : 1u];
+  uint4* l_st = STASH ? l_stash : nullptr;
   if (threadIdx.x == 0) stamp(W, 0);
-  const uint32_t unhandled = d3_classify_body(P, W, outs, dgaps, threadIdx.x, 1024u, l_gi, l_dm, l_ds, l_sk, red, true);
+  const uint32_t unhandled = d3_classify_body(P, W, outs, dgaps, threadIdx.x, 1024u, l_gi, l_dm, l_ds, l_sk, l_st, red, true);
   __syncthreads();
   if (threadIdx.x == 0) stamp(W, 1);
-  d3_scan_body(P, W, outs, l_gi, l_dm, l_ds, l_sk, true, unhandled, sh, sh_f, true);
+  d3_scan_body(P, W, outs, l_gi, l_dm, l_ds, l_sk, true, unhandled, sh, sh_f, true, l_st);
   if (threadIdx.x == 0) stamp(W, 2);
 }
 
@@ -1016,7 +1037,7 @@
                                                       const uint32_t* __restrict__ rnd, uint64_t capacity, const g2s::D3Side side) {
   __shared__ unsigned long long red[4 * 8];
   D3Summary* S = W.sum;
-  (void)d3_classify_body(P, W, outs, dgaps, blockIdx.x * 256u + threadIdx.x, gridDim.x * 256u, nullptr, nullptr, nullptr, nullptr, red, false);
+  (void)d3_classify_body(P, W, outs, dgaps, blockIdx.x * 256u + threadIdx.x, gridDim.x * 256u, nullptr, nullptr, nullptr, nullptr, nullptr, red, false);
   (void)d3_handoff_body<true>(P, W, outs, sub, rnd, capacity, side, blockIdx.x * 256u + (threadIdx.x & ~63u), nullptr, nullptr, nullptr, nullptr);
   if ((threadIdx.x & 63u) == 0u) {
     asm volatile("s_waitcnt vmcnt(0)" ::: "memory");
@@ -1031,8 +1052,6 @@
   }
 }
 #define D3_BACK_TAB 24576u
-#define D3_CHAIN_GAPS 768u
-#define D3_CHAIN_ROOM 4096u
 __global__ __launch_bounds__(1024) void g2s_d3_back(const D3Params P, const D3Work W, const GapOut* __restrict__ outs,
                                                     const SubRec* __restrict__ sub, const uint32_t* __restrict__ Wd, uint64_t capacity,
                                                     const g2s::D3Side side) {
@@ -1094,6 +1113,9 @@
   }
 }
 
+__host__ __device__ __forceinline__ uint32_t d3_trace_lds_words(const D3Params& P) {
+  return (P.seg_cap * (uint32_t)(sizeof(SegRec) + 16) + P.map_cap * 8u + 16u) / 4u;
+}
 template <int NW, bool CHAIN = false>
 __global__ __launch_bounds__(64 * NW) void g2s_d3_trace(const D3Params P, const D3Work W, GapOut* __restrict__ outs,
                                                    const SubRec* __restrict__ sub, const char* __restrict__ chu,
@@ -1118,16 +1140,17 @@
   static_assert(sizeof(g2s_result) == 112, "g2s_result layout");
   unsigned long long* laps = (unsigned long long*)((char*)W.sum + 512);
   const unsigned long long tk0 = P.laps ? wall_clock64() : 0ull;
-  unsigned long long tk1 = 0, tk2 = 0, tk3 = 0, hops = 0, tkm = 0;
+  unsigned long long tk1 = 0, tk2 = 0, tk3 = 0, hops = 0, tkm = 0, tkw = 0;
   if (P.laps && i == 0 && tid == 0) laps[13] = tk0;
   const uint32_t status = uni(S->status);
   struct {
-    uint32_t flags, dflags, start_seg, start_t, sub_vertices, sub_edges, top_level;
+    uint32_t flags, dflags, start_seg, start_t, sub_vertices, sub_edges, top_level, stat6, stat7;
     int32_t c_count, n_len, len[2], reached_j, count_s;
   } go;
   {
     const GapOut& g = outs[i];
     go.top_level = uni(g.top_level);
+    go.stat6 = uni(g.stat[6]); go.stat7 = uni(g.stat[7]);
     go.flags = uni(g.flags); go.dflags = uni(g.dflags); go.start_seg = uni(g.start_seg); go.start_t = uni(g.start_t);
     go.sub_vertices = uni(g.sub_vertices); go.sub_edges = uni(g.sub_edges);
     go.c_count = (int32_t)uni((uint32_t)g.c_count); go.n_len = (int32_t)uni((uint32_t)g.n_len);
@@ -1137,6 +1160,9 @@
   g2s::D3Trace td;
   uint32_t c_dmin = 0, c_vr = 0, c_base = 0, c_V = 0, c_dev = 0, c_step = 0, c_ns = 0, c_handoff = 0;
   uint64_t c_T = 0, c_draws_min = 0;
+  bool early = false, early_win = false;
+  uint4 cw0 = {}, cw1 = {};
+  uint32_t pw[D3_WIN_AHEAD / 256u] = {};
   if constexpr (!CHAIN) {
     const uint4 h0 = ((const uint4*)&W.tdesc[i])[0], h1 = ((const uint4*)&W.tdesc[i])[1];
     td.arena_off = (uint64_t)uni(h0.x) | ((uint64_t)uni(h0.y) << 32);
@@ -1147,7 +1173,7 @@
     const uint32_t n = P.n;
     const uint32_t toff_len = (n + 2u) & ~1u;
     const uint32_t tab_room = chain_room > toff_len ? min(chain_room - toff_len, D3_CHAIN_ROOM) & ~1u : 0u;
-    uint16_t* ltoff = (uint16_t*)lds;
+    uint16_t* ltoff = (uint16_t*)(lds + d3_trace_lds_words(P));
     uint16_t* ltab = ltoff + toff_len;
     const uint4 h0 = ((const uint4*)&W.tdesc[i])[0];
     uint32_t gi_w = W.ginfo[i], dm_w = W.dmin[i], vr_w = W.vrank[i], bs_w = W.base[i], ns_w = outs[i].n_xl, V_w = S->n_var;
@@ -1175,6 +1201,23 @@
     c_dmin = uni(dm_w); c_vr = uni(vr_w); c_base = uni(bs_w); c_V = uni(V_w); c_handoff = uni(hg_w);
     c_T = (uint64_t)uni((uint32_t)c_T) | ((uint64_t)uni((uint32_t)(c_T >> 32)) << 32);
     c_draws_min = (uint64_t)uni((uint32_t)c_draws_min) | ((uint64_t)uni((uint32_t)(c_draws_min >> 32)) << 32);
+    asm volatile("" ::: "memory");
+    const bool reach = !status && (td.gi & GI_PHASE_D) && !(td.gi & (GI_BAD | GI_SKIPPED | GI_MEM | GI_HOST)) &&
+                       !(go.dflags & (G2S_DEVA_TRACED | G2S_DEVA_D2_PENDING));
+    early = reach && c_ns != 0u && c_ns <= P.seg_cap;
+    {
+      const uint4* src = early ? (const uint4*)(sub + td.sub_at) : (const uint4*)&W.tdesc[i];
+      const uint32_t last = early ? 2u * c_ns - 1u : 0u;
+      cw0 = src[min((uint32_t)tid, last)];
+      cw1 = src[min((uint32_t)tid + 256u, last)];
+    }
+    early_win = reach && (uint64_t)c_base < capacity;
+    {
+      const uint32_t* src = early_win ? rnd + c_base : (const uint32_t*)&W.tdesc[i];
+      const uint32_t last = early_win ? (uint32_t)min(capacity - c_base - 1ull, 0xFFFFFFFFull) : 0u;
+#pragma unroll
+      for (uint32_t q = 0; q < D3_WIN_AHEAD / 256u; q++) pw[q] = src[min((uint32_t)tid + 256u * q, last)];
+    }
     __syncthreads();
     if (!status) {
       const bool in_lds = c_T <= (uint64_t)tab_room && c_T <= 0xFFFFull && c_V <= n;
@@ -1218,6 +1261,7 @@
       }
     }
     __syncthreads();
+    if (P.laps) tkw = wall_clock64();
   }
   bool d2_lost = false;
   if ((go.dflags & G2S_DEVA_D2_PENDING) && !(go.dflags & (G2S_DEVA_RUNS | G2S_DEVA_D2_FAILED)) && !P.skip_confident) {
@@ -1286,7 +1330,8 @@
         atomicMax(&laps[14], tk1 ? tk1 - tk0 : 0ull); atomicMax(&laps[15], tk2 ? tk2 - tk1 : 0ull);
         atomicMax(&laps[16], tk3 ? tk3 - tk2 : 0ull); atomicMax(&laps[17], ((tk4 - tk0) << 24) | ((td.gi & GI_HOST) ? 1ull << 23 : 0ull) | (unsigned long long)(i & 0x7FFFFFu)); atomicMax(&laps[18], tk4);
         atomicMax(&laps[19], ((tk2 ? tk2 - tk1 : 0ull) << 32) | (hops << 16) | (tkm ? tkm - tk1 : 0ull));
-        if ((P.laps >> 4) == i + 1u) { laps[26] = tk0; laps[27] = tk1; laps[28] = tkm; laps[29] = tk2; laps[30] = tk3; laps[31] = tk4; }
+        atomicMax(&laps[34], tkw ? tkw - tk0 : 0ull);
+        if ((P.laps >> 4) == i + 1u) { laps[26] = tk0; laps[27] = tk1; laps[28] = tkm; laps[29] = tk2; laps[30] = tk3; laps[31] = tk4; laps[35] = tkw; }
       }
       const uint32_t c = i & 63u, n = gridDim.x;
       const unsigned long long before = atomicAdd(&W.fill_bytes[c * 16u], (unsigned long long)fill_len | (1ull << 40));
@@ -1333,7 +1378,7 @@
   }
   const bool spec = (go.dflags & G2S_DEVA_SPEC) != 0u && W.spec_text != nullptr && !(gi & (GI_BAD | GI_SKIPPED | GI_MEM | GI_HOST)) && (gi & GI_PHASE_D);
   const int spec_stop = (int)(go.top_level & 0xFFFFu), spec_len = (int)(go.top_level >> 16);
-  const unsigned long long spec_chain = spec ? ((unsigned long long)uni(outs[i].stat[6]) | ((unsigned long long)uni(outs[i].stat[7]) << 32)) : 0ull;
+  const unsigned long long spec_chain = spec ? ((unsigned long long)go.stat6 | ((unsigned long long)go.stat7 << 32)) : 0ull;
   struct { uint16_t lmf; } dg = {td.lmf};
   const uint64_t abs_off = td.arena_off;
   char* buf = arena + abs_off;
@@ -1430,11 +1475,28 @@
   uint32_t* cmap = lds + (size_t)P.seg_cap * 8u;
   uint32_t* lwin = cmap + P.map_cap;
   const uint32_t nwin = min(td.want, P.map_cap);
-  for (uint32_t x = (uint32_t)tid; x < nwin; x += (uint32_t)NT) lwin[x] = (uint64_t)td.off + x < capacity ? rnd[td.off + x] : 0u;
+  uint32_t covered = 0;
+  if (CHAIN && early_win) {
+    const uint32_t dv = td.off - c_base;
+#pragma unroll
+    for (uint32_t q = 0; q < D3_WIN_AHEAD / 256u; q++) {
+      const uint32_t g = (uint32_t)tid + 256u * q;
+      if (g >= dv && g - dv < nwin) lwin[g - dv] = (uint64_t)c_base + g < capacity ? pw[q] : 0u;
+    }
+    covered = dv < D3_WIN_AHEAD ? D3_WIN_AHEAD - dv : 0u;
+  }
+  for (uint32_t x = (uint32_t)tid; x < nwin; x += (uint32_t)NT)
+    if (x >= covered) lwin[x] = (uint64_t)td.off + x < capacity ? rnd[td.off + x] : 0u;
   if (!big) {
     const uint4* src = (const uint4*)gsegs;
     uint4* dst = (uint4*)segs;
-    for (uint32_t w = (uint32_t)tid; w < 2u * nsegs; w += (uint32_t)NT) dst[w] = src[w];
+    uint32_t w = (uint32_t)tid;
+    if (CHAIN && early) {
+      if (w < 2u * nsegs) dst[w] = cw0;
+      if (w + 256u < 2u * nsegs) dst[w + 256u] = cw1;
+      w += 512u;
+    }
+    for (; w < 2u * nsegs; w += (uint32_t)NT) dst[w] = src[w];
   }
   __syncthreads();
   if (P.laps) tk1 = wall_clock64();
@@ -1884,6 +1946,79 @@
   return e;
 }
 
+hipError_t test_d3_front(uint32_t n, bool generic, const uint32_t* segs, uint32_t nsegs, int32_t n_len, int32_t len0, int32_t len1,
+                         uint32_t start_seg, const uint32_t* stops, uint32_t lmf, const uint32_t* rnd, uint64_t rnd_cap,
+                         uint32_t* vdesc, uint32_t* tile_var, uint32_t tile_cap, uint16_t* entries, uint8_t* bad, uint32_t entry_cap,
+                         uint64_t* counts) {
+  std::vector<SegW> hs(std::max(nsegs, 1u));
+  for (uint32_t q = 0; q < nsegs; q++) {
+    SegW w = {};
+    w.depth_len = segs[4u * q]; w.par01 = segs[4u * q + 1u]; w.par23 = segs[4u * q + 2u]; w.flags = segs[4u * q + 3u];
+    hs[q] = w;
+  }
+  const size_t n_rnd = 31u + (size_t)rnd_cap + 64u;
+  std::vector<uint32_t> hr(n_rnd, 0u);
+  for (uint64_t x = 0; x < rnd_cap; x++) hr[31u + x] = rnd[x];
+  auto start_t = [&](int pick) -> uint32_t {
+    const uint32_t sg = (start_seg >> (16 * pick)) & 0xFFFFu;
+    const int t = sg < nsegs ? (pick ? len1 : len0) - (int)(segs[4u * sg] & 0xFFFFu) : 0;
+    return t >= 0 && t <= 0xFFFF ? (uint32_t)t : 0u;
+  };
+  std::vector<GapOut> ho(n);
+  std::vector<D3Gap> hg(n);
+  for (uint32_t i = 0; i < n; i++) {
+    GapOut g;
+    memset(&g, 0, sizeof g);
+    g.c_count = 1; g.count_s = 1; g.n_len = n_len; g.len[0] = len0; g.len[1] = len1;
+    g.n_xl = nsegs; g.stat[3] = nsegs; g.sub_off = 0;
+    g.start_seg = start_seg; g.start_t = start_t(0) | (start_t(1) << 16);
+    g.dflags = G2S_DEVA_ANALYSED; g.stop[0] = stops[2u * i]; g.stop[1] = stops[2u * i + 1u];
+    ho[i] = g;
+    D3Gap d;
+    memset(&d, 0, sizeof d);
+    d.arena_off = (uint64_t)i * 64u; d.skip_thr = -1; d.lmf = (uint16_t)lmf;
+    hg[i] = d;
+  }
+  void *d_work = nullptr, *d_outs = nullptr, *d_gaps = nullptr, *d_seg = nullptr, *d_rnd = nullptr, *d_bad = nullptr;
+  auto release = [&]() { for (void* p : {d_work, d_outs, d_gaps, d_seg, d_rnd, d_bad}) if (p) (void)hipFree(p); };
+  hipError_t e = hipSuccess;
+  auto ok = [&](hipError_t x) { if (e == hipSuccess) e = x; return e == hipSuccess; };
+  const size_t work = d3_work_bytes(n);
+  D3Summary sum = {};
+  if (ok(hipMalloc(&d_work, work)) && ok(hipMalloc(&d_outs, n * sizeof(GapOut))) && ok(hipMalloc(&d_gaps, n * sizeof(D3Gap))) &&
+      ok(hipMalloc(&d_seg, hs.size() * sizeof(SegW))) && ok(hipMalloc(&d_rnd, n_rnd * 4)) && ok(hipMalloc(&d_bad, std::max(entry_cap, 1u))) &&
+      ok(hipMemset(d_work, 0, work - (size_t)G2S_D3_TABLE_BUDGET * 2)) && ok(hipMemset(d_bad, 0xFF, std::max(entry_cap, 1u))) &&
+      ok(hipMemcpy(d_outs, ho.data(), n * sizeof(GapOut), hipMemcpyHostToDevice)) &&
+      ok(hipMemcpy(d_gaps, hg.data(), n * sizeof(D3Gap), hipMemcpyHostToDevice)) &&
+      ok(hipMemcpy(d_seg, hs.data(), hs.size() * sizeof(SegW), hipMemcpyHostToDevice)) &&
+      ok(hipMemcpy(d_rnd, hr.data(), n_rnd * 4, hipMemcpyHostToDevice))) {
+    D3Params P;
+    memset(&P, 0, sizeof P);
+    P.n = n; P.group_size = n; P.all_paths = 1; P.max_states = ~0ull; P.seg_cap = 192u; P.k = 31;
+    P.map_cap = ((uint32_t)std::max(std::max(len0, len1), 0) + 2u + 3u) & ~3u;
+    D3Work W;
+    d3_work_carve(d_work, n, &W);
+    W.tab_bad = (uint8_t*)d_bad;
+    if (ok(hipMemset(W.tab, 0xFF, (size_t)entry_cap * 2))) {
+      if (n <= D3_CHAIN_GAPS && !generic) hipLaunchKernelGGL((g2s_d3_front<D3_CHAIN_GAPS, true>), dim3(1), dim3(1024), 0, nullptr, P, W, (const GapOut*)d_outs, (const D3Gap*)d_gaps);
+      else hipLaunchKernelGGL((g2s_d3_front<D3_FRONT_GAPS, false>), dim3(1), dim3(1024), 0, nullptr, P, W, (const GapOut*)d_outs, (const D3Gap*)d_gaps);
+      if (ok(hipGetLastError()) && ok(hipDeviceSynchronize()) && ok(hipMemcpy(&sum, W.sum, sizeof sum, hipMemcpyDeviceToHost))) {
+        const bool fits = sum.status == 0u && sum.table_entries <= (uint64_t)entry_cap && sum.tiles <= tile_cap;
+        if (fits && ok(launch_tables(nullptr, P, W, (const SubRec*)d_seg, (uint32_t*)d_rnd, rnd_cap)) && ok(hipDeviceSynchronize()) &&
+            ok(hipMemcpy(entries, W.tab, (size_t)sum.table_entries * 2, hipMemcpyDeviceToHost)) &&
+            ok(hipMemcpy(bad, d_bad, (size_t)sum.table_entries, hipMemcpyDeviceToHost)) &&
+            ok(hipMemcpy(tile_var, W.tile_var, (size_t)sum.tiles * 4, hipMemcpyDeviceToHost)))
+          (void)ok(hipMemcpy(&sum, W.sum, sizeof sum, hipMemcpyDeviceToHost));
+        (void)ok(hipMemcpy(vdesc, W.vdesc, ((size_t)n + 1u) * sizeof(D3Var), hipMemcpyDeviceToHost));
+        counts[0] = sum.status; counts[1] = sum.n_var; counts[2] = sum.tiles; counts[3] = sum.table_entries; counts[4] = sum.anomalies;
+        counts[5] = sum.draws_min; counts[6] = sum.draws_spread; counts[7] = fits ? 1u : 0u;
+      }
+    }
+  }
+  release();
+  return e;
+}
+
 hipError_t launch_rand_window(hipStream_t st, uint32_t* rnd_all, const uint32_t* link) {
   hipLaunchKernelGGL(g2s_rand_window, dim3(1), dim3(64), 0, st, rnd_all, link);
   return hipGetLastError();
@@ -1941,8 +2076,13 @@
   if (P.restart) {
     if (ev_d2) { e = hipStreamWaitEvent(st, ev_d2, 0); if (e != hipSuccess) return e; }
     hipLaunchKernelGGL(g2s_d3_restart, dim3((P.n + 255u) / 256u), dim3(256), 0, st, P, W, outs, dgaps, sub, rnd_all + 31, rnd_capacity, side);
-  } else if (short_list) hipLaunchKernelGGL(g2s_d3_front, dim3(1), dim3(1024), 0, st, P, W, outs, dgaps);
-  else {
+  } else if (short_list) {
+    const char* gen_s = GENV("G2S_TEST_FRONT_GENERIC");
+    if (P.n <= D3_CHAIN_GAPS && !(gen_s && atoi(gen_s) != 0))
+      hipLaunchKernelGGL((g2s_d3_front<D3_CHAIN_GAPS, true>), dim3(1), dim3(1024), 0, st, P, W, outs, dgaps);
+    else
+      hipLaunchKernelGGL((g2s_d3_front<D3_FRONT_GAPS, false>), dim3(1), dim3(1024), 0, st, P, W, outs, dgaps);
+  } else {
     hipLaunchKernelGGL(g2s_d3_classify, dim3((P.n + 255u) / 256u), dim3(256), 0, st, P, W, outs, dgaps);
     launch_scan(st, P, W, outs);
   }
@@ -1951,7 +2091,7 @@
   const char* waves_s = GENV("G2S_TRACE_WAVES");
   const int waves_env = waves_s ? atoi(waves_s) : 0;
   const bool four = waves_env ? waves_env == 4 : P.n <= 768u;
-  const size_t lds = (size_t)P.seg_cap * (sizeof(SegRec) + 16) + (size_t)P.map_cap * 8 + 16;
+  size_t lds = (size_t)d3_trace_lds_words(P) * 4u;
   bool chain_in_trace = false;
   uint32_t chain_room = 0;
   static_assert(D3_CHAIN_GAPS <= 768u, "g2s_d3_trace<4, true> is the four-wave kernel");
@@ -1959,8 +2099,10 @@
     const char* back_s = GENV("G2S_D3_BACK");
     chain_in_trace = !(back_s && atoi(back_s) != 0);
     const char* room_s = GENV("G2S_TEST_CHAIN_ROOM");
-    chain_room = (uint32_t)std::min<size_t>(lds / 2u, 0x7FFFFFFFu);
+    const uint32_t toff_len = (P.n + 2u) & ~1u;
+    chain_room = toff_len + D3_CHAIN_ROOM;
     if (room_s) chain_room = std::min(chain_room, (uint32_t)std::max(atoi(room_s), 0));
+    if (chain_in_trace) lds += ((size_t)std::max(chain_room, toff_len) * 2u + 15u) & ~(size_t)15u;
   }
   if (P.restart) (void)ev_chain;
   else if (chain_in_trace) (void)ev_chain;
diff --git a/gap2seq_amd/csrc/g2s_api.hip b/gap2seq_amd/csrc/g2s_api.hip
--- a/gap2seq_amd/csrc/g2s_api.hip
+++ b/gap2seq_amd/csrc/g2s_api.hip
@@ -3572,7 +3572,7 @@
   if (timed) HIP_TRY_S(hipEventElapsedTime(&ms_d3, d3_begin, s->ev[3]));
   *ms_d3_out = ms_d3;
   if (GENV("G2S_DEBUG")) {
-    unsigned long long lp[34];
+    unsigned long long lp[36];
     HIP_TRY_S(hipMemcpy(lp, (char*)W.sum + 512, sizeof lp, hipMemcpyDeviceToHost));
     auto us = [&](int a, int b) { return lp[a] && lp[b] ? ((double)lp[b] - (double)lp[a]) / 100.0 : -1.0; };
     fprintf(stderr, "[g2s] phase D3 laps (us): front classify %.1f scan %.1f | to tables %.1f: status %.1f records %.1f closure %.1f walks %.1f | to back %.1f: tables into LDS %.1f chain %.1f hand-off %.1f fence %.1f | to trace %.1f, longest wave: to closure %.1f walk %.1f bases %.1f all %.1f, first entry to last end %.1f\n",
@@ -3581,6 +3581,8 @@
     fprintf(stderr, "[g2s] the longest wave of the trace kernel: gap %llu%s\n", lp[17] & 0x7FFFFFull, (lp[17] >> 23) & 1ull ? " (handed to the host)" : "");
     fprintf(stderr, "[g2s] scan (us): sums %.1f, base + layout pass %.1f, table offsets + records %.1f\n", us(20, 21), us(21, 22), us(22, 23));
     fprintf(stderr, "[g2s] the last wave of the trace kernel: the summary's copy to the host begins %.1f us after the kernel's first entry and takes %.1f us\n", us(13, 24), us(24, 25));
+    if (lp[34]) fprintf(stderr, "[g2s] the trace kernel's longest walk of the offsets' chain ends %.1f us after its wave's entry\n", lp[34] / 100.0);
+    if (GENV("G2S_DEBUG_GAP") && lp[26] && lp[35]) fprintf(stderr, "[g2s] gap %s in the trace kernel: the offsets' chain walked %.1f us after its entry\n", GENV("G2S_DEBUG_GAP"), us(26, 35));
     if (GENV("G2S_DEBUG_GAP") && lp[26])
       fprintf(stderr, "[g2s] gap %s in the trace kernel (us): enters %.1f behind the kernel's first wave | to closure in LDS %.1f | chain %.1f | bases classified %.1f | text %.1f | record %.1f\n",
               GENV("G2S_DEBUG_GAP"), us(13, 26), us(26, 27), us(27, 28), us(28, 29), us(29, 30), us(30, 31));
@@ -4967,6 +4969,21 @@
   return G2S_OK;
 }
 
+extern "C" int g2s_test_d3_front(int device, uint32_t n, int generic, const uint32_t* segs, uint32_t n_segs, int32_t n_len, int32_t len0,
+                                 int32_t len1, uint32_t start_seg, const uint32_t* stops, uint32_t lmf, const uint32_t* rnd,
+                                 uint64_t rnd_cap, uint32_t* vdesc, uint32_t* tile_var, uint32_t tile_cap, uint16_t* entries,
+                                 uint8_t* bad, uint32_t entry_cap, uint64_t* counts) {
+  if (n < 1 || n > 3072u || (!segs && n_segs) || (!rnd && rnd_cap) || !stops || !vdesc || !tile_var || !entries || !bad || !counts ||
+      n_segs > 0xFFFFu || n_len < 1 || n_len > 2 || lmf > 0xFFFFu || (uint64_t)entry_cap > (uint64_t)G2S_D3_TABLE_BUDGET)
+    return fail(G2S_ERR_ARG, "g2s_test_d3_front: bad argument");
+  int ndev = 0;
+  if (hipGetDeviceCount(&ndev) != hipSuccess || device < 0 || device >= ndev) return fail(G2S_ERR_NO_DEVICE, "no such device");
+  HIP_TRY(hipSetDevice(device));
+  HIP_TRY(test_d3_front(n, generic != 0, segs, n_segs, n_len, len0, len1, start_seg, stops, lmf, rnd, rnd_cap, vdesc, tile_var, tile_cap,
+                        entries, bad, entry_cap, counts));
+  return G2S_OK;
+}
+
 extern "C" uint64_t g2s_test_d3_chain_launches(void) { return d3_chain_launches(); }
 
 extern "C" int g2s_test_rand_skip(uint32_t seed, uint64_t skip, uint32_t n, int32_t* out) {
diff --git a/gap2seq_amd/lib.py b/gap2seq_amd/lib.py
--- a/gap2seq_amd/lib.py
+++ b/gap2seq_amd/lib.py
@@ -224,6 +224,10 @@
     "g2s_test_d3_tables": (C.c_int, [C.c_int, C.POINTER(C.c_uint32), C.c_uint32, C.c_int32, C.c_int32, C.c_int32, C.c_uint32,
                                      C.POINTER(C.c_uint32), C.c_uint64, C.c_uint32, C.c_uint32, C.c_uint32, C.c_uint32,
                                      C.POINTER(C.c_uint16), C.POINTER(C.c_uint8), C.POINTER(C.c_uint32)]),
+    "g2s_test_d3_front": (C.c_int, [C.c_int, C.c_uint32, C.c_int, C.POINTER(C.c_uint32), C.c_uint32, C.c_int32, C.c_int32, C.c_int32,
+                                    C.c_uint32, C.POINTER(C.c_uint32), C.c_uint32, C.POINTER(C.c_uint32), C.c_uint64,
+                                    C.POINTER(C.c_uint32), C.POINTER(C.c_uint32), C.c_uint32, C.POINTER(C.c_uint16),
+                                    C.POINTER(C.c_uint8), C.c_uint32, C.POINTER(C.c_uint64)]),
     "g2s_test_d3_chain_launches": (C.c_uint64, []),
     "g2s_test_post_closure": (C.c_int, [_VP, C.POINTER(g2s_params), C.POINTER(g2s_gap), C.c_uint32,
                                         C.POINTER(C.c_uint32), C.c_uint32, C.POINTER(C.c_uint64), C.c_int32, C.c_int32,
@@ -1148,6 +1152,23 @@
     return list(ent), list(bad), anom.value
 
 
+def test_d3_front(device, n, generic, segs, n_len, len0, len1, start_seg, stops, lmf, rnd, tile_cap=4096, entry_cap=1 << 20):
+    flat = [w for s in segs for w in s]
+    sa = (C.c_uint32 * max(1, len(flat)))(*flat)
+    ra = (C.c_uint32 * max(1, len(rnd)))(*rnd)
+    st = (C.c_uint32 * (2 * n))(*[w for s in stops for w in s])
+    vd, tv = (C.c_uint32 * (16 * (n + 1)))(), (C.c_uint32 * tile_cap)()
+    ent, bad, counts = (C.c_uint16 * entry_cap)(), (C.c_uint8 * entry_cap)(), (C.c_uint64 * 8)()
+    _check(load_library().g2s_test_d3_front(device, n, int(generic), sa, len(segs), n_len, len0, len1, start_seg, st, lmf, ra, len(rnd),
+                                            vd, tv, tile_cap, ent, bad, entry_cap, counts))
+    names = ("status", "n_var", "tiles", "table_entries", "anomalies", "draws_min", "draws_spread", "fits")
+    out = dict(zip(names, [int(c) for c in counts]))
+    T, tiles = (out["table_entries"], out["tiles"]) if out["fits"] else (0, 0)
+    out.update(vdesc=[list(vd[16 * v:16 * v + 16]) for v in range(n + 1)], tile_var=list(tv[:tiles]), entries=list(ent[:T]),
+               bad=list(bad[:T]))
+    return out
+
+
 def test_d3_chain_launches():
     return int(load_library().g2s_test_d3_chain_launches())
 
```

New measurement: 3.198 million. Within noise of the previous version (-0.5%).
